# CCIG-Champalimaud/adell-mri

Hardware: AMD Instinct MI355X
Metric: volumes/sec 3D U-Net 128^3 2-ch seg (train step: fwd+loss+bwd+SGD) (higher is better)
Workload: dtype f32 (f16x3 split MFMA, fp32 accumulate); 1 GPU; BASELINE configs[1]: u-net-3d-resnet.yaml UNetPL, 2x128^3, batch 2/GPU, dice+focal, SGD-Nesterov; per_gpu_batch=2, parallelism=dp1, yaml=configs/u-net-3d-resnet.yaml, built_by=parse_config_unet -> get_segmentation_network('unet'), gradient_exchange=none (1 rank)

## Files before the change

### adell_mri_amd/_lib.py

```python
import ctypes
import os

_HERE = os.path.dirname(os.path.abspath(__file__))
LIB_PATH = os.environ.get("ADELL_HIP_LIBRARY") or os.path.join(_HERE, "libadellhip.so")

_lib = None

OK = 0
E_BADARG, E_UNSUPPORTED, E_HIP, E_NOMEM = -1, -2, -3, -4

ACT_IDS = {
    "identity": 0, "swish": 1, "silu": 1, "relu": 2, "leaky_relu": 3, "prelu": 4,
    "gelu": 5, "sigmoid": 6, "tanh": 7, "elu": 8,
}


class AdellHipError(RuntimeError):
    pass


class ConvDesc(ctypes.Structure):
    _fields_ = [(n, ctypes.c_int32) for n in (
        "N", "D", "H", "W", "C0", "C1", "Cout", "KD", "KH", "KW", "SD", "SH", "SW",
        "PD", "PH", "PW", "Do", "Ho", "Wo")]


class NormActDesc(ctypes.Structure):
    _fields_ = [
        ("N", ctypes.c_int64), ("V", ctypes.c_int64), ("C", ctypes.c_int32),
        ("stats_per_item", ctypes.c_int32), ("act", ctypes.c_int32),
        ("act_w_n", ctypes.c_int32), ("act_p", ctypes.c_float),
        ("drop_p", ctypes.c_float), ("seed", ctypes.c_uint64),
        ("rng_offset", ctypes.c_uint32),
    ]


class AdnSite(ctypes.Structure):
    _fields_ = [("y", ctypes.c_void_p), ("mean", ctypes.c_void_p), ("rstd", ctypes.c_void_p),
                ("keep_mask", ctypes.c_void_p), ("drop_p", ctypes.c_float),
                ("act_p", ctypes.c_float), ("act", ctypes.c_int32)]


_vp, _i, _l, _f = ctypes.c_void_p, ctypes.c_int, ctypes.c_long, ctypes.c_float
_d = ctypes.c_double

DECONF_MAX_HEADS = 8


class DeconfHeads(ctypes.Structure):
    _fields_ = [("n_heads", ctypes.c_int32), ("n_cont", ctypes.c_int32),
                ("K", ctypes.c_int32 * DECONF_MAX_HEADS), ("W", _vp * DECONF_MAX_HEADS),
                ("b", _vp * DECONF_MAX_HEADS), ("Wc", _vp), ("bc", _vp)]


class DeconfHeadGrads(ctypes.Structure):
    _fields_ = [("dW", _vp * DECONF_MAX_HEADS), ("db", _vp * DECONF_MAX_HEADS), ("dWc", _vp),
                ("dbc", _vp)]


class AttentionDesc(ctypes.Structure):
    _fields_ = [("BH", ctypes.c_int32), ("H", ctypes.c_int32), ("T", ctypes.c_int32),
                ("A", ctypes.c_int32), ("Dv", ctypes.c_int32), ("scale", _f), ("drop_p", _f),
                ("rng_offset", ctypes.c_uint32), ("seed", ctypes.c_uint64), ("bias", _vp),
                ("labels", _vp), ("nbias", ctypes.c_int32), ("nlab", ctypes.c_int32),
                ("strided", ctypes.c_int32), ("stride", ctypes.c_int64 * 3 * 8)]


SIGNATURES = {
    "adell_abi_version": (_i, []),
    "adell_last_error": (ctypes.c_char_p, []),
    "adell_pack_weight": (_i, [_vp, _vp, _i, _i, _i, _i, _i, _i, _vp]),
    "adell_conv3d_fwd_ntiles": (_i, [ctypes.POINTER(ConvDesc)]),
    "adell_plan_epoch": (_l, []),
    "adell_conv3d_fwd": (_i, [ctypes.POINTER(ConvDesc), _vp, _vp, _vp, _vp, _vp, _vp, _vp, _i, _vp]),
    "adell_conv3d_bwd_data": (_i, [ctypes.POINTER(ConvDesc), _vp, _vp, _vp, _vp, _vp]),
    "adell_pack_weight_f16x3_bytes": (_l, [_i, _i, _i, _i]),
    "adell_pack_weight_f16x3": (_i, [_vp, _vp, _vp, _i, _i, _i, _i, _i, _i, _vp]),
    "adell_conv3d_fwd_ntiles_f16x3": (_i, [ctypes.POINTER(ConvDesc)]),
    "adell_conv3d_fwd_ntiles_f16x3_ws": (_i, [ctypes.POINTER(ConvDesc)]),
    "adell_conv3d_fwd_f16x3": (_i, [ctypes.POINTER(ConvDesc)] + [_vp] * 8 + [_i, _vp, _vp]),
    "adell_conv3d_bwd_data_f16x3": (_i, [ctypes.POINTER(ConvDesc)] + [_vp] * 7),
    "adell_pack_weight_f16x3_multi": (_i, [_vp, _i, _l, _vp]),
    "adell_conv3d_bwd_data_s2_f16x3": (_i, [ctypes.POINTER(ConvDesc)] + [_vp] * 6),
    "adell_conv3d_bwd_data_s2_f16x3_add": (_i, [ctypes.POINTER(ConvDesc)] + [_vp] * 7),
    "adell_conv3d_fwd_s2_fused_applicable": (_i, [ctypes.POINTER(ConvDesc)]),
    "adell_conv3d_fwd_s2_fused_ntiles": (_i, [ctypes.POINTER(ConvDesc)]),
    "adell_conv3d_fwd_s2_fused": (_i, [ctypes.POINTER(ConvDesc)] + [_vp] * 6 + [_i, _vp, _vp]),
    "adell_conv3d_bwd_data_s2_fused_applicable": (_i, [ctypes.POINTER(ConvDesc)]),
    "adell_conv3d_bwd_data_s2_fused": (_i, [ctypes.POINTER(ConvDesc)] + [_vp] * 7),
    "adell_conv3d_splitk_workspace": (_l, [ctypes.POINTER(ConvDesc), _i]),
    "adell_conv3d_f16x3_plan": (_i, [ctypes.POINTER(ConvDesc), _i, _vp]),
    "adell_conv3d_fwd_f16x3_ws": (_i, [ctypes.POINTER(ConvDesc)] + [_vp] * 8 + [_i, _vp, _vp,
                                                                         ctypes.c_size_t, _vp]),
    "adell_conv3d_bwd_data_f16x3_ws": (_i, [ctypes.POINTER(ConvDesc)] + [_vp] * 7 + [ctypes.c_size_t, _vp]),
    "adell_conv3d_bwd_data_f16x3_add": (_i, [ctypes.POINTER(ConvDesc)] + [_vp] * 7
                                        + [ctypes.c_size_t, _vp]),
    "adell_conv3d_bwd_weight_workspace": (_l, [ctypes.POINTER(ConvDesc)]),
    "adell_conv3d_bwd_weight": (_i, [ctypes.POINTER(ConvDesc), _vp, _vp, _vp, _vp, _vp, _vp, ctypes.c_size_t, _vp]),
    "adell_conv3d_bwd_weight_f16x3_workspace": (_l, [ctypes.POINTER(ConvDesc)]),
    "adell_conv3d_bwd_weight_f16x3": (_i, [ctypes.POINTER(ConvDesc), _vp, _vp, _vp, _vp, _vp, _vp, _vp, _vp, ctypes.c_size_t, _vp]),
    "adell_bias_grad_workspace": (_l, [_l, _i]),
    "adell_bias_grad": (_i, [_vp, _l, _i, _vp, _vp, ctypes.c_size_t, _vp]),
    "adell_convtranspose3d_k2s2_bwd_weight_workspace": (_l, [_i, _i, _i, _i, _i, _i]),
    "adell_convtranspose3d_k2s2_bwd_weight": (_i, [_i, _i, _i, _i, _i, _i, _vp, _vp, _vp, _vp, ctypes.c_size_t, _vp]),
    "adell_convtranspose3d_fwd": (_i, [_i] * 9 + [_vp] * 5),
    "adell_convtranspose3d_bwd_data": (_i, [_i] * 9 + [_vp] * 4),
    "adell_convtranspose3d_bwd_weight_workspace": (_l, [_i] * 9),
    "adell_convtranspose3d_bwd_weight": (_i, [_i] * 9 + [_vp] * 4 + [ctypes.c_size_t, _vp]),
    "adell_convtranspose3d_k2s2_fwd": (_i, [_i, _i, _i, _i, _i, _i, _vp, _vp, _vp, _vp, _vp]),
    "adell_convtranspose3d_k2s2_bwd_data": (_i, [_i, _i, _i, _i, _i, _i, _vp, _vp, _vp, _vp]),
    "adell_stats_finalize_workspace": (_l, [_i, _i, _i]),
    "adell_stats_finalize": (_i, [_vp, _i, _i, _i, _l, _f, _i, _vp, _vp, _vp, ctypes.c_size_t, _vp]),
    "adell_bn_running_update": (_i, [_vp] * 5 + [_i, _l, _f, _f, _vp]),
    "adell_bn_stats_sums": (_i, [_vp, _i, _i, _i, _l, _vp, _vp, ctypes.c_size_t, _vp]),
    "adell_bn_stats_from_sums": (_i, [_vp, _i, _f, _vp, _vp, _vp, _vp, _vp, _f, _vp]),
    "adell_channel_partials_ntiles": (_i, [_l]),
    "adell_channel_partials": (_i, [_vp, _i, _l, _i, _vp, _vp]),
    "adell_norm_act_fwd": (_i, [ctypes.POINTER(NormActDesc), _vp, _vp, _vp, _vp, _vp, _vp, _vp, _vp]),
    "adell_norm_act_mask_bytes": (_l, [ctypes.POINTER(NormActDesc)]),
    "adell_norm_act_fwd_split": (_i, [ctypes.POINTER(NormActDesc)] + [_vp] * 7 + [_i, _vp, _vp]),
    "adell_split_rows_from_f32": (_i, [_vp, _i, _l, _i, _vp, _vp, _vp]),
    "adell_split_rows_to_f32": (_i, [_vp, _i, _l, _i, _vp, _vp, _vp]),
    "adell_conv3d_f16x3_rows_ok": (_i, [ctypes.POINTER(ConvDesc)]),
    "adell_conv3d_bwd_weight_f16x3_rows_ok": (_i, [ctypes.POINTER(ConvDesc)]),
    "adell_conv3d_bwd_weight_f16x3_plan": (_i, [ctypes.POINTER(ConvDesc), _vp]),
    "adell_conv3d_bwd_weight_f16x3_rows": (_i, [ctypes.POINTER(ConvDesc)] + [_vp] * 10
                                           + [ctypes.c_size_t, _vp]),
    "adell_conv3d_bwd_weight_f16x3_share": (_i, [ctypes.POINTER(ConvDesc)] + [_vp] * 8
                                            + [ctypes.c_size_t, _vp, _i]),
    "adell_conv3d_bwd_weight_f16x3_rows_share": (_i, [ctypes.POINTER(ConvDesc)] + [_vp] * 10
                                                 + [ctypes.c_size_t, _vp, _i]),
    "adell_conv3d_fwd_f16x3_rows": (_i, [ctypes.POINTER(ConvDesc)] + [_vp] * 10 + [_i, _vp, _vp]),
    "adell_norm_act_fwd_mask": (_i, [ctypes.POINTER(NormActDesc)] + [_vp] * 9),
    "adell_norm_act_bwd_from_dt": (_i, [ctypes.POINTER(NormActDesc)] + [_vp] * 5 + [_i, _i, _i, _vp, _vp,
                                                                              ctypes.c_size_t, _vp]),
    "adell_conv3d_bwd_data_f16x3_adn_ntiles": (_i, [ctypes.POINTER(ConvDesc)]),
    "adell_conv3d_bwd_data_f16x3_adn": (_i, [ctypes.POINTER(ConvDesc)] + [_vp] * 7
                                        + [ctypes.POINTER(AdnSite), ctypes.POINTER(AdnSite), _vp, _i, _vp]),
    "adell_norm_act_bwd_workspace": (_l, [ctypes.POINTER(NormActDesc)]),
    "adell_norm_act_bwd": (_i, [ctypes.POINTER(NormActDesc)] + [_vp] * 11 + [ctypes.c_size_t, _vp]),
    "adell_norm_act_plan": (_i, [ctypes.POINTER(NormActDesc)] + [_i] * 6 + [_vp]),
    "adell_norm_act_stats_plan": (_i, [_i, _i, _i, _vp]),
    "adell_norm_act_bwd_sums": (_i, [ctypes.POINTER(NormActDesc)] + [_vp] * 11 + [ctypes.c_size_t, _vp]),
    "adell_norm_act_bwd_apply_sums": (_i, [ctypes.POINTER(NormActDesc)] + [_vp] * 10
                                      + [ctypes.c_size_t, _vp]),
    "adell_norm_act_bwd_lowrank": (_i, [ctypes.POINTER(NormActDesc), _vp, _vp, _vp, _i, _vp, _vp, _vp,
                                        _vp, ctypes.c_size_t, _vp]),
    "adell_dice_focal_workspace": (_l, [_i, _l]),
    "adell_dice_focal_fwd": (_i, [_vp, _vp, _i, _l, _f, _f, _f, _f, _f, _vp, _vp, _vp, _vp, ctypes.c_size_t, _vp]),
    "adell_dice_focal_bwd": (_i, [_vp, _vp, _i, _l, _f, _f, _f, _f, _f, _vp, _f, _f, _vp, _vp]),
    "adell_dice_focal_bwd_dev": (_i, [_vp, _vp, _i, _l, _f, _f, _f, _f, _f, _vp, _vp, _vp, _vp, _vp]),
    "adell_class_sums_workspace": (_l, [_i, _l, _i]),
    "adell_class_sums_fwd": (_i, [_vp, _vp, _i, _l, _i, _vp, _vp, ctypes.c_size_t, _vp]),
    "adell_class_sums_bwd": (_i, [_vp, _vp, _i, _l, _i, _vp, _vp]),
    "adell_sgd_step": (_i, [_vp, _vp, _vp, _l, _f, _f, _f, _i, _i, _f, _vp]),
    "adell_adamw_step": (_i, [_vp, _vp, _vp, _vp, _l, _f, _d, _d, _f, _f, _l, _f, _vp]),
    "adell_adam_step": (_i, [_vp, _vp, _vp, _vp, _l, _f, _d, _d, _f, _f, _l, _f, _vp]),
    "adell_ema_update": (_i, [_vp, _vp, _l, _f, _vp]),
    "adell_layernorm_fwd": (_i, [_vp, _vp, _vp, _vp, _vp, _vp, _l, _i, _f, _vp]),
    "adell_layernorm_bwd_workspace": (_l, [_l, _i]),
    "adell_layernorm_bwd": (_i, [_vp] * 8 + [_l, _i, _vp, ctypes.c_size_t, _vp]),
    "adell_add_bcast": (_i, [_vp, _vp, _vp, _l, _l, _vp]),
    "adell_sum_bcast": (_i, [_vp, _vp, _l, _l, _vp]),
    "adell_attention_fwd": (_i, [ctypes.POINTER(AttentionDesc)] + [_vp] * 6),
    "adell_attention_bwd": (_i, [ctypes.POINTER(AttentionDesc)] + [_vp] * 10),
    "adell_attention_plan": (_i, [_i] * 5 + [_vp]),
    "adell_attention_bias_grad_workspace_floats": (_l, [_i, _i]),
    "adell_attention_bias_grad": (_i, [ctypes.POINTER(AttentionDesc)] + [_vp] * 8 + [_l, _vp]),
    "adell_copy_channels": (_i, [_vp, _vp, _l, _i, _i, _i, _i, _vp]),
    "adell_interp_nearest_fwd": (_i, [_vp, _vp] + [_i] * 8 + [_vp]),
    "adell_interp_nearest_bwd": (_i, [_vp, _vp] + [_i] * 8 + [_vp]),
    "adell_interp_linear_fwd": (_i, [_vp, _vp] + [_i] * 8 + [_f] * 3 + [_i, _vp]),
    "adell_interp_linear_bwd": (_i, [_vp, _vp] + [_i] * 8 + [_f] * 3 + [_i, _vp]),
    "adell_fold_x_taps": (_i, [_vp, _vp] + [_i] * 8 + [_vp]),
    "adell_scale_bc": (_i, [_vp, _vp, _vp, _i, _l, _i, _vp]),
    "adell_scale_bc_dscale_workspace_floats": (_l, [_i, _l, _i]),
    "adell_scale_bc_dscale": (_i, [_vp, _vp, _vp, _i, _l, _i, _vp, _vp]),
    "adell_cse_apply": (_i, [_vp, _vp, _vp, _vp, _vp, _vp, _i, _l, _i, _vp]),
    "adell_cse_apply_bwd_workspace_floats": (_l, [_i, _l, _i]),
    "adell_cse_apply_bwd": (_i, [_vp, _vp, _vp, _vp, _vp, _vp, _vp, _vp, _i, _l, _i, _vp, _vp]),
    "adell_bcast_nc": (_i, [_vp, _vp, _i, _l, _i, _f, _vp]),
    "adell_maxpool3d_fwd": (_i, [ctypes.POINTER(ConvDesc), _vp, _vp, _vp, _vp]),
    "adell_maxpool3d_bwd": (_i, [ctypes.POINTER(ConvDesc), _vp, _vp, _vp, _vp]),
    "adell_dwconv3d_fwd": (_i, [_i] * 8 + [_vp] * 5),
    "adell_dwconv3d_bwd_data": (_i, [_i] * 8 + [_vp] * 4),
    "adell_dwconv3d_bwd_weight_workspace_floats": (_l, [_i] * 8),
    "adell_dwconv3d_bwd_weight": (_i, [_i] * 8 + [_vp] * 6),
    "adell_vicreg_scratch_floats": (_l, [_i, _i]),
    "adell_vicreg_fwd": (_i, [_vp, _vp, _i, _i, _f, _f, _vp, _vp, _vp]),
    "adell_vicreg_bwd": (_i, [_vp, _vp, _i, _i, _f, _f, _vp, _vp, _vp, _vp, _vp]),
    "adell_top_pairs_workspace_words": (_l, [_i, _i, _i]),
    "adell_top_pairs": (_i, [_vp, _vp, _i, _i, _i, _i, _vp, _l, _vp, _vp, _vp]),
    "adell_top_pairs_boxes": (_i, [_vp, _vp, _i, _i, ctypes.POINTER(ctypes.c_int), _i, _vp, _l, _vp,
                                   _vp, _vp]),
    "adell_gather_rows_fwd": (_i, [_vp, _vp, _i, _i, _i, _i, _i, _vp, _vp]),
    "adell_gather_rows_bwd": (_i, [_vp, _vp, _i, _i, _i, _i, _i, _vp, _vp]),
    "adell_dino_loss_plan": (_i, [_i, _i, _vp]),
    "adell_dino_loss_workspace_floats": (_l, [_i, _i]),
    "adell_dino_loss_fwd": (_i, [_vp, _vp, _vp, _i, _i, _f, _f, _i, _vp, _l, _vp, _vp, _vp, _vp]),
    "adell_dino_loss_bwd": (_i, [_vp, _vp, _vp, _vp, _vp, _vp, _f, _i, _i, _f, _f, _i, _vp, _vp,
                                 _vp]),
    "adell_dino_scores": (_i, [_vp, _vp, _vp, _i, _i, _i, _i, _f, _vp, _vp]),
    "adell_dino_center_sum": (_i, [_vp, _i, _i, _vp, _vp]),
    "adell_dino_center_apply": (_i, [_vp, _vp, _i, _f, _f, _f, _vp]),
    "adell_dino_sk_proto_sums": (_i, [_vp, _vp, _i, _i, _f, _vp, _vp]),
    "adell_dino_sk_sample_weights": (_i, [_vp, _vp, _i, _i, _f, _f, _vp, _vp]),
    "adell_dino_sk_final": (_i, [_vp, _vp, _vp, _i, _i, _f, _f, _vp, _vp]),
    "adell_l2_normalize_rows_fwd": (_i, [_vp, _i, _i, _f, _vp, _vp, _vp]),
    "adell_l2_normalize_rows_bwd": (_i, [_vp, _vp, _vp, _i, _i, _f, _vp, _vp]),
    "adell_row_inv_norm_fwd": (_i, [_vp, _vp, _i, _i, _vp, _vp]),
    "adell_row_inv_norm_bwd": (_i, [_vp, _vp, _vp, _i, _i, _vp, _vp]),
    "adell_row_mean_fwd": (_i, [_vp, _i, _i, _vp, _vp]),
    "adell_row_mean_bwd": (_i, [_vp, _i, _i, _vp, _vp]),
    "adell_col_scale": (_i, [_vp, _vp, _i, _i, _vp, _vp]),
    "adell_col_scale_dscale": (_i, [_vp, _vp, _i, _i, _vp, _vp]),
    "adell_ibot_mask_tokens_fwd": (_i, [_vp, _vp, _vp, _i, _i, _i, _i, _vp, _vp]),
    "adell_ibot_mask_tokens_bwd": (_i, [_vp, _vp, _i, _i, _i, _i, _vp, _vp, _vp]),
    "adell_ibot_token_sums_plan": (_i, [_i, _i, _i, _vp]),
    "adell_ibot_token_sums_workspace_doubles": (_l, [_i, _i, _i]),
    "adell_ibot_center_sum": (_i, [_vp, _i, _i, _vp, _vp]),
    "adell_ibot_token_sums": (_i, [_vp, _i, _i, _i, _i, _f, _vp, _l, _vp, _vp, _vp]),
    "adell_ibot_loss_fwd": (_i, [_vp, _vp, _vp, _vp, _i, _i, _i, _i, _f, _f, _i, _vp, _l, _vp, _vp,
                                 _vp, _vp]),
    "adell_ibot_bwd": (_i, [_vp, _vp, _vp, _vp, _vp, _vp, _vp, _i, _i, _i, _i, _i, _i, _f, _f, _i,
                            _vp, _vp]),
    "adell_ijepa_gather_fwd": (_i, [_vp, _vp, _i, _i, _i, _i, _vp, _vp]),
    "adell_ijepa_gather_bwd": (_i, [_vp, _vp, _i, _i, _i, _i, _vp, _vp]),
    "adell_ijepa_predictor_fwd": (_i, [_vp, _vp, _vp, _vp, _vp, _i, _i, _i, _i, _i, _vp, _vp]),
    "adell_ijepa_predictor_bwd": (_i, [_vp, _vp, _vp, _vp, _i, _i, _i, _i, _i, _vp, _vp, _vp, _vp]),
    "adell_ijepa_loss_fwd": (_i, [_vp, _vp, _vp, _i, _i, _i, _i, _vp, _vp, _vp, _vp]),
    "adell_ijepa_loss_bwd": (_i, [_vp, _vp, _vp, _vp, _vp, _i, _i, _i, _i, _vp, _vp]),
    "adell_mae_gather_rows": (_i, [_vp, _vp, _i, _i, _i, _i, _vp, _vp]),
    "adell_mae_restore_fwd": (_i, [_vp, _vp, _vp, _vp, _vp, _i, _i, _i, _i, _vp, _vp]),
    "adell_mae_restore_bwd_chunks": (_i, [_i, _i]),
    "adell_mae_restore_bwd": (_i, [_vp, _vp, _vp, _vp, _vp, _i, _i, _i, _i, _vp, _vp, _vp, _vp, _vp,
                                   _i, _vp]),
    "adell_mae_loss_fwd": (_i, [_vp, _vp, _i, _i, _i, _i, _vp, _vp, _vp]),
    "adell_mae_loss_bwd": (_i, [_vp, _vp, _vp, _i, _i, _i, _i, _vp, _vp]),
    "adell_mae_to_image": (_i, [_vp, _i, _i, _i, _i, _vp, _vp]),
    "adell_mae_from_image": (_i, [_vp, _i, _i, _i, _i, _vp, _vp]),
    "adell_cls_loss_fwd": (_i, [_i, _vp, _vp, _vp, _vp, _i, _i, _i, _vp, _vp, _vp, _vp]),
    "adell_cls_loss_bwd": (_i, [_i, _vp, _vp, _vp, _vp, _i, _vp, _i, _vp, _i, _i, _vp, _vp]),
    "adell_cls_roc_fwd": (_i, [_vp, _vp, _i, _vp, _vp, _vp, _vp]),
    "adell_cls_roc_bwd": (_i, [_vp, _vp, _vp, _vp, _i, _vp, _vp]),
    "adell_cls_mixup": (_i, [_vp, _vp, _vp, _i, _l, _vp, _vp]),
    "adell_cls_confusion_update": (_i, [_i, _vp, _vp, _vp, _l, _i, _vp, _vp]),
    "adell_cls_auroc_pairs": (_i, [_vp, _vp, _i, _vp, _vp]),
    "adell_mil_volume_to_slices": (_i, [_vp, _i, _i, _i, _i, _vp, _vp]),
    "adell_mil_slices_to_volume": (_i, [_vp, _i, _i, _i, _i, _vp, _vp]),
    "adell_mil_pool_fwd": (_i, [_i] + [_vp] * 5 + [_i] * 4 + [_vp] * 5),
    "adell_mil_pool_bwd": (_i, [_i] + [_vp] * 9 + [_i] * 4 + [_vp] * 7),
    "adell_mil_slice_tokens_fwd": (_i, [_vp, _vp, _vp, _i, _i, _i, _vp, _vp]),
    "adell_mil_slice_tokens_bwd": (_i, [_vp, _i, _i, _i, _i, _vp, _vp, _vp, _vp]),
    "adell_det_table_blocks": (_l, [_l]),
    "adell_det_positive_table": (_i, [_vp] + [_i] * 9 + [_f] + [_vp] * 4),
    "adell_det_loss_partials": (_l, [_l]),
    "adell_det_loss_fwd": (_i, [_vp] * 7 + [_f] * 3 + [_i] * 9 + [_vp] * 4),
    "adell_det_loss_bwd": (_i, [_vp] * 7 + [_f] * 3 + [_i] * 9 + [_vp] * 5),
    "adell_det_nms_max": (_i, []),
    "adell_det_nms": (_i, [_vp, _i, _f, _vp, _vp, _vp]),
    "adell_det_decode": (_i, [_vp] * 4 + [_i] + [_vp] * 3 + [_f] * 3 + [_i] * 6 + [_vp] * 5),
    "adell_det_match": (_i, [_vp, _vp, _i, _vp, _vp, _vp, _vp, _vp]),
    "adell_det_encode": (_i, [_vp] * 4 + [ctypes.c_double] * 4 + [_i] * 6 + [_vp, _vp]),
    "adell_adamw_amsgrad_step": (_i, [_vp, _vp, _vp, _vp, _vp, _l, _f, _d, _d, _f, _f, _l, _f, _vp]),
    "adell_eca_gates_fwd": (_i, [_vp, _i, _vp, _i, _vp, _i, _i, _f, _vp, _vp]),
    "adell_eca_gates_bwd": (_i, [_vp, _i, _vp, _vp, _i, _i, _vp]),
    "adell_eca_apply_fwd": (_i, [_vp, _vp, _i, _vp, _i, _l, _i, _vp]),
    "adell_eca_apply_bwd_workspace_doubles": (_l, [_i, _l, _i]),
    "adell_eca_apply_bwd": (_i, [_vp, _vp, _vp, _i, _vp, _vp, _vp, _i, _l, _i, _vp]),
    "adell_diffusion_noise": (_i, [_vp, _vp, _vp, _i, _vp, _vp, _i, _l, _vp]),
    "adell_diffusion_reverse_step": (_i, [_vp] * 5 + [_l] + [_f] * 7 + [_i, _vp]),
    "adell_mse_workspace_bytes": (_l, []),
    "adell_mse_fwd": (_i, [_vp, _vp, _l, _vp, _vp, _vp]),
    "adell_mse_bwd": (_i, [_vp, _vp, _vp, _l, _vp, _vp]),
    "adell_gp_route": (_i, [_i, _i, _i]),
    "adell_gp_phi_fwd": (_i, [_vp] * 6 + [_i] * 4 + [_f, _f] + [_vp] * 5),
    "adell_gp_phi_bwd": (_i, [_vp] * 11 + [_i] * 4 + [_f, _f] + [_vp] * 6),
    "adell_gp_cos": (_i, [_vp, _vp, _vp, _l, _i, _f, _vp, _vp]),
    "adell_gp_precision_update": (_i, [_vp, _vp, _i, _i, _i, _i, _f, _vp, _vp]),
    "adell_gp_variance": (_i, [_vp, _vp, _i, _i, _vp, _vp]),
    "adell_gp_sample": (_i, [_vp, _vp, _vp, _i, _i, _i, _vp, _vp, _vp, _vp]),
    "adell_ensemble_pool_fwd": (_i, [_vp, _vp, _vp, _i, _i, _vp, _vp, _vp]),
    "adell_ensemble_pool_bwd": (_i, [_vp, _vp, _vp, _vp, _i, _i, _vp, _vp]),
    "adell_ensemble_average_fwd": (_i, [_vp, _i, _i, _i, _vp, _vp]),
    "adell_ensemble_average_bwd": (_i, [_vp, _vp, _i, _i, _i, _vp, _vp]),
    "adell_be_expand": (_i, [_vp, _vp, _vp, _i, _i, _i, _f, _vp, _i, _l, _i, _vp]),
    "adell_be_members_sum": (_i, [_vp, _vp, _vp, _i, _i, _i, _f, _i, _vp, _i, _l, _i, _vp]),
    "adell_be_tgrad_workspace_doubles": (_l, [_i, _l, _i, _i]),
    "adell_be_tgrad": (_i, [_vp, _vp, _vp, _vp, _i, _i, _i, _f, _vp, _vp, _vp, _i, _l, _i, _vp]),
    "adell_deconf_split_fwd": (_i, [_vp, _vp, _vp, _i, _i, _i, _vp]),
    "adell_deconf_split_bwd": (_i, [_vp, _vp, _vp, _i, _i, _i, _vp]),
    "adell_deconf_corr_workspace_doubles": (_l, [_i, _i, _i]),
    "adell_deconf_corr_saved_doubles": (_l, [_i, _i, _i]),
    "adell_deconf_corr_fwd": (_i, [_vp, _i, _i, _i, _vp, _vp, _vp, _vp]),
    "adell_deconf_corr_bwd": (_i, [_vp, _vp, _vp, _i, _i, _i, _vp, _vp]),
# ... 193 lines not shown
```

### adell_mri_amd/csrc/norm_act.hip

```cpp
#include "common.h"

ADELL_RNG_STEP_DEFINE(norm_act)

#define ADELL_NA_GENERIC_MAXBLOCKS (256 * 16)
#define ADELL_NA_FAST_MAXROWS 1024
#define ADELL_NA_FAST_MAXC 1024
#define ADELL_STATS_FOLD_ABOVE 512
#define ADELL_STATS_FOLD_ROWS 256
#define ADELL_FIN8_SPAN 56
#define ADELL_FIN2_SPAN 32

__global__ __launch_bounds__(256) void adell_stats_finalize_kernel(
    const float* __restrict__ part, int N, int ntiles, int C, double count, float eps,
    int per_item, float* __restrict__ mean, float* __restrict__ rstd) {
  __shared__ double sh[8][32][2];
  const int cl = threadIdx.x & 31, sl = threadIdx.x >> 5;
  const int c = blockIdx.x * 32 + cl;
  const int nbeg = per_item ? blockIdx.y : 0, nend = per_item ? blockIdx.y + 1 : N;
  double s1 = 0.0, s2 = 0.0;
  if (c < C) {
    for (int n = nbeg; n < nend; ++n) {
      const float* p = part + ((size_t)n * ntiles * C + c) * 2;
      int t = sl;
      for (; t + ADELL_FIN8_SPAN < ntiles; t += 64) {
        float2 v[8];
#pragma unroll
        for (int u = 0; u < 8; ++u)
          v[u] = *reinterpret_cast<const float2*>(p + (size_t)(t + 8 * u) * C * 2);
#pragma unroll
        for (int u = 0; u < 8; ++u) {
          s1 += (double)v[u].x;
          s2 += (double)v[u].y;
        }
      }
      for (; t < ntiles; t += 8) {
        const float2 v = *reinterpret_cast<const float2*>(p + (size_t)t * C * 2);
        s1 += (double)v.x;
        s2 += (double)v.y;
      }
    }
  }
  sh[sl][cl][0] = s1;
  sh[sl][cl][1] = s2;
  __syncthreads();
  if (sl == 0 && c < C) {
    double a = 0.0, b = 0.0;
#pragma unroll
    for (int k = 0; k < 8; ++k) {
      a += sh[k][cl][0];
      b += sh[k][cl][1];
    }
    const double cnt = per_item ? count : count * N;
    const double m = a / cnt;
    double var = b / cnt - m * m;
    if (var < 0.0) var = 0.0;
    const size_t o = per_item ? (size_t)blockIdx.y * C + c : (size_t)c;
    mean[o] = (float)m;
    rstd[o] = (float)(1.0 / sqrt(var + (double)eps));
  }
}

__global__ __launch_bounds__(256) void adell_stats_fold_kernel(const float* __restrict__ part,
                                                               int ntiles, int C, int Z,
                                                               float* __restrict__ out,
                                                               int pstride, int poff) {
  __shared__ double sh[8][32][2];
  const int cl = threadIdx.x & 31, sl = threadIdx.x >> 5;
  const int c = blockIdx.x * 32 + cl, n = blockIdx.y, z = blockIdx.z;
  const int t0 = z * ADELL_STATS_FOLD_ROWS;
  const int t1 = t0 + ADELL_STATS_FOLD_ROWS < ntiles ? t0 + ADELL_STATS_FOLD_ROWS : ntiles;
  double s1 = 0.0, s2 = 0.0;
  if (c < C) {
    const float* p = part + ((size_t)n * ntiles * pstride + poff + c) * 2;
    int t = t0 + sl;
    for (; t + ADELL_FIN8_SPAN < t1; t += 64) {
      float2 v[8];
#pragma unroll
      for (int u = 0; u < 8; ++u)
        v[u] = *reinterpret_cast<const float2*>(p + (size_t)(t + 8 * u) * pstride * 2);
#pragma unroll
      for (int u = 0; u < 8; ++u) {
        s1 += (double)v[u].x;
        s2 += (double)v[u].y;
      }
    }
    for (; t < t1; t += 8) {
      const float2 v = *reinterpret_cast<const float2*>(p + (size_t)t * pstride * 2);
      s1 += (double)v.x;
      s2 += (double)v.y;
    }
  }
  sh[sl][cl][0] = s1;
  sh[sl][cl][1] = s2;
  __syncthreads();
  if (sl == 0 && c < C) {
    double a = 0.0, b = 0.0;
#pragma unroll
    for (int k = 0; k < 8; ++k) {
      a += sh[k][cl][0];
      b += sh[k][cl][1];
    }
    float* o = out + (((size_t)n * Z + z) * C + c) * 2;
    o[0] = (float)a;
    o[1] = (float)b;
  }
}

struct AdellNaStatsPlan {
  int levels;
  int Z;
  long ws_bytes;
};

static AdellNaStatsPlan adell_na_stats_plan(long N, long ntiles, long C) {
  AdellNaStatsPlan p = {1, 0, 0};
  if (ntiles <= ADELL_STATS_FOLD_ABOVE) return p;
  p.levels = 2;
  p.Z = (int)((ntiles + ADELL_STATS_FOLD_ROWS - 1) / ADELL_STATS_FOLD_ROWS);
  p.ws_bytes = (long)sizeof(float) * N * p.Z * C * 2;
  return p;
}

extern "C" long adell_stats_finalize_workspace(int N, int ntiles, int C) {
  return adell_na_stats_plan(N, ntiles, C).ws_bytes;
}

extern "C" int adell_norm_act_stats_plan(int N, int ntiles, int C, long* out) {
  ADELL_REQUIRE(out && N > 0 && ntiles > 0 && C > 0, "norm_act_stats_plan: bad arguments");
  const AdellNaStatsPlan p = adell_na_stats_plan(N, ntiles, C);
  out[0] = p.levels;
  out[1] = p.Z;
  out[2] = p.ws_bytes;
  out[3] = ADELL_FIN8_SPAN + 1;
  out[4] = ADELL_FIN2_SPAN + 1;
  return ADELL_OK;
}

extern "C" int adell_stats_finalize(const float* partials, int N, int ntiles, int C,
                                    long count, float eps, int per_item, float* mean,
                                    float* rstd, void* workspace, size_t workspace_bytes,
                                    void* stream) {
  ADELL_REQUIRE(N > 0 && ntiles > 0 && C > 0 && count > 0, "stats_finalize: bad dims");
  const AdellNaStatsPlan sp = adell_na_stats_plan(N, ntiles, C);
  ADELL_REQUIRE(sp.levels == 1 || (workspace && (long)workspace_bytes >= sp.ws_bytes),
                "stats_finalize: workspace too small");
  ADELL_REQUIRE(partials && mean && rstd, "stats_finalize: null pointer");
  hipStream_t st = (hipStream_t)stream;
  if (sp.levels == 2) {
    const int Z = sp.Z;
    hipLaunchKernelGGL(adell_stats_fold_kernel, dim3(adell_cdiv(C, 32), N, Z), dim3(256), 0, st,
                       partials, ntiles, C, Z, (float*)workspace, C, 0);
    partials = (const float*)workspace;
    ntiles = Z;
  }
  hipLaunchKernelGGL(adell_stats_finalize_kernel, dim3(adell_cdiv(C, 32), per_item ? N : 1),
                     dim3(256), 0, st, partials, N, ntiles, C, (double)count, eps, per_item, mean,
                     rstd);
  ADELL_CHECK_HIP(hipGetLastError());
  return ADELL_OK;
}

__global__ __launch_bounds__(256) void adell_bn_running_update_kernel(
    const float* __restrict__ mean, const float* __restrict__ rstd, float* __restrict__ rmean,
    float* __restrict__ rvar, long long* __restrict__ nbt, int C, float unbias, float eps,
    float momentum) {
  long long t = nbt != nullptr ? nbt[0] + 1 : 0;
  const float mom = momentum >= 0.f ? momentum : 1.f / (float)t;
  __syncthreads();
  for (int c = threadIdx.x; c < C; c += 256) {
    const float r = rstd[c];
    const float var = (1.f / (r * r) - eps) * unbias;
    rmean[c] = rmean[c] * (1.f - mom) + mom * mean[c];
    rvar[c] = rvar[c] * (1.f - mom) + mom * var;
  }
  if (threadIdx.x == 0 && nbt != nullptr) nbt[0] = t;
}

extern "C" int adell_bn_running_update(const float* mean, const float* rstd, float* running_mean,
                                       float* running_var, long long* num_batches_tracked, int C,
                                       long count, float eps, float momentum, void* stream) {
  ADELL_REQUIRE(mean && rstd && running_mean && running_var && C > 0 && count > 0,
                "bn_running_update: bad arguments");
  ADELL_REQUIRE(momentum >= 0.f || num_batches_tracked != nullptr,
                "bn_running_update: the cumulative average needs num_batches_tracked");
  const float unbias = (float)((double)count / (double)(count > 1 ? count - 1 : 1));
  hipLaunchKernelGGL(adell_bn_running_update_kernel, dim3(1), dim3(256), 0, (hipStream_t)stream, mean,
                     rstd, running_mean, running_var, num_batches_tracked, C, unbias, eps, momentum);
  ADELL_CHECK_HIP(hipGetLastError());
  return ADELL_OK;
}

#define ADELL_STATS_SLAB 1024
__global__ __launch_bounds__(256) void adell_channel_partials_kernel(
    const float* __restrict__ x, long V, int C, float* __restrict__ part,
    int ntiles) {
  __shared__ float sh[256][2];
  const int n = blockIdx.y, tile = blockIdx.x;
  const long v0 = (long)tile * ADELL_STATS_SLAB;
  long v1 = v0 + ADELL_STATS_SLAB;
  if (v1 > V) v1 = V;
  const int CG = C < 256 ? C : 256;
  const int VL = 256 / CG;
  const int cl = threadIdx.x % CG, vl = threadIdx.x / CG;
  for (int cb = 0; cb < C; cb += CG) {
    const int c = cb + cl;
    float s1 = 0.f, s2 = 0.f;
    if (vl < VL && c < C) {
      const float* p = x + ((size_t)n * V) * C + c;
      for (long v = v0 + vl; v < v1; v += VL) {
        const float t = p[v * C];
        s1 += t;
        s2 += t * t;
      }
    }
    sh[threadIdx.x][0] = s1;
    sh[threadIdx.x][1] = s2;
    __syncthreads();
    if (vl == 0 && c < C) {
      float a = 0.f, b = 0.f;
      for (int k = 0; k < VL; ++k) {
        a += sh[k * CG + cl][0];
        b += sh[k * CG + cl][1];
      }
      float* o = part + (((size_t)n * ntiles + tile) * C + c) * 2;
      o[0] = a;
      o[1] = b;
    }
    __syncthreads();
  }
}

__global__ __launch_bounds__(256) void adell_channel_partials_vec_kernel(
    const float* __restrict__ x, long V, int C, float* __restrict__ part, int ntiles) {
  __shared__ f32x4 sh[256][2];
  const int n = blockIdx.y, tile = blockIdx.x;
  const long v0 = (long)tile * ADELL_STATS_SLAB;
  long v1 = v0 + ADELL_STATS_SLAB;
  if (v1 > V) v1 = V;
  const int CQ = C >> 2;
  const int QG = CQ < 256 ? CQ : 256;
  const int VL = 256 / QG;
  const int ql = threadIdx.x % QG, vl = threadIdx.x / QG;
  for (int qb = 0; qb < CQ; qb += QG) {
    const int q = qb + ql;
    f32x4 s1 = {0.f, 0.f, 0.f, 0.f}, s2 = {0.f, 0.f, 0.f, 0.f};
    if (vl < VL && q < CQ) {
      const f32x4* p = reinterpret_cast<const f32x4*>(x + ((size_t)n * V) * C) + q;
      long v = v0 + vl;
      for (; v + 3L * VL < v1; v += 4L * VL) {
        const f32x4 a = p[v * CQ], b = p[(v + VL) * CQ], c = p[(v + 2L * VL) * CQ],
                    d = p[(v + 3L * VL) * CQ];
        s1 += (a + b) + (c + d);
        s2 += (a * a + b * b) + (c * c + d * d);
      }
      for (; v < v1; v += VL) {
        const f32x4 a = p[v * CQ];
        s1 += a;
        s2 += a * a;
      }
    }
    sh[threadIdx.x][0] = s1;
    sh[threadIdx.x][1] = s2;
    __syncthreads();
    if (vl == 0 && q < CQ) {
      f32x4 a = {0.f, 0.f, 0.f, 0.f}, b = {0.f, 0.f, 0.f, 0.f};
      for (int k = 0; k < VL; ++k) {
        a += sh[k * QG + ql][0];
        b += sh[k * QG + ql][1];
      }
      float* o = part + (((size_t)n * ntiles + tile) * C + 4 * q) * 2;
      o[0] = a.x; o[1] = b.x; o[2] = a.y; o[3] = b.y; o[4] = a.z; o[5] = b.z; o[6] = a.w; o[7] = b.w;
    }
    __syncthreads();
  }
}

extern "C" int adell_channel_partials_ntiles(long V) {
  return (int)((V + ADELL_STATS_SLAB - 1) / ADELL_STATS_SLAB);
}

extern "C" int adell_channel_partials(const float* x, int N, long V, int C,
                                      float* partials, void* stream) {
  ADELL_REQUIRE(x && partials, "channel_partials: null pointer");
  ADELL_REQUIRE(N > 0 && V > 0 && C > 0, "channel_partials: bad dims");
  const int nt = adell_channel_partials_ntiles(V);
  if ((C & 3) == 0 && (((uintptr_t)x) & 15) == 0)
    hipLaunchKernelGGL(adell_channel_partials_vec_kernel, dim3(nt, N), dim3(256), 0,
                       (hipStream_t)stream, x, V, C, partials, nt);
  else
    hipLaunchKernelGGL(adell_channel_partials_kernel, dim3(nt, N), dim3(256), 0,
                       (hipStream_t)stream, x, V, C, partials, nt);
  ADELL_CHECK_HIP(hipGetLastError());
  return ADELL_OK;
}


struct NormActArgs {
  const float* x;
  const float* mean;
  const float* rstd;
  const float* gamma;
  const float* beta;
  const float* act_w;
  float* out;
  long VC;
  long total;
  int C;
  int stat_stride_n;
  int act;
  int act_w_n;
  float act_p;
  float drop_p;
  uint32_t seed_lo, seed_hi;
  uint32_t rng_offset;
  int vec;
  unsigned long long* mask;
  long groups;
  int rev;
  int split;
  float split_scale;
};

__global__ __launch_bounds__(256) void adell_norm_act_fwd_kernel(NormActArgs a) {
  const long n4 = a.vec ? (a.total >> 2) : 0;
  const float keep_scale = a.drop_p > 0.f ? 1.0f / (1.0f - a.drop_p) : 1.0f;
  for (long i = blockIdx.x * (long)blockDim.x + threadIdx.x; i < n4;
       i += (long)gridDim.x * blockDim.x) {
    const long e = i << 2;
    const int c = (int)(e % a.C);
    const long nidx = e / a.VC;
    float4 v = reinterpret_cast<const float4*>(a.x)[i];
    float h[4] = {v.x, v.y, v.z, v.w};
    uint4 r = make_uint4(0, 0, 0, 0);
    if (a.drop_p > 0.f)
      r = adell_philox4((uint32_t)i, (uint32_t)(i >> 32), a.rng_offset + g_adell_rng_step, 0u, a.seed_lo,
                        a.seed_hi);
    const uint32_t rr[4] = {r.x, r.y, r.z, r.w};
#pragma unroll
    for (int j = 0; j < 4; ++j) {
      const int cj = c + j;
      float t = h[j];
      if (a.mean) {
        const long si = nidx * a.stat_stride_n + cj;
        t = (t - a.mean[si]) * a.rstd[si];
      }
      if (a.gamma) t = t * a.gamma[cj];
      if (a.beta) t = t + a.beta[cj];
      if (a.drop_p > 0.f) {
        const float u = (float)(rr[j] >> 8) * (1.0f / 16777216.0f);
        t = (u >= a.drop_p) ? t * keep_scale : 0.f;
      }
      float p = a.act_p;
      if (a.act_w) p = a.act_w[a.act_w_n > 1 ? cj : 0];
      h[j] = adell_act_fwd(a.act, t, p);
    }
    reinterpret_cast<float4*>(a.out)[i] = make_float4(h[0], h[1], h[2], h[3]);
  }
  const long tail0 = n4 << 2;
  for (long e = tail0 + blockIdx.x * (long)blockDim.x + threadIdx.x; e < a.total;
       e += (long)gridDim.x * blockDim.x) {
    const int cj = (int)(e % a.C);
    const long nidx = e / a.VC;
    float t = a.x[e];
    if (a.mean) {
      const long si = nidx * a.stat_stride_n + cj;
      t = (t - a.mean[si]) * a.rstd[si];
    }
    if (a.gamma) t = t * a.gamma[cj];
    if (a.beta) t = t + a.beta[cj];
    if (a.drop_p > 0.f) {
      const uint4 r = adell_philox4((uint32_t)(e >> 2), (uint32_t)(e >> 34),
                                    a.rng_offset + g_adell_rng_step, 0u, a.seed_lo, a.seed_hi);
      const uint32_t rr[4] = {r.x, r.y, r.z, r.w};
      const float u = (float)(rr[e & 3] >> 8) * (1.0f / 16777216.0f);
      t = (u >= a.drop_p) ? t * keep_scale : 0.f;
    }
    float p = a.act_p;
    if (a.act_w) p = a.act_w[a.act_w_n > 1 ? cj : 0];
    a.out[e] = adell_act_fwd(a.act, t, p);
  }
}

#ifndef ADELL_EW_UNROLL
#define ADELL_EW_UNROLL 4
#endif
#define ADELL_ACT_DISPATCH(KERN, act, grid, st, args)                                         \
  switch (act) {                                                                              \
    case 0: hipLaunchKernelGGL(KERN<0>, grid, dim3(256), 0, st, args); break;                 \
    case 1: hipLaunchKernelGGL(KERN<1>, grid, dim3(256), 0, st, args); break;                 \
    case 2: hipLaunchKernelGGL(KERN<2>, grid, dim3(256), 0, st, args); break;                 \
    case 3: hipLaunchKernelGGL(KERN<3>, grid, dim3(256), 0, st, args); break;                 \
    case 4: hipLaunchKernelGGL(KERN<4>, grid, dim3(256), 0, st, args); break;                 \
    case 5: hipLaunchKernelGGL(KERN<5>, grid, dim3(256), 0, st, args); break;                 \
    case 6: hipLaunchKernelGGL(KERN<6>, grid, dim3(256), 0, st, args); break;                 \
    case 7: hipLaunchKernelGGL(KERN<7>, grid, dim3(256), 0, st, args); break;                 \
    default: hipLaunchKernelGGL(KERN<8>, grid, dim3(256), 0, st, args); break;                \
  }
#define ADELL_ACT_DISPATCH_LR(KERN, act, grid, st, args)                                      \
  switch (act) {                                                                              \
    case 0: hipLaunchKernelGGL((KERN<0, true>), grid, dim3(256), 0, st, args); break;         \
    case 1: hipLaunchKernelGGL((KERN<1, true>), grid, dim3(256), 0, st, args); break;         \
    case 2: hipLaunchKernelGGL((KERN<2, true>), grid, dim3(256), 0, st, args); break;         \
    case 3: hipLaunchKernelGGL((KERN<3, true>), grid, dim3(256), 0, st, args); break;         \
    case 4: hipLaunchKernelGGL((KERN<4, true>), grid, dim3(256), 0, st, args); break;         \
    case 5: hipLaunchKernelGGL((KERN<5, true>), grid, dim3(256), 0, st, args); break;         \
    case 6: hipLaunchKernelGGL((KERN<6, true>), grid, dim3(256), 0, st, args); break;         \
    case 7: hipLaunchKernelGGL((KERN<7, true>), grid, dim3(256), 0, st, args); break;         \
    default: hipLaunchKernelGGL((KERN<8, true>), grid, dim3(256), 0, st, args); break;        \
  }
#ifndef ADELL_EW_MAXBLOCKS
#define ADELL_EW_MAXBLOCKS 65535
#endif
#ifndef ADELL_EW_CONTIG
#define ADELL_EW_CONTIG 1
#endif
__device__ __forceinline__ unsigned adell_ew_block(int rev) {
  if (!rev) return blockIdx.x;
  const unsigned nb = gridDim.x, per = nb >> 3;
  if (per == 0 || (nb & 7)) return nb - 1 - blockIdx.x;
  return (blockIdx.x & 7) * per + (per - 1 - (blockIdx.x >> 3));
}
#if ADELL_EW_CONTIG
#define ADELL_EW_RANGE(n4)                                                                   \
  const long chunk_ = (((n4) + gridDim.x - 1) / gridDim.x + 1023) / 1024 * 1024;            \
  const long jbeg = (long)adell_ew_block(a.rev) * chunk_;                         \
  const long jend = jbeg + chunk_ < (n4) ? jbeg + chunk_ : (n4);                             \
  const long j0 = jbeg + threadIdx.x;                                                        \
  const long stride = 256
#else
#define ADELL_EW_RANGE(n4)                                                                   \
  const long jbeg = (long)blockIdx.x * 256;                                                  \
  const long jend = (n4);                                                                    \
  const long j0 = jbeg + threadIdx.x;                                                        \
  const long stride = (long)gridDim.x * 256
#endif
template <int ACT> __global__ void adell_norm_act_fwd_fast_kernel(NormActArgs a);

static int adell_na_fill(NormActArgs* a, const adell_norm_act_desc* d) {
  ADELL_REQUIRE(d != nullptr, "norm_act: null descriptor");
  ADELL_REQUIRE(d->N > 0 && d->V > 0 && d->C > 0, "norm_act: bad dims");
  ADELL_REQUIRE(d->act >= 0 && d->act <= ADELL_ACT_ELU, "norm_act: unknown activation");
  ADELL_REQUIRE(d->drop_p >= 0.f && d->drop_p < 1.f, "norm_act: dropout p must be in [0,1)");
  ADELL_REQUIRE(d->stats_per_item == 0 || d->stats_per_item == 1,
                "norm_act: stats_per_item must be 0/1");
  a->VC = d->V * d->C;
  a->total = d->N * a->VC;
  a->C = d->C;
  a->stat_stride_n = d->stats_per_item ? d->C : 0;
  a->act = d->act;
  a->act_w_n = d->act_w_n;
  a->act_p = d->act_p;
  a->drop_p = d->drop_p;
  a->seed_lo = (uint32_t)(d->seed & 0xffffffffu);
  a->seed_hi = (uint32_t)(d->seed >> 32);
  a->rng_offset = d->rng_offset;
  a->rev = 0;
  return ADELL_OK;
}

struct AdellNaPlan {
  int fwd;
  long fwd_gx, fwd_gy;
  int bwd;
  long rows;
  long apply_gx, apply_gy;
  int finalize;
  long ws_bytes;
  long mask_bytes;
};

static long adell_ew_blocks(long units) {
  long b = (units + 255) / 256;
  if (b > ADELL_NA_GENERIC_MAXBLOCKS) b = ADELL_NA_GENERIC_MAXBLOCKS;
  if (b < 1) b = 1;
  return b;
}
static long adell_na_fast_grid(long VC) {
  long bx = ((VC >> 2) + 256 * ADELL_EW_UNROLL - 1) / (256 * ADELL_EW_UNROLL);
  if (bx > ADELL_EW_MAXBLOCKS) bx = ADELL_EW_MAXBLOCKS;
  if (bx < 1) bx = 1;
  return bx;
}
static long adell_na_fast_blocks(long V, int C) {
  long bx = ((V * C >> 2) + 256 * 4 - 1) / (256 * 4);
  if (bx > ADELL_NA_FAST_MAXROWS) bx = ADELL_NA_FAST_MAXROWS;
  if (bx < 1) bx = 1;
  return bx;
}

static long adell_na_mask_bytes(const adell_norm_act_desc* d) {
  return d->N * ((d->V * d->C + 255) / 256) * 32;
}
static long adell_na_bwd_ws_bytes(const adell_norm_act_desc* d) {
  long nt = adell_channel_partials_ntiles(d->V);
  const long ntf = adell_na_fast_blocks(d->V, d->C);
  if (ntf > nt) nt = ntf;
  return (long)sizeof(float) * (d->N * nt * d->C * 2 + 2 * d->N * d->C);
}

static AdellNaPlan adell_na_plan(const adell_norm_act_desc* d, bool al_x, bool al_out, bool al_dout,
                                 bool al_dx, bool want_mask, bool split, int lr_co, bool norm,
                                 bool affine_grads) {
  AdellNaPlan p = {};
  const long VC = d->V * d->C, total = d->N * VC;
  const bool mask = want_mask && d->drop_p > 0.f;
  const bool fast_c = adell_is_pow2(d->C) && d->C <= ADELL_NA_FAST_MAXC;
  {
    const bool aligned = al_x && al_out;
    const bool vec = d->C % 4 == 0 && aligned;
    const bool narrow = d->C < 4 && VC % 4 == 0 && !mask && aligned;
    if ((vec || narrow) && fast_c && (VC >> 2) < (1L << 40)) {
      p.fwd = vec ? ADELL_NA_FAST : ADELL_NA_NARROW;
      p.fwd_gx = adell_na_fast_grid(VC);
      p.fwd_gy = d->N;
    } else if (mask || split) {
      p.fwd = ADELL_NA_REFUSED;
    } else {
      p.fwd = vec ? ADELL_NA_FLOAT4 : ADELL_NA_SCALAR;
      p.fwd_gx = adell_ew_blocks(vec ? total >> 2 : total);
      p.fwd_gy = 1;
    }
    if (split && d->C < 16) p.fwd = ADELL_NA_REFUSED, p.fwd_gx = p.fwd_gy = 0;
    p.mask_bytes = mask && p.fwd == ADELL_NA_FAST ? adell_na_mask_bytes(d) : 0;
  }
  {
    const bool aligned = al_x && al_dout && al_dx;
    const bool vec = d->C % 4 == 0 && aligned;
    const bool narrow = d->C < 4 && VC % 4 == 0 && lr_co == 0 && aligned;
    const bool fast = (vec || narrow) && fast_c;
    const bool reduce = norm || affine_grads;
    if (fast) {
      p.bwd = vec ? ADELL_NA_FAST : ADELL_NA_NARROW;
      p.rows = reduce ? adell_na_fast_blocks(d->V, d->C) : 0;
      p.apply_gx = adell_na_fast_grid(VC);
      p.apply_gy = d->N;
    } else if (lr_co != 0) {
      p.bwd = ADELL_NA_REFUSED;
    } else {
      p.bwd = vec ? ADELL_NA_FLOAT4 : ADELL_NA_SCALAR;
      p.rows = reduce ? adell_channel_partials_ntiles(d->V) : 0;
      p.apply_gx = adell_ew_blocks(vec ? total / 4 : total);
      p.apply_gy = 1;
    }
    if (p.bwd != ADELL_NA_REFUSED && reduce) {
      p.finalize = d->stats_per_item && !affine_grads && d->N <= 65535 ? ADELL_NA_FIN_PER_ITEM
                                                                       : ADELL_NA_FIN_ALL_ITEMS;
      p.ws_bytes = adell_na_bwd_ws_bytes(d);
    }
  }
  return p;
}

static bool adell_na_al16(const void* p) { return ((uintptr_t)p & 15) == 0; }

extern "C" int adell_norm_act_plan(const adell_norm_act_desc* d, int aligned, int want_mask,
                                   int split, int lowrank, int norm, int affine_grads, long* out) {
  ADELL_REQUIRE(d && out && d->N > 0 && d->V > 0 && d->C > 0, "norm_act_plan: bad arguments");
  ADELL_REQUIRE(lowrank >= 0 && lowrank <= 4, "norm_act_plan: 0..4 low-rank factors");
  const AdellNaPlan p =
      adell_na_plan(d, (aligned & ADELL_NA_ALIGNED_X) != 0, (aligned & ADELL_NA_ALIGNED_OUT) != 0,
                    (aligned & ADELL_NA_ALIGNED_DOUT) != 0, (aligned & ADELL_NA_ALIGNED_DX) != 0,
                    want_mask != 0, split != 0, lowrank, norm != 0, affine_grads != 0);
  out[0] = p.fwd; out[1] = p.fwd_gx; out[2] = p.fwd_gy;
  out[3] = p.bwd; out[4] = p.rows; out[5] = p.apply_gx; out[6] = p.apply_gy;
  out[7] = p.finalize; out[8] = p.ws_bytes; out[9] = p.mask_bytes;
  return ADELL_OK;
}

extern "C" long adell_norm_act_mask_bytes(const adell_norm_act_desc* d) {
  if (!d || d->N <= 0 || d->V <= 0 || d->C <= 0) return ADELL_E_BADARG;
  return adell_na_mask_bytes(d);
}

static int adell_norm_act_fwd_impl(const adell_norm_act_desc* d, const float* x,
                                   const float* mean, const float* rstd,
                                   const float* gamma, const float* beta,
                                   const float* act_w, float* out, void* keep_mask,
                                   void* stream, int split = 0, int split_exp = 0) {
  NormActArgs a = {};
  int rc = adell_na_fill(&a, d);
  if (rc != ADELL_OK) return rc;
  a.split = split;
  a.split_scale = __builtin_ldexpf(1.0f, split_exp);
  a.mask = (unsigned long long*)keep_mask;
  a.groups = (a.VC + 255) / 256;
  ADELL_REQUIRE(x && out, "norm_act_fwd: null pointer");
  ADELL_REQUIRE((mean == nullptr) == (rstd == nullptr), "norm_act_fwd: mean/rstd mismatch");
  ADELL_REQUIRE(d->C % 4 == 0 || a.total < (1L << 31),
                "norm_act_fwd: C %% 4 != 0 needs < 2^31 elements");
  a.x = x; a.mean = mean; a.rstd = rstd; a.gamma = gamma; a.beta = beta;
  a.act_w = act_w; a.out = out;
  const AdellNaPlan p = adell_na_plan(d, adell_na_al16(x), adell_na_al16(out), true, true,
                                      keep_mask != nullptr, split != 0, 0, false, false);
  if (p.fwd == ADELL_NA_REFUSED) {
    adell_set_error("norm_act_fwd_mask / _split: needs a power-of-two C <= 1024 and 16-byte aligned tensors");
    return ADELL_E_UNSUPPORTED;
  }
  a.vec = p.fwd == ADELL_NA_FLOAT4;
  const dim3 grid((unsigned)p.fwd_gx, (unsigned)p.fwd_gy);
  if (p.fwd == ADELL_NA_FAST || p.fwd == ADELL_NA_NARROW) {
    ADELL_ACT_DISPATCH(adell_norm_act_fwd_fast_kernel, d->act, grid, (hipStream_t)stream, a);
  } else {
    hipLaunchKernelGGL(adell_norm_act_fwd_kernel, grid, dim3(256), 0, (hipStream_t)stream, a);
  }
  ADELL_CHECK_HIP(hipGetLastError());
  return ADELL_OK;
}

extern "C" int adell_norm_act_fwd(const adell_norm_act_desc* d, const float* x,
                                  const float* mean, const float* rstd,
                                  const float* gamma, const float* beta,
                                  const float* act_w, float* out, void* stream) {
  return adell_norm_act_fwd_impl(d, x, mean, rstd, gamma, beta, act_w, out, nullptr, stream);
}

extern "C" int adell_norm_act_fwd_mask(const adell_norm_act_desc* d, const float* x,
                                       const float* mean, const float* rstd,
                                       const float* gamma, const float* beta,
                                       const float* act_w, float* out, void* keep_mask,
                                       void* stream) {
  ADELL_REQUIRE(d && (d->drop_p == 0.f || keep_mask), "norm_act_fwd_mask: null mask");
  return adell_norm_act_fwd_impl(d, x, mean, rstd, gamma, beta, act_w, out,
                                 d->drop_p > 0.f ? keep_mask : nullptr, stream);
}

extern "C" int adell_norm_act_fwd_split(const adell_norm_act_desc* d, const float* x,
                                        const float* mean, const float* rstd,
                                        const float* gamma, const float* beta,
                                        const float* act_w, void* out_rows, int split_exp,
                                        void* keep_mask, void* stream) {
  ADELL_REQUIRE(d && d->N > 0 && d->V > 0 && d->C > 0, "norm_act_fwd_split: bad dims");
  ADELL_REQUIRE(split_exp >= -100 && split_exp <= 100, "norm_act_fwd_split: bad exponent");
  ADELL_REQUIRE(adell_na_plan(d, adell_na_al16(x), adell_na_al16(out_rows), true, true,
                              keep_mask != nullptr, true, 0, false, false).fwd == ADELL_NA_FAST,
                "norm_act_fwd_split: C must be a power of two in 16..1024, the tensors 16-byte aligned");
  return adell_norm_act_fwd_impl(d, x, mean, rstd, gamma, beta, act_w, (float*)out_rows,
                                 d->drop_p > 0.f ? keep_mask : nullptr, stream, 1, split_exp);
}

typedef _Float16 na_half8 __attribute__((ext_vector_type(8)));
typedef _Float16 na_half4 __attribute__((ext_vector_type(4)));
__global__ __launch_bounds__(256) void adell_rows_from_f32_kernel(const float* __restrict__ x,
                                                                  const int* __restrict__ xk,
                                                                  char* __restrict__ rows, long V,
                                                                  int C, long total) {
  const int nch = C >> 4;
  for (long i = blockIdx.x * 256L + threadIdx.x; i < total; i += (long)gridDim.x * 256L) {
    const int ch = (int)(i % nch);
    const long v = i / nch;
    const int n = (int)(v / V);
    const float scale = __int_as_float((xk[n * nch + ch] + 127) << 23);
    const float4* p = reinterpret_cast<const float4*>(x + v * C + ch * 16);
    na_half8 o[4];
#pragma unroll
    for (int q = 0; q < 4; ++q) {
      const float4 t4 = p[q];
      const float t[4] = {t4.x * scale, t4.y * scale, t4.z * scale, t4.w * scale};
#pragma unroll
      for (int j = 0; j < 4; ++j) {
        const _Float16 h = (_Float16)t[j];
        o[q >> 1][(q & 1) * 4 + j] = h;
        o[2 + (q >> 1)][(q & 1) * 4 + j] = (_Float16)(t[j] - (float)h);
      }
    }
    na_half8* dst = reinterpret_cast<na_half8*>(rows + i * 64);
    dst[0] = o[0]; dst[1] = o[1]; dst[2] = o[2]; dst[3] = o[3];
  }
}
__global__ __launch_bounds__(256) void adell_rows_to_f32_kernel(const char* __restrict__ rows,
                                                                const int* __restrict__ xk,
                                                                float* __restrict__ x, long V, int C,
                                                                long total) {
  const int nch = C >> 4;
  for (long i = blockIdx.x * 256L + threadIdx.x; i < total; i += (long)gridDim.x * 256L) {
    const int ch = (int)(i % nch);
    const long v = i / nch;
    const int n = (int)(v / V);
    const float inv = __int_as_float((127 - xk[n * nch + ch]) << 23);
    const na_half8* src = reinterpret_cast<const na_half8*>(rows + i * 64);
    const na_half8 h0 = src[0], h1 = src[1], l0 = src[2], l1 = src[3];
    float4* p = reinterpret_cast<float4*>(x + v * C + ch * 16);
    p[0] = make_float4(((float)h0[0] + (float)l0[0]) * inv, ((float)h0[1] + (float)l0[1]) * inv,
                       ((float)h0[2] + (float)l0[2]) * inv, ((float)h0[3] + (float)l0[3]) * inv);
    p[1] = make_float4(((float)h0[4] + (float)l0[4]) * inv, ((float)h0[5] + (float)l0[5]) * inv,
                       ((float)h0[6] + (float)l0[6]) * inv, ((float)h0[7] + (float)l0[7]) * inv);
    p[2] = make_float4(((float)h1[0] + (float)l1[0]) * inv, ((float)h1[1] + (float)l1[1]) * inv,
                       ((float)h1[2] + (float)l1[2]) * inv, ((float)h1[3] + (float)l1[3]) * inv);
    p[3] = make_float4(((float)h1[4] + (float)l1[4]) * inv, ((float)h1[5] + (float)l1[5]) * inv,
                       ((float)h1[6] + (float)l1[6]) * inv, ((float)h1[7] + (float)l1[7]) * inv);
  }
}
static int adell_rows_convert(const void* src, void* dst, int N, long V, int C, const int* xk,
                              int to_rows, void* stream) {
  ADELL_REQUIRE(src && dst && xk && N > 0 && V > 0 && C >= 16 && C % 16 == 0,
                "split rows: bad arguments (C must be a multiple of 16)");
  ADELL_REQUIRE((((uintptr_t)src | (uintptr_t)dst) & 15) == 0, "split rows: 16-byte aligned tensors");
  const long total = (long)N * V * (C >> 4);
  long blocks = (total + 255) / 256;
  if (blocks > 65536) blocks = 65536;
  if (to_rows)
    hipLaunchKernelGGL(adell_rows_from_f32_kernel, dim3((unsigned)blocks), dim3(256), 0,
                       (hipStream_t)stream, (const float*)src, xk, (char*)dst, V, C, total);
  else
    hipLaunchKernelGGL(adell_rows_to_f32_kernel, dim3((unsigned)blocks), dim3(256), 0,
                       (hipStream_t)stream, (const char*)src, xk, (float*)dst, V, C, total);
  ADELL_CHECK_HIP(hipGetLastError());
  return ADELL_OK;
}
extern "C" int adell_split_rows_from_f32(const float* x, int N, long V, int C, const int* xk,
                                         void* rows, void* stream) {
  return adell_rows_convert(x, rows, N, V, C, xk, 1, stream);
}
extern "C" int adell_split_rows_to_f32(const void* rows, int N, long V, int C, const int* xk,
                                       float* x, void* stream) {
  return adell_rows_convert(rows, x, N, V, C, xk, 0, stream);
}

struct NormActBwdArgs {
  const float* x;
  const float* dout;
  const float* mean;
  const float* rstd;
  const float* gamma;
  const float* beta;
  const float* act_w;
  const float* c1;
  const float* c2;
  float* dx;
  float* part;
  long V;
  long VC, total;
  int C, stat_stride_n, act, act_w_n, ntiles;
  float act_p, drop_p;
  uint32_t seed_lo, seed_hi, rng_offset;
  int rev;
  const float* lr_g;
  const float* lr_w;
  int lr_co, lr_shift;
};

__device__ __forceinline__ void adell_na_bwd_elem(const NormActBwdArgs& a, float x, float dout,
                                                  long nidx, int c, bool keep,
                                                  float keep_scale, float* dt, float* hn) {
  float h = x;
  if (a.mean) {
    const long si = nidx * a.stat_stride_n + c;
    h = (x - a.mean[si]) * a.rstd[si];
  }
  float t = h;
  if (a.gamma) t *= a.gamma[c];
  if (a.beta) t += a.beta[c];
  const float u = keep ? t * keep_scale : 0.f;
  float p = a.act_p;
  if (a.act_w) p = a.act_w[a.act_w_n > 1 ? c : 0];
  const float du = dout * adell_act_grad(a.act, u, p);
  *dt = keep ? du * keep_scale : 0.f;
  *hn = h;
}

__device__ __forceinline__ void adell_na_keep4(const NormActBwdArgs& a, long e4, bool keep[4]) {
  keep[0] = keep[1] = keep[2] = keep[3] = true;
  if (a.drop_p > 0.f) {
    const uint4 r = adell_philox4((uint32_t)e4, (uint32_t)(e4 >> 32), a.rng_offset + g_adell_rng_step, 0u,
                                  a.seed_lo, a.seed_hi);
    const uint32_t rr[4] = {r.x, r.y, r.z, r.w};
#pragma unroll
    for (int j = 0; j < 4; ++j)
      keep[j] = (float)(rr[j] >> 8) * (1.0f / 16777216.0f) >= a.drop_p;
  }
}

template <bool VEC>
__global__ __launch_bounds__(256) void adell_na_bwd_partials_kernel(NormActBwdArgs a) {
  __shared__ float sh[256][2][VEC ? 4 : 1];
  constexpr int W = VEC ? 4 : 1;
  const int n = blockIdx.y, tile = blockIdx.x;
  const long v0 = (long)tile * ADELL_STATS_SLAB;
  long v1 = v0 + ADELL_STATS_SLAB;
  if (v1 > a.V) v1 = a.V;
  const int CW = a.C / W;
  const int CG = CW < 256 ? CW : 256;
  const int VL = 256 / CG;
  const int cl = threadIdx.x % CG, vl = threadIdx.x / CG;
  const float keep_scale = a.drop_p > 0.f ? 1.0f / (1.0f - a.drop_p) : 1.0f;
  for (int cb = 0; cb < CW; cb += CG) {
    const int cw = cb + cl;
    float A[W], B[W];
#pragma unroll
    for (int j = 0; j < W; ++j) A[j] = B[j] = 0.f;
    if (vl < VL && cw < CW) {
      for (long v = v0 + vl; v < v1; v += VL) {
        const long e = ((long)n * a.V + v) * a.C + (long)cw * W;
        if constexpr (VEC) {
          const float4 xv = *reinterpret_cast<const float4*>(a.x + e);
          const float4 gv = *reinterpret_cast<const float4*>(a.dout + e);
          const float xs[4] = {xv.x, xv.y, xv.z, xv.w}, gs[4] = {gv.x, gv.y, gv.z, gv.w};
          bool keep[4];
          adell_na_keep4(a, e >> 2, keep);
#pragma unroll
          for (int j = 0; j < 4; ++j) {
            float dt, hn;
            adell_na_bwd_elem(a, xs[j], gs[j], n, cw * 4 + j, keep[j], keep_scale, &dt, &hn);
            A[j] += dt;
            B[j] += dt * hn;
          }
        } else {
          bool keep[4];
          adell_na_keep4(a, e >> 2, keep);
          float dt, hn;
          adell_na_bwd_elem(a, a.x[e], a.dout[e], n, cw, keep[e & 3], keep_scale, &dt, &hn);
          A[0] += dt;
          B[0] += dt * hn;
        }
      }
    }
#pragma unroll
    for (int j = 0; j < W; ++j) {
      sh[threadIdx.x][0][j] = A[j];
      sh[threadIdx.x][1][j] = B[j];
    }
    __syncthreads();
    if (vl == 0 && cw < CW) {
#pragma unroll
      for (int j = 0; j < W; ++j) {
        float s1 = 0.f, s2 = 0.f;
        for (int k = 0; k < VL; ++k) {
          s1 += sh[k * CG + cl][0][j];
          s2 += sh[k * CG + cl][1][j];
        }
        float* o = a.part + (((size_t)n * a.ntiles + tile) * a.C + cw * W + j) * 2;
        o[0] = s1;
        o[1] = s2;
      }
    }
    __syncthreads();
  }
}

__global__ __launch_bounds__(1024) void adell_na_bwd_finalize_kernel(
    const float* __restrict__ part, int N, int ntiles, int C, double count, int per_item,
    const float* __restrict__ gamma, float* __restrict__ c1, float* __restrict__ c2,
    float* __restrict__ dgamma, float* __restrict__ dbeta) {
  __shared__ double sh[32][32][2];
  const int cl = threadIdx.x & 31, sl = threadIdx.x >> 5;
  const int c = blockIdx.x * 32 + cl;
  double accA = 0.0, accB = 0.0;
  for (int n = 0; n < N; ++n) {
    double s1 = 0.0, s2 = 0.0;
    if (c < C)
      for (int t = sl; t < ntiles; t += 32) {
        const float2 v =
            *reinterpret_cast<const float2*>(part + (((size_t)n * ntiles + t) * C + c) * 2);
        s1 += (double)v.x;
        s2 += (double)v.y;
      }
    sh[sl][cl][0] = s1;
    sh[sl][cl][1] = s2;
    __syncthreads();
    if (sl == 0 && c < C) {
      double A = 0.0, B = 0.0;
#pragma unroll
      for (int k = 0; k < 32; ++k) {
        A += sh[k][cl][0];
        B += sh[k][cl][1];
      }
      accA += A;
      accB += B;
      if (per_item) {
        const double g = gamma ? (double)gamma[c] : 1.0;
        c1[(size_t)n * C + c] = (float)(g * A / count);
        c2[(size_t)n * C + c] = (float)(g * B / count);
      }
    }
    __syncthreads();
  }
  if (sl == 0 && c < C) {
    if (!per_item) {
      const double g = gamma ? (double)gamma[c] : 1.0;
      c1[c] = (float)(g * accA / (count * N));
      c2[c] = (float)(g * accB / (count * N));
    }
    if (dgamma) dgamma[c] = (float)accB;
    if (dbeta) dbeta[c] = (float)accA;
  }
}

__global__ __launch_bounds__(256) void adell_na_bwd_finalize_item_kernel(
    const float* __restrict__ part, int ntiles, int C, double count,
    const float* __restrict__ gamma, float* __restrict__ c1, float* __restrict__ c2,
    int pstride, int poff) {
  __shared__ double sh[32][8][2];
  const int cl = threadIdx.x & 7, sl = threadIdx.x >> 3;
  const int c = blockIdx.x * 8 + cl, n = blockIdx.y;
  double a0 = 0.0, a1 = 0.0, b0 = 0.0, b1 = 0.0;
  if (c < C) {
    int t = sl;
    for (; t + ADELL_FIN2_SPAN < ntiles; t += 64) {
      const float2 u =
          *reinterpret_cast<const float2*>(part + (((size_t)n * ntiles + t) * pstride + poff + c) * 2);
      const float2 v = *reinterpret_cast<const float2*>(
          part + (((size_t)n * ntiles + t + 32) * pstride + poff + c) * 2);
      a0 += (double)u.x; b0 += (double)u.y;
      a1 += (double)v.x; b1 += (double)v.y;
    }
    for (; t < ntiles; t += 32) {
      const float2 u =
          *reinterpret_cast<const float2*>(part + (((size_t)n * ntiles + t) * pstride + poff + c) * 2);
      a0 += (double)u.x; b0 += (double)u.y;
    }
  }
  sh[sl][cl][0] = a0 + a1;
  sh[sl][cl][1] = b0 + b1;
  __syncthreads();
  if (sl == 0 && c < C) {
    double A = 0.0, B = 0.0;
#pragma unroll
    for (int k = 0; k < 32; ++k) {
      A += sh[k][cl][0];
      B += sh[k][cl][1];
    }
    const double g = gamma ? (double)gamma[c] : 1.0;
    c1[(size_t)n * C + c] = (float)(g * A / count);
    c2[(size_t)n * C + c] = (float)(g * B / count);
  }
}

template <bool VEC>
__global__ __launch_bounds__(256) void adell_na_bwd_apply_kernel(NormActBwdArgs a) {
  constexpr int W = VEC ? 4 : 1;
  const long nw = a.total / W;
  const float keep_scale = a.drop_p > 0.f ? 1.0f / (1.0f - a.drop_p) : 1.0f;
  for (long i = blockIdx.x * (long)blockDim.x + threadIdx.x; i < nw;
       i += (long)gridDim.x * blockDim.x) {
    const long e = i * W;
    const int c = (int)(e % a.C);
    const long nidx = e / a.VC;
    bool keep[4];
    adell_na_keep4(a, e >> 2, keep);
    float xs[W], gs[W], out[W];
    if constexpr (VEC) {
      const float4 xv = *reinterpret_cast<const float4*>(a.x + e);
      const float4 gv = *reinterpret_cast<const float4*>(a.dout + e);
      xs[0] = xv.x; xs[1] = xv.y; xs[2] = xv.z; xs[3] = xv.w;
      gs[0] = gv.x; gs[1] = gv.y; gs[2] = gv.z; gs[3] = gv.w;
    } else {
      xs[0] = a.x[e];
      gs[0] = a.dout[e];
    }
#pragma unroll
    for (int j = 0; j < W; ++j) {
      const int cj = c + j;
      float dt, hn;
      adell_na_bwd_elem(a, xs[j], gs[j], nidx, cj, VEC ? keep[j] : keep[e & 3], keep_scale,
                        &dt, &hn);
      float r = dt;
      if (a.gamma) r *= a.gamma[cj];
      if (a.mean) {
        const long si = nidx * a.stat_stride_n + cj;
        r = a.rstd[si] * (r - a.c1[si] - hn * a.c2[si]);
      }
      out[j] = r;
    }
    if constexpr (VEC)
      *reinterpret_cast<float4*>(a.dx + e) = make_float4(out[0], out[1], out[2], out[3]);
    else
      a.dx[e] = out[0];
  }
}

template <int ACT, bool LR = false> __global__ void adell_na_bwd_apply_fast_kernel(NormActBwdArgs a);
template <int ACT, bool LR = false> __global__ void adell_na_bwd_partials_fast_kernel(NormActBwdArgs a);

static int adell_nab_fill(NormActBwdArgs* a, const adell_norm_act_desc* d) {
  ADELL_REQUIRE(d != nullptr, "norm_act_bwd: null descriptor");
  ADELL_REQUIRE(d->N > 0 && d->V > 0 && d->C > 0, "norm_act_bwd: bad dims");
  ADELL_REQUIRE(d->act >= 0 && d->act <= ADELL_ACT_ELU, "norm_act_bwd: unknown activation");
  ADELL_REQUIRE(d->drop_p >= 0.f && d->drop_p < 1.f, "norm_act_bwd: dropout p must be in [0,1)");
  a->V = d->V;
  a->VC = d->V * d->C;
  a->total = d->N * a->VC;
  a->C = d->C;
  a->stat_stride_n = d->stats_per_item ? d->C : 0;
  a->act = d->act;
  a->act_w_n = d->act_w_n;
  a->act_p = d->act_p;
  a->drop_p = d->drop_p;
  a->seed_lo = (uint32_t)(d->seed & 0xffffffffu);
  a->seed_hi = (uint32_t)(d->seed >> 32);
  a->rng_offset = d->rng_offset;
  a->ntiles = adell_channel_partials_ntiles(d->V);
  return ADELL_OK;
}

extern "C" long adell_norm_act_bwd_workspace(const adell_norm_act_desc* d) {
  if (!d || d->N <= 0 || d->V <= 0 || d->C <= 0) return ADELL_E_BADARG;
  return adell_na_bwd_ws_bytes(d);
}

static int adell_norm_act_bwd_impl(const adell_norm_act_desc* d, const float* x,
                                   const float* dout, const float* mean, const float* rstd,
                                   const float* gamma, const float* beta, const float* act_w,
                                   float* dx, float* dgamma, float* dbeta, void* workspace,
                                   size_t workspace_bytes, void* stream, const float* lr_g,
                                   const float* lr_w, int lr_co);

extern "C" int adell_norm_act_bwd(const adell_norm_act_desc* d, const float* x,
                                  const float* dout, const float* mean, const float* rstd,
                                  const float* gamma, const float* beta, const float* act_w,
                                  float* dx, float* dgamma, float* dbeta, void* workspace,
                                  size_t workspace_bytes, void* stream) {
  ADELL_REQUIRE(dout, "norm_act_bwd: null pointer");
  return adell_norm_act_bwd_impl(d, x, dout, mean, rstd, gamma, beta, act_w, dx, dgamma, dbeta,
                                 workspace, workspace_bytes, stream, nullptr, nullptr, 0);
}

extern "C" int adell_norm_act_bwd_lowrank(const adell_norm_act_desc* d, const float* x,
                                          const float* g, const float* w, int co,
                                          const float* mean, const float* rstd, float* dx,
                                          void* workspace, size_t workspace_bytes, void* stream) {
  ADELL_REQUIRE(d && g && w && co >= 1 && co <= 4, "norm_act_bwd_lowrank: 1..4 factors expected");
  return adell_norm_act_bwd_impl(d, x, x, mean, rstd, nullptr, nullptr, nullptr, dx, nullptr,
                                 nullptr, workspace, workspace_bytes, stream, g, w, co);
}

static AdellNaPlan adell_na_bwd_plan(const NormActBwdArgs& a, const adell_norm_act_desc* d, bool norm,
                                     bool affine_grads) {
  return adell_na_plan(d, adell_na_al16(a.x), true, adell_na_al16(a.dout), adell_na_al16(a.dx), false,
                       false, a.lr_g ? a.lr_co : 0, norm, affine_grads);
}

static void adell_na_bwd_partials_launch(NormActBwdArgs& a, const adell_norm_act_desc* d,
                                         const AdellNaPlan& p, hipStream_t st) {
  a.ntiles = (int)p.rows;
  const dim3 grid(a.ntiles, (unsigned)d->N);
  if (p.bwd == ADELL_NA_FAST || p.bwd == ADELL_NA_NARROW) {
    if (a.lr_g) {
      ADELL_ACT_DISPATCH_LR(adell_na_bwd_partials_fast_kernel, d->act, grid, st, a);
    } else {
      ADELL_ACT_DISPATCH(adell_na_bwd_partials_fast_kernel, d->act, grid, st, a);
    }
  } else if (p.bwd == ADELL_NA_FLOAT4)
    hipLaunchKernelGGL(adell_na_bwd_partials_kernel<true>, grid, dim3(256), 0, st, a);
  else
    hipLaunchKernelGGL(adell_na_bwd_partials_kernel<false>, grid, dim3(256), 0, st, a);
}

static void adell_na_bwd_apply_launch(const NormActBwdArgs& a, const adell_norm_act_desc* d,
                                      const AdellNaPlan& p, hipStream_t st) {
  const dim3 grid((unsigned)p.apply_gx, (unsigned)p.apply_gy);
  if (p.bwd == ADELL_NA_FAST || p.bwd == ADELL_NA_NARROW) {
    if (a.lr_g) {
      ADELL_ACT_DISPATCH_LR(adell_na_bwd_apply_fast_kernel, d->act, grid, st, a);
    } else {
      ADELL_ACT_DISPATCH(adell_na_bwd_apply_fast_kernel, d->act, grid, st, a);
    }
  } else if (p.bwd == ADELL_NA_FLOAT4)
    hipLaunchKernelGGL(adell_na_bwd_apply_kernel<true>, grid, dim3(256), 0, st, a);
  else
    hipLaunchKernelGGL(adell_na_bwd_apply_kernel<false>, grid, dim3(256), 0, st, a);
}

static int adell_norm_act_bwd_impl(const adell_norm_act_desc* d, const float* x,
                                   const float* dout, const float* mean, const float* rstd,
                                   const float* gamma, const float* beta, const float* act_w,
                                   float* dx, float* dgamma, float* dbeta, void* workspace,
                                   size_t workspace_bytes, void* stream, const float* lr_g,
                                   const float* lr_w, int lr_co) {
  NormActBwdArgs a = {};
  int rc = adell_nab_fill(&a, d);
  if (rc != ADELL_OK) return rc;
  a.lr_g = lr_g; a.lr_w = lr_w; a.lr_co = lr_co;
  a.lr_shift = adell_ilog2(d->C) - 2;
  hipStream_t st = (hipStream_t)stream;
  a.x = x; a.dout = dout; a.mean = mean; a.rstd = rstd; a.gamma = gamma; a.beta = beta;
  a.act_w = act_w; a.dx = dx;
  const AdellNaPlan p = adell_na_bwd_plan(a, d, mean != nullptr, dgamma || dbeta);
  ADELL_REQUIRE(p.bwd != ADELL_NA_REFUSED,
                "norm_act_bwd_lowrank: needs a power-of-two C in 4..1024 and aligned tensors");
  ADELL_REQUIRE(p.finalize == ADELL_NA_FIN_NONE || (workspace && (long)workspace_bytes >= p.ws_bytes),
                "norm_act_bwd: workspace too small");
  ADELL_REQUIRE(x && dout && dx, "norm_act_bwd: null pointer");
  ADELL_REQUIRE((mean == nullptr) == (rstd == nullptr), "norm_act_bwd: mean/rstd mismatch");
  if (p.finalize != ADELL_NA_FIN_NONE) {
    float* part = (float*)workspace;
    float* c1 = part + (size_t)p.ws_bytes / sizeof(float) - 2 * (size_t)d->N * d->C;
    float* c2 = c1 + (size_t)d->N * d->C;
    a.part = part; a.c1 = c1; a.c2 = c2;
    adell_na_bwd_partials_launch(a, d, p, st);
    if (p.finalize == ADELL_NA_FIN_PER_ITEM)
      hipLaunchKernelGGL(adell_na_bwd_finalize_item_kernel,
                         dim3(adell_cdiv(d->C, 8), (unsigned)d->N), dim3(256), 0, st,
                         (const float*)part, a.ntiles, d->C, (double)d->V, gamma, c1, c2, d->C, 0);
    else
      hipLaunchKernelGGL(adell_na_bwd_finalize_kernel, dim3(adell_cdiv(d->C, 32)), dim3(1024), 0,
                         st, (const float*)part, (int)d->N, a.ntiles, d->C, (double)d->V,
                         d->stats_per_item, gamma, c1, c2, dgamma, dbeta);
  }
  adell_na_bwd_apply_launch(a, d, p, st);
  ADELL_CHECK_HIP(hipGetLastError());
  return ADELL_OK;
}

struct NaConst {
  float m[4], r[4], g[4], b[4], p[4], c1[4], c2[4];
};

__device__ __forceinline__ void adell_na_consts(NaConst& k, const float* mean, const float* rstd,
                                                const float* gamma, const float* beta,
                                                const float* act_w, int act_w_n, float act_p,
                                                const float* c1, const float* c2, long sbase,
                                                int c, int cmask) {
#pragma unroll
  for (int j = 0; j < 4; ++j) {
    const int cj = (c + j) & cmask;
    k.m[j] = mean ? mean[sbase + cj] : 0.f;
    k.r[j] = rstd ? rstd[sbase + cj] : 1.f;
    k.g[j] = gamma ? gamma[cj] : 1.f;
    k.b[j] = beta ? beta[cj] : 0.f;
    k.p[j] = act_w ? act_w[act_w_n > 1 ? cj : 0] : act_p;
    k.c1[j] = c1 ? c1[sbase + cj] : 0.f;
    k.c2[j] = c2 ? c2[sbase + cj] : 0.f;
  }
}

struct NaLowRank {
  float w[4][4];
};
__device__ __forceinline__ void adell_na_lr_load(NaLowRank& l, const NormActBwdArgs& a, int c) {
#pragma unroll
  for (int o = 0; o < 4; ++o)
#pragma unroll
    for (int q = 0; q < 4; ++q)
      l.w[o][q] = o < a.lr_co ? a.lr_w[o * a.C + c + q] : 0.f;
}
__device__ __forceinline__ float4 adell_na_lr_dout(const NaLowRank& l, const NormActBwdArgs& a,
                                                   int n, long jj) {
  const float* g = a.lr_g + ((long)n * a.V + (jj >> a.lr_shift)) * a.lr_co;
  float4 r = make_float4(0.f, 0.f, 0.f, 0.f);
#pragma unroll
  for (int o = 0; o < 4; ++o)
    if (o < a.lr_co) {
      const float gv = g[o];
      r.x = fmaf(gv, l.w[o][0], r.x); r.y = fmaf(gv, l.w[o][1], r.y);
      r.z = fmaf(gv, l.w[o][2], r.z); r.w = fmaf(gv, l.w[o][3], r.w);
    }
  return r;
}

template <int ACT>
__global__ __launch_bounds__(256) void adell_norm_act_fwd_fast_kernel(NormActArgs a) {
  const int n = a.rev ? (int)(gridDim.y - 1 - blockIdx.y) : (int)blockIdx.y;
  const long n4 = a.VC >> 2;
  ADELL_EW_RANGE(n4);
  const int c = (int)((j0 << 2) & (a.C - 1));
  NaConst k;
  adell_na_consts(k, a.mean, a.rstd, a.gamma, a.beta, a.act_w, a.act_w_n, a.act_p, nullptr,
                  nullptr, (long)n * a.stat_stride_n, c, a.C - 1);
  const float keep_scale = a.drop_p > 0.f ? 1.0f / (1.0f - a.drop_p) : 1.0f;
  const float4* xin = reinterpret_cast<const float4*>(a.x) + (long)n * n4;
  float4* yout = reinterpret_cast<float4*>(a.out) + (long)n * n4;
  for (long j = j0; j < jend; j += stride * ADELL_EW_UNROLL) {
    float4 v[ADELL_EW_UNROLL];
#pragma unroll
    for (int u = 0; u < ADELL_EW_UNROLL; ++u)
      if (j + u * stride < jend) v[u] = xin[j + u * stride];
#pragma unroll
    for (int u = 0; u < ADELL_EW_UNROLL; ++u) {
      const long jj = j + u * stride;
      if (jj >= jend) break;
      float h[4] = {v[u].x, v[u].y, v[u].z, v[u].w};
      uint32_t rr[4] = {0, 0, 0, 0};
      if (a.drop_p > 0.f) {
        const long gi = (long)n * n4 + jj;
        const uint4 r = adell_philox4((uint32_t)gi, (uint32_t)(gi >> 32), a.rng_offset + g_adell_rng_step, 0u,
                                      a.seed_lo, a.seed_hi);
        rr[0] = r.x; rr[1] = r.y; rr[2] = r.z; rr[3] = r.w;
      }
      bool kept[4] = {true, true, true, true};
#pragma unroll
      for (int q = 0; q < 4; ++q) {
        float t = ((h[q] - k.m[q]) * k.r[q]) * k.g[q] + k.b[q];
        if (a.drop_p > 0.f) {
          const float uu = (float)(rr[q] >> 8) * (1.0f / 16777216.0f);
          kept[q] = uu >= a.drop_p;
          t = kept[q] ? t * keep_scale : 0.f;
        }
        h[q] = adell_act_fwd(ACT, t, k.p[q]);
      }
      if (a.split) {
        na_half4 hi, lo;
#pragma unroll
        for (int q = 0; q < 4; ++q) {
          const float t = __builtin_amdgcn_fmed3f(h[q] * a.split_scale, -65504.f, 65504.f);
          const _Float16 hh = (_Float16)t;
          hi[q] = hh;
          lo[q] = (_Float16)(t - (float)hh);
        }
        const int within = (int)((jj << 2) & 15);
        char* row = reinterpret_cast<char*>(a.out) + 4 * ((long)n * a.VC + (jj << 2) - within);
        *reinterpret_cast<na_half4*>(row + within * 2) = hi;
        *reinterpret_cast<na_half4*>(row + 32 + within * 2) = lo;
      } else {
        yout[jj] = make_float4(h[0], h[1], h[2], h[3]);
      }
      if (a.mask != nullptr) {
        unsigned long long b[4];
#pragma unroll
        for (int q = 0; q < 4; ++q) b[q] = __ballot(kept[q]);
        const int ln = threadIdx.x & 63;
        unsigned long long* w = a.mask + ((long)n * a.groups + (jj >> 6)) * 4;
        if (ln < 4) w[ln] = ln == 0 ? b[0] : (ln == 1 ? b[1] : (ln == 2 ? b[2] : b[3]));
        const unsigned long long live = __ballot(true);
        if (live < 15 && ln == 0) {
          if (!(live & 2)) w[1] = b[1];
          if (!(live & 4)) w[2] = b[2];
          w[3] = b[3];
        }
      }
    }
  }
}

template <int ACT, bool LR>
__global__ __launch_bounds__(256) void adell_na_bwd_apply_fast_kernel(NormActBwdArgs a) {
  const int n = blockIdx.y;
  const long n4 = a.VC >> 2;
  ADELL_EW_RANGE(n4);
  const int c = (int)((j0 << 2) & (a.C - 1));
  NaConst k;
  adell_na_consts(k, a.mean, a.rstd, a.gamma, a.beta, a.act_w, a.act_w_n, a.act_p, a.c1, a.c2,
                  (long)n * a.stat_stride_n, c, a.C - 1);
  const float keep_scale = a.drop_p > 0.f ? 1.0f / (1.0f - a.drop_p) : 1.0f;
  const float4* xin = reinterpret_cast<const float4*>(a.x) + (long)n * n4;
  const float4* gin = reinterpret_cast<const float4*>(a.dout) + (long)n * n4;
  float4* dxo = reinterpret_cast<float4*>(a.dx) + (long)n * n4;
  const bool norm = a.mean != nullptr;
  NaLowRank lr;
  if (LR) adell_na_lr_load(lr, a, c);
  for (long j = j0; j < jend; j += stride * ADELL_EW_UNROLL) {
    float4 xv[ADELL_EW_UNROLL], gv[ADELL_EW_UNROLL];
#pragma unroll
    for (int u = 0; u < ADELL_EW_UNROLL; ++u)
      if (j + u * stride < jend) {
        xv[u] = xin[j + u * stride];
        gv[u] = LR ? adell_na_lr_dout(lr, a, n, j + u * stride) : gin[j + u * stride];
      }
#pragma unroll
    for (int u = 0; u < ADELL_EW_UNROLL; ++u) {
      const long jj = j + u * stride;
      if (jj >= jend) break;
      const float xs[4] = {xv[u].x, xv[u].y, xv[u].z, xv[u].w};
      const float gs[4] = {gv[u].x, gv[u].y, gv[u].z, gv[u].w};
      bool keep[4];
      adell_na_keep4(a, (long)n * n4 + jj, keep);
      float o[4];
#pragma unroll
      for (int q = 0; q < 4; ++q) {
        const float hn = (xs[q] - k.m[q]) * k.r[q];
        const float t = hn * k.g[q] + k.b[q];
        const float uu = keep[q] ? t * keep_scale : 0.f;
        const float du = gs[q] * adell_act_grad(ACT, uu, k.p[q]);
        const float dt = keep[q] ? du * keep_scale : 0.f;
        float r = dt * k.g[q];
        if (norm) r = k.r[q] * (r - k.c1[q] - hn * k.c2[q]);
        o[q] = r;
      }
      dxo[jj] = make_float4(o[0], o[1], o[2], o[3]);
    }
  }
}

template <int ACT, bool LR>
__global__ __launch_bounds__(256) void adell_na_bwd_partials_fast_kernel(NormActBwdArgs a) {
  __shared__ float sh[8][256];
  const int n = blockIdx.y;
  const long n4 = a.VC >> 2;
  ADELL_EW_RANGE(n4);
  const int c = (int)((j0 << 2) & (a.C - 1));
  NaConst k;
  adell_na_consts(k, a.mean, a.rstd, a.gamma, a.beta, a.act_w, a.act_w_n, a.act_p, nullptr,
                  nullptr, (long)n * a.stat_stride_n, c, a.C - 1);
  const float keep_scale = a.drop_p > 0.f ? 1.0f / (1.0f - a.drop_p) : 1.0f;
  const float4* xin = reinterpret_cast<const float4*>(a.x) + (long)n * n4;
  const float4* gin = reinterpret_cast<const float4*>(a.dout) + (long)n * n4;
  float A[4] = {0.f, 0.f, 0.f, 0.f}, B[4] = {0.f, 0.f, 0.f, 0.f};
  NaLowRank lr;
  if (LR) adell_na_lr_load(lr, a, c);
  for (long j = j0; j < jend; j += stride * ADELL_EW_UNROLL) {
    float4 xv[ADELL_EW_UNROLL], gv[ADELL_EW_UNROLL];
#pragma unroll
    for (int u = 0; u < ADELL_EW_UNROLL; ++u)
      if (j + u * stride < jend) {
        xv[u] = xin[j + u * stride];
        gv[u] = LR ? adell_na_lr_dout(lr, a, n, j + u * stride) : gin[j + u * stride];
      }
#pragma unroll
    for (int u = 0; u < ADELL_EW_UNROLL; ++u) {
      const long jj = j + u * stride;
      if (jj >= jend) break;
      const float xs[4] = {xv[u].x, xv[u].y, xv[u].z, xv[u].w};
      const float gs[4] = {gv[u].x, gv[u].y, gv[u].z, gv[u].w};
      bool keep[4];
      adell_na_keep4(a, (long)n * n4 + jj, keep);
#pragma unroll
      for (int q = 0; q < 4; ++q) {
        const float hn = (xs[q] - k.m[q]) * k.r[q];
        const float t = hn * k.g[q] + k.b[q];
        const float uu = keep[q] ? t * keep_scale : 0.f;
        const float du = gs[q] * adell_act_grad(ACT, uu, k.p[q]);
        const float dt = keep[q] ? du * keep_scale : 0.f;
        A[q] += dt;
        B[q] += dt * hn;
      }
    }
  }
#pragma unroll
  for (int q = 0; q < 4; ++q) {
    sh[q][threadIdx.x] = A[q];
    sh[4 + q][threadIdx.x] = B[q];
  }
  __syncthreads();
  if (a.C < 4) {
    if (threadIdx.x < 2 * a.C) {
      const int ch = threadIdx.x % a.C, which = threadIdx.x / a.C;
      float s1 = 0.f;
      for (int kk = 0; kk < 256; ++kk)
        for (int q = ch; q < 4; q += a.C) s1 += sh[which * 4 + q][kk];
      a.part[(((size_t)n * a.ntiles + blockIdx.x) * a.C + ch) * 2 + which] = s1;
    }
    return;
  }
  const int CG = a.C >> 2;
  const int VL = CG >= 256 ? 1 : 256 / CG;
  const int nout = (CG < 256 ? CG : 256) * 8;
  for (int o = threadIdx.x; o < nout; o += 256) {
    const int cl = o % (nout / 8), q8 = o / (nout / 8);
    float s1 = 0.f;
    for (int kk = 0; kk < VL; ++kk) s1 += sh[q8][kk * CG + cl];
    const int quad = (int)(((jbeg + cl) << 2) & (a.C - 1));
    const int ch = quad + (q8 & 3);
    a.part[(((size_t)n * a.ntiles + blockIdx.x) * a.C + ch) * 2 + (q8 >> 2)] = s1;
  }
}


__global__ __launch_bounds__(256) void adell_na_bwd_apply_dt_kernel(NormActBwdArgs a) {
  const int n = blockIdx.y;
  const long n4 = a.VC >> 2;
  ADELL_EW_RANGE(n4);
  const int c = (int)((j0 << 2) & (a.C - 1));
  NaConst k;
  adell_na_consts(k, a.mean, a.rstd, nullptr, nullptr, nullptr, 0, 0.f, a.c1, a.c2,
                  (long)n * a.stat_stride_n, c, a.C - 1);
  const float4* xin = reinterpret_cast<const float4*>(a.x) + (long)n * n4;
  const float4* gin = reinterpret_cast<const float4*>(a.dout) + (long)n * n4;
  float4* dxo = reinterpret_cast<float4*>(a.dx) + (long)n * n4;
  for (long j = j0; j < jend; j += stride * ADELL_EW_UNROLL) {
    float4 xv[ADELL_EW_UNROLL], gv[ADELL_EW_UNROLL];
#pragma unroll
    for (int u = 0; u < ADELL_EW_UNROLL; ++u)
      if (j + u * stride < jend) {
        xv[u] = xin[j + u * stride];
        gv[u] = gin[j + u * stride];
      }
#pragma unroll
    for (int u = 0; u < ADELL_EW_UNROLL; ++u) {
      const long jj = j + u * stride;
      if (jj >= jend) break;
      const float xs[4] = {xv[u].x, xv[u].y, xv[u].z, xv[u].w};
      const float gs[4] = {gv[u].x, gv[u].y, gv[u].z, gv[u].w};
      float o[4];
#pragma unroll
      for (int q = 0; q < 4; ++q) {
        const float hn = (xs[q] - k.m[q]) * k.r[q];
        o[q] = k.r[q] * (gs[q] - k.c1[q] - hn * k.c2[q]);
      }
      dxo[jj] = make_float4(o[0], o[1], o[2], o[3]);
    }
  }
}

extern "C" int adell_norm_act_bwd_from_dt(const adell_norm_act_desc* d, const float* x,
                                          const float* dt, const float* mean, const float* rstd,
                                          const float* partials, int ntiles, int pstride, int poff,
                                          float* dx, void* workspace, size_t workspace_bytes,
                                          void* stream) {
  NormActBwdArgs a = {};
  int rc = adell_nab_fill(&a, d);
  if (rc != ADELL_OK) return rc;
  ADELL_REQUIRE(d->stats_per_item == 1 && d->N <= 65535,
                "norm_act_bwd_from_dt: instance statistics only");
  ADELL_REQUIRE(ntiles > 0 && pstride >= d->C && poff >= 0 && poff + d->C <= pstride,
                "norm_act_bwd_from_dt: bad partials layout");
  a.x = x; a.dout = dt; a.dx = dx;
  const AdellNaPlan p = adell_na_bwd_plan(a, d, true, false);
  ADELL_REQUIRE(p.bwd == ADELL_NA_FAST,
                "norm_act_bwd_from_dt: needs a power-of-two C in 4..1024 and aligned tensors");
  const AdellNaStatsPlan sp = adell_na_stats_plan(d->N, ntiles, d->C);
  const int Z = sp.Z;
  ADELL_REQUIRE(workspace && workspace_bytes >= sizeof(float) * 2 * (size_t)d->N * d->C + (size_t)sp.ws_bytes,
                "norm_act_bwd_from_dt: workspace too small");
  ADELL_REQUIRE(x && dt && dx && mean && rstd && partials, "norm_act_bwd_from_dt: null pointer");
  hipStream_t st = (hipStream_t)stream;
  float* c1 = (float*)workspace;
  float* c2 = c1 + (size_t)d->N * d->C;
  if (Z > 0) {
    float* folded = c2 + (size_t)d->N * d->C;
    hipLaunchKernelGGL(adell_stats_fold_kernel, dim3(adell_cdiv(d->C, 32), (unsigned)d->N, Z),
                       dim3(256), 0, st, partials, ntiles, d->C, Z, folded, pstride, poff);
    partials = folded;
    ntiles = Z;
    pstride = d->C;
    poff = 0;
  }
  hipLaunchKernelGGL(adell_na_bwd_finalize_item_kernel, dim3(adell_cdiv(d->C, 8), (unsigned)d->N),
                     dim3(256), 0, st, partials, ntiles, d->C, (double)d->V, (const float*)nullptr,
                     c1, c2, pstride, poff);
  a.x = x; a.dout = dt; a.mean = mean; a.rstd = rstd; a.c1 = c1; a.c2 = c2; a.dx = dx;
  hipLaunchKernelGGL(adell_na_bwd_apply_dt_kernel, dim3((unsigned)p.apply_gx, (unsigned)p.apply_gy),
                     dim3(256), 0, st, a);
  ADELL_CHECK_HIP(hipGetLastError());
  return ADELL_OK;
}

__global__ __launch_bounds__(256) void adell_prelu_wgrad_partial_kernel(NormActBwdArgs a, int chunk) {
  __shared__ float sh[4][64];
  const long rows = a.total / a.C;
  const long r0 = (long)blockIdx.x * chunk;
  long r1 = r0 + chunk;
  if (r1 > rows) r1 = rows;
  const int cl = threadIdx.x & 63, vl = threadIdx.x >> 6;
  const int c = blockIdx.y * 64 + cl;
  const float keep_scale = a.drop_p > 0.f ? 1.0f / (1.0f - a.drop_p) : 1.0f;
  float s = 0.f;
  if (c < a.C) {
    for (long r = r0 + vl; r < r1; r += 4) {
      const long n = r / a.V;
      const long e = r * a.C + c;
      float h = a.x[e];
      if (a.mean) {
        const long si = n * a.stat_stride_n + c;
        h = (h - a.mean[si]) * a.rstd[si];
      }
      float t = h;
      if (a.gamma) t *= a.gamma[c];
      if (a.beta) t += a.beta[c];
      bool keep[4];
      adell_na_keep4(a, e >> 2, keep);
      const float u = keep[e & 3] ? t * keep_scale : 0.f;
      if (u < 0.f) s += a.dout[e] * u;
    }
  }
  sh[vl][cl] = s;
  __syncthreads();
  if (vl == 0 && c < a.C)
    a.part[(size_t)blockIdx.x * a.C + c] = (sh[0][cl] + sh[1][cl]) + (sh[2][cl] + sh[3][cl]);
}

__global__ __launch_bounds__(1024) void adell_prelu_wgrad_final_kernel(
    const float* __restrict__ part, int nb, int C, int single, float* __restrict__ out) {
  __shared__ double sh[16][64];
  __shared__ double tot[64];
  const int cl = threadIdx.x & 63, vl = threadIdx.x >> 6;
  double grand = 0.0;
  for (int cb = 0; cb < C; cb += 64) {
    const int c = cb + cl;
    double s = 0.0;
    if (c < C)
      for (int b = vl; b < nb; b += 16) s += (double)part[(size_t)b * C + c];
    sh[vl][cl] = s;
    __syncthreads();
    if (vl == 0) {
      s = 0.0;
#pragma unroll
      for (int k = 0; k < 16; ++k) s += sh[k][cl];
      if (c < C && !single) out[c] = (float)s;
      tot[cl] = c < C ? s : 0.0;
    }
    __syncthreads();
    if (threadIdx.x == 0)
      for (int k = 0; k < 64; ++k) grand += tot[k];
    __syncthreads();
  }
  if (single && threadIdx.x == 0) out[0] = (float)grand;
}

static int adell_prelu_chunk(long rows) {
  long chunk = (rows + 1023) / 1024;
  if (chunk < 16) chunk = 16;
  return (int)((chunk + 3) / 4 * 4);
}

extern "C" long adell_prelu_wgrad_workspace(const adell_norm_act_desc* d) {
  if (!d || d->N <= 0 || d->V <= 0 || d->C <= 0) return ADELL_E_BADARG;
  const long rows = d->N * d->V;
  const int chunk = adell_prelu_chunk(rows);
  return (long)sizeof(float) * ((rows + chunk - 1) / chunk) * d->C;
}

extern "C" int adell_prelu_wgrad(const adell_norm_act_desc* d, const float* x, const float* dout,
                                 const float* mean, const float* rstd, const float* gamma,
                                 const float* beta, float* dact_w, void* workspace,
                                 size_t workspace_bytes, void* stream) {
  NormActBwdArgs a = {};
  int rc = adell_nab_fill(&a, d);
  if (rc != ADELL_OK) return rc;
  ADELL_REQUIRE(x && dout && dact_w && workspace, "prelu_wgrad: null pointer");
  ADELL_REQUIRE(d->act == ADELL_ACT_PRELU && (d->act_w_n == 1 || d->act_w_n == d->C),
                "prelu_wgrad: needs a PReLU with 1 or C parameters");
  ADELL_REQUIRE((long)workspace_bytes >= adell_prelu_wgrad_workspace(d),
                "prelu_wgrad: workspace too small");
  a.x = x; a.dout = dout; a.mean = mean; a.rstd = rstd; a.gamma = gamma; a.beta = beta;
  a.part = (float*)workspace;
  const long rows = d->N * d->V;
  const int chunk = adell_prelu_chunk(rows);
  const int nb = (int)((rows + chunk - 1) / chunk);
  hipStream_t st = (hipStream_t)stream;
  hipLaunchKernelGGL(adell_prelu_wgrad_partial_kernel, dim3(nb, adell_cdiv(d->C, 64)), dim3(256), 0,
                     st, a, chunk);
  hipLaunchKernelGGL(adell_prelu_wgrad_final_kernel, dim3(1), dim3(1024), 0, st,
                     (const float*)workspace, nb, d->C, d->act_w_n == 1 ? 1 : 0, dact_w);
  ADELL_CHECK_HIP(hipGetLastError());
  return ADELL_OK;
}

__global__ __launch_bounds__(256) void adell_bn_sums_kernel(const float* __restrict__ part, int N,
                                                            int ntiles, int C, double count,
                                                            double* __restrict__ rec) {
  __shared__ double sh[8][32][2];
  const int cl = threadIdx.x & 31, sl = threadIdx.x >> 5;
  const int c = blockIdx.x * 32 + cl;
  double s1 = 0.0, s2 = 0.0;
  if (c < C) {
    for (int n = 0; n < N; ++n) {
      const float* p = part + ((size_t)n * ntiles * C + c) * 2;
      int t = sl;
      for (; t + ADELL_FIN8_SPAN < ntiles; t += 64) {
        float2 v[8];
#pragma unroll
        for (int u = 0; u < 8; ++u)
          v[u] = *reinterpret_cast<const float2*>(p + (size_t)(t + 8 * u) * C * 2);
#pragma unroll
        for (int u = 0; u < 8; ++u) {
          s1 += (double)v[u].x;
          s2 += (double)v[u].y;
        }
      }
      for (; t < ntiles; t += 8) {
        const float2 v = *reinterpret_cast<const float2*>(p + (size_t)t * C * 2);
        s1 += (double)v.x;
        s2 += (double)v.y;
      }
    }
  }
  sh[sl][cl][0] = s1;
  sh[sl][cl][1] = s2;
  __syncthreads();
  if (sl == 0 && c < C) {
    double a = 0.0, b = 0.0;
#pragma unroll
    for (int k = 0; k < 8; ++k) {
      a += sh[k][cl][0];
      b += sh[k][cl][1];
    }
    rec[c] = a;
    rec[C + c] = b;
  }
  if (blockIdx.x == 0 && threadIdx.x == 0) rec[2 * C] = count * N;
}

extern "C" int adell_bn_stats_sums(const float* partials, int N, int ntiles, int C, long count,
// ... 173 lines not shown
```

### adell_mri_amd/functional.py

```python
import collections
import ctypes
import itertools
import math
import os
import weakref

import numpy as np
import torch
import torch.distributed as dist

from . import _lib, ops

_dropout_counter = itertools.count(1)

CONV_PRECISION = os.environ.get("ADELL_CONV_PRECISION", "f16x3")
FLAGS = {"s2class_always": bool(os.environ.get("ADELL_S2CLASS_ALWAYS")),
         "no_s2class": bool(os.environ.get("ADELL_NO_S2CLASS")),
         "no_fold": bool(os.environ.get("ADELL_NO_FOLD")),
         "no_adn_fuse": bool(os.environ.get("ADELL_NO_ADN_FUSE")),
         "no_lowrank": bool(os.environ.get("ADELL_NO_LOWRANK")),
         "wgrad_stream": os.environ.get("ADELL_WGRAD_STREAM", "1") != "0",
         "no_wgrad_share": bool(os.environ.get("ADELL_NO_WGRAD_SHARE")),
         "no_rows": bool(os.environ.get("ADELL_NO_ROWS")),
         "no_pointwise_gemm": bool(os.environ.get("ADELL_NO_POINTWISE_GEMM")),
         "no_seq_attention": bool(os.environ.get("ADELL_NO_SEQ_ATTENTION")),
         "no_mlp_fuse": not bool(os.environ.get("ADELL_MLP_FUSE")),
         "mlp_min_elems": int(os.environ.get("ADELL_MLP_MIN_ELEMS", str(1 << 20))),
         "no_cinfold_wgrad_f16": bool(os.environ.get("ADELL_NO_CINFOLD_WGRAD_F16"))}


def set_conv_precision(mode):
    global CONV_PRECISION
    if mode not in ("f16x3", "fp32"):
        raise ValueError("conv precision must be 'f16x3' or 'fp32'")
    CONV_PRECISION = mode
    _sync_dw_precision()


def _sync_dw_precision():
    if os.path.exists(_lib.LIB_PATH) and not os.environ.get("ADELL_DW_NOMFMA"):
        _lib.lib().adell_set_tuning(b"dw_nomfma", 1 if CONV_PRECISION == "fp32" else 0)


if CONV_PRECISION == "fp32":
    _sync_dw_precision()


class _Ref:

    __slots__ = ("obj",)

    def __init__(self, obj):
        self.obj = obj


_PACK_REG = {}
_PACK_BATCH = {"epoch": -1, "sig": None, "table": None, "blocks": 0}


class _PackFence:

    __slots__ = ("stream", "event")

    def __init__(self):
        self.stream = ops._stream().value
        self.event = torch.cuda.Event()
        self.event.record()

    def order(self):
        if ops._stream().value != self.stream:
            torch.cuda.current_stream().wait_event(self.event)


def _pack_tag(w):
    return (w._version, w.data_ptr(), ops.WEIGHT_EPOCH)


def _repack_registered():
    live = []
    for key, ent in list(_PACK_REG.items()):
        w = ent[0]()
        if w is None or not w.is_contiguous() or not w.is_cuda:
            del _PACK_REG[key]
            continue
        live.append((w, ent))
    if not live:
        return False
    rows, first = [], 0
    for w, ent in live:
        d0, d1 = w.shape[0], w.shape[1]
        taps = w.shape[2] * w.shape[3] * w.shape[4]
        rows.append((w.data_ptr(), ent[2].halfs.data_ptr(), ent[2].scale.data_ptr(), ent[1], d0,
                     d1, taps, first))
        first += d0 if ent[1] == 0 else d1
    sig = tuple(rows)
    if _PACK_BATCH["sig"] != sig and torch.cuda.is_current_stream_capturing():
        return False
    if _PACK_BATCH["sig"] != sig:
        _PACK_BATCH["table"] = torch.tensor(rows, dtype=torch.int64, device=live[0][0].device)
        _PACK_BATCH["sig"] = sig
        _PACK_BATCH["blocks"] = first
    ops.pack_weight_f16x3_multi(_PACK_BATCH["table"], len(rows), _PACK_BATCH["blocks"])
    fence = _PackFence()
    for w, ent in live:
        ent[3] = _pack_tag(w)
        ent[4] = fence
    _PACK_BATCH["epoch"] = ops.WEIGHT_EPOCH
    return True


def _tensor_pack_cache(w, key, build):
    cache = getattr(w, "_adell_packs", None)
    if cache is None:
        cache = w._adell_packs = {}
    tag = _pack_tag(w)
    hit = cache.get(key)
    if hit is not None and hit[0] == tag:
        if w.is_cuda:
            hit[2].order()
        return hit[1]
    p = build()
    cache[key] = (tag, p, _PackFence() if w.is_cuda else None)
    return p


def _packed(w, mode):
    split = CONV_PRECISION == "f16x3" and mode in (0, 1, 2, 3)
    transient = w.grad_fn is not None or getattr(w, "_adell_transient", False) \
        or (w._base is not None and getattr(w._base, "_adell_transient", False))
    if split and mode in (0, 1) and w.dim() == 5 and w.is_contiguous() and not transient:
        key = (id(w), mode)
        ent = _PACK_REG.get(key)
        if ent is not None and ent[0]() is not w:
            ent = None
        if ent is not None:
            if ent[3] == _pack_tag(w):
                ent[4].order()
                return ent[2]
            if _PACK_BATCH["epoch"] != ops.WEIGHT_EPOCH and _repack_registered() \
                    and ent[3] == _pack_tag(w):
                ent[4].order()
                return ent[2]
        p = ops.pack_weight_f16x3(w.detach(), mode)
        _PACK_REG[key] = [weakref.ref(w), mode, p, _pack_tag(w), _PackFence()]
        return p

    def build():
        wd = w.detach()
        if wd.dim() == 2:
            wd = wd.view(wd.shape[0], wd.shape[1], 1, 1, 1)
        if split and mode == 2:
            v = wd.permute(2, 3, 4, 1, 0).reshape(-1, wd.shape[0], 1, 1, 1)
            return ops.pack_weight_f16x3(v, 0)
        if split and mode == 3:
            return ops.pack_weight_f16x3(wd, 0)
        return ops.pack_weight_f16x3(wd, mode) if split else ops.pack_weight(wd, mode)
    return _tensor_pack_cache(w, (mode, split), build)


def _packed_s2_classes(w, padding):
    def build():
        wd = w.detach()
        packs = []
        for c in range(8):
            par = (c >> 2, (c >> 1) & 1, c & 1)
            t0 = [(par[a] + padding[a]) & 1 for a in range(3)]
            sub = wd[:, :, t0[0]::2, t0[1]::2, t0[2]::2].contiguous()
            packs.append(ops.pack_weight_f16x3(sub, 1))
        return packs
    return _tensor_pack_cache(w, ("s2", tuple(padding)), build)


def _packed_folded(w):
    def build():
        wd = w.detach()
        co, ci, kd, kh, kw = wd.shape
        wf = wd.permute(0, 4, 1, 2, 3).reshape(co, kw * ci, kd, kh, 1)
        if kw * ci < 16:
            wf = torch.cat([wf, wf.new_zeros(co, 16 - kw * ci, kd, kh, 1)], 1)
        return ops.pack_weight_f16x3(wf.contiguous(), 0)
    return _tensor_pack_cache(w, "fold", build)
# ... 504 lines not shown
def conv3d(x0, weight, bias=None, stride=1, padding=0, x1=None, residual=None, want_stats=True,
           carry_in=None, carry_out=None, carry_x0=None, carry_cat=None):
    stride, padding = ops._triple(stride), ops._triple(padding)
    rows0 = getattr(x0, "_adell_rows", None)
    rows1 = getattr(x1, "_adell_rows", None) if x1 is not None else None
    route = conv3d_route(x0, weight, stride, padding,
                         None if x1 is None else x1.shape[1], residual is not None,
                         not (carry_in is None and carry_out is None and carry_x0 is None
                              and carry_cat is None), rows0 is not None)
    if route == "pointwise_gemm":
        xr = ops.ndhwc(x0)
        N, C, D, H, W = xr.shape
        y2 = linear(xr.permute(0, 2, 3, 4, 1).reshape(-1, C), weight.view(weight.shape[0], C), bias)
        return y2.view(N, D, H, W, -1).permute(0, 4, 1, 2, 3)
    _note_use(weight)
    adn = _adn_sites_of(x0, x1, weight, stride, padding)
    site = getattr(x0, "_adell_site", None) if getattr(x0, "_adell_single", False) else None
    lowrank_site = site if (route == "conv1_small" and site is not None and x1 is None
                            and carry_in is None and carry_x0 is None and not grad_observed(x0)
                            and not FLAGS["no_adn_fuse"] and not FLAGS["no_lowrank"]
                            and torch.is_grad_enabled()
                            and ops.norm_act_lowrank_ok(x0, weight.shape[0])) else None
    wp = (_packed_folded(weight) if route == "fold" else
          _packed(weight, 0) if route == "igemm" else None)
    call = _ConvCall(route, stride, padding, want_stats, _Ref(weight), carry_in, carry_out,
                     carry_x0, carry_cat, adn, lowrank_site, rows0, rows1)
    y, part = _Conv3dFn.apply(x0, x1, weight, bias, residual, wp, call)
    if want_stats and part.numel() > 0:
        y._adell_partials = part
    return y


def conv_transpose3d_route(x_shape, weight_shape):
    return "k2" if len(x_shape) == 5 and ops.convt_k2_ok(x_shape, _Shape(weight_shape)) else "igemm"


class _ConvT3dFn(torch.autograd.Function):
    @staticmethod
    def forward(ctx, x, weight, bias, wp, wref, route):
        factors = tuple(weight.shape[2:])
        y = (ops.convt_k2_fwd(x, weight, bias) if route == "k2" else
             ops.convtranspose3d_fwd(x, wp, bias, weight.shape[1], factors))
        ctx.save_for_backward(x, weight)
        ctx.route, ctx.wref, ctx.factors = route, wref, factors
        ctx.has_bias, ctx.bias_ref = bias is not None, _Ref(bias)
        return y

    @staticmethod
    def backward(ctx, dy):
        x, weight = ctx.saved_tensors
        need = ctx.needs_input_grad
        k2 = ctx.route == "k2"
        dy = ops.ndhwc(dy)
        dx = dw = db = None
        if need[0]:
            dx = (ops.convt_k2_bwd_data(dy, weight) if k2 else
                  ops.convtranspose3d_bwd_data(dy, _packed(ctx.wref.obj, 3), weight.shape[0],
                                               ctx.factors))
        want_db = ctx.has_bias and need[2]

        def weight_grads():
            dw = db = None
            if need[1] and k2 and want_db:
                dw, db = ops.convt_k2_bwd_weight(x, dy, want_db=True, factors=ctx.factors)
            elif need[1]:
                dw = (ops.convt_k2_bwd_weight(x, dy, factors=ctx.factors) if k2 else
                      ops.convtranspose3d_bwd_weight(x, dy, ctx.factors))
            if want_db and db is None:
                db = ops.bias_grad(dy)
            return dw, db

        if (need[1] or want_db) and _side_ok(ctx.wref.obj, ctx.bias_ref.obj):
            dw, db = side_run(weight_grads, (x, dy))
        else:
            dw, db = weight_grads()
        return dx, dw, db, None, None, None


def conv_transpose3d(x, weight, bias=None):
    route = conv_transpose3d_route(x.shape, weight.shape)
    wp = _packed(weight, 2) if route == "igemm" else None
    _note_use(weight)
    return _ConvT3dFn.apply(x, weight, bias, wp, _Ref(weight), route)


conv_transpose3d_k2s2 = conv_transpose3d


class _NormDropActFn(torch.autograd.Function):
    @staticmethod
    def forward(ctx, x, mean, rstd, gamma, beta, act_w, conf):
        act, act_p, per_item, drop_p, seed, offset, site, split_exp, _group = conf
        if site is not None:
            out, mask = ops.norm_act_fwd(x, mean, rstd, act, gamma=gamma, beta=beta, act_w=act_w,
                                         act_p=act_p, stats_per_item=per_item, drop_p=drop_p,
                                         seed=seed, rng_offset=offset, want_mask=True,
                                         split_exp=split_exp)
            site.x, site.mean, site.rstd, site.mask = x, mean, rstd, mask
        else:
            out = ops.norm_act_fwd(x, mean, rstd, act, gamma=gamma, beta=beta, act_w=act_w,
                                   act_p=act_p, stats_per_item=per_item, drop_p=drop_p, seed=seed,
                                   rng_offset=offset, split_exp=split_exp)
        ctx.save_for_backward(x, mean, rstd, gamma, beta, act_w)
        ctx.conf = conf
        return out

    @staticmethod
    def backward(ctx, dout):
        x, mean, rstd, gamma, beta, act_w = ctx.saved_tensors
        act, act_p, per_item, drop_p, seed, offset, site, _split_exp, group = ctx.conf
        if site is not None:
            fused, part, poff = site.fused, site.part, site.poff
            site.fused, site.part = False, None
            lowrank, site.lowrank = site.lowrank, None
            site.x = site.mean = site.rstd = site.mask = None
            if lowrank is not None:
                dx = ops.norm_act_bwd_lowrank(x, lowrank[0], lowrank[1], mean, rstd, act,
                                              act_p=act_p, drop_p=drop_p, seed=seed,
                                              rng_offset=offset)
                return dx, None, None, None, None, None, None
            if fused:
                dx = ops.norm_act_bwd_from_dt(x, ops.ndhwc(dout), mean, rstd, part, poff)
                return dx, None, None, None, None, None, None
        dact_w = None
        if act_w is not None and ctx.needs_input_grad[5]:
            dact_w = ops.prelu_wgrad(x, dout, mean, rstd, act_w, gamma=gamma, beta=beta,
                                     stats_per_item=per_item, drop_p=drop_p, seed=seed,
                                     rng_offset=offset)
        want_affine = gamma is not None and (ctx.needs_input_grad[3] or ctx.needs_input_grad[4])
        if group is not None:
            rec, dgamma, dbeta = ops.norm_act_bwd_sums(
                x, dout, mean, rstd, act, gamma=gamma, beta=beta, act_w=act_w, act_p=act_p,
                drop_p=drop_p, seed=seed, rng_offset=offset, want_affine_grads=want_affine)
            dist.all_reduce(rec, op=dist.ReduceOp.SUM, group=group)
            dx = ops.norm_act_bwd_apply_sums(x, dout, mean, rstd, rec, act, gamma=gamma, beta=beta,
                                             act_w=act_w, act_p=act_p, drop_p=drop_p, seed=seed,
                                             rng_offset=offset)
            if beta is None:
                dbeta = None
            return dx, None, None, dgamma, dbeta, dact_w, None
        dx, dgamma, dbeta = ops.norm_act_bwd(
            x, dout, mean, rstd, act, gamma=gamma, beta=beta, act_w=act_w, act_p=act_p,
            stats_per_item=per_item, drop_p=drop_p, seed=seed, rng_offset=offset,
            want_affine_grads=want_affine)
        if beta is None:
            dbeta = None
        return dx, None, None, dgamma, dbeta, dact_w, None


def norm_drop_act(x, *, norm="none", eps=1e-5, gamma=None, beta=None, running=None,
                  momentum=0.1, act="identity", act_p=0.0, act_w=None, drop_p=0.0,
                  training=False, rows_reader=None, sync_group=None):
    part = getattr(x, "_adell_partials", None)
    x = ops.ndhwc(x)
    N, C = x.shape[:2]
    V = x.shape[2] * x.shape[3] * x.shape[4]
    mean = rstd = group = None
    per_item = 1
    if norm == "instance":
        if part is None:
            part = ops.channel_partials(x.detach())
        mean, rstd = ops.stats_finalize(part, V, eps, per_item=True)
    elif norm == "batch":
        per_item = 0
        if (training and sync_group is not None
                and dist.get_world_size(group=sync_group) > 1):
            if part is None:
                part = ops.channel_partials(x.detach())
            rec = ops.bn_stats_sums(part, V)
            dist.all_reduce(rec, op=dist.ReduceOp.SUM, group=sync_group)
            mean, rstd = ops.bn_stats_from_sums(rec, eps, running, momentum)
            group = sync_group
        elif training or running is None or running[0] is None:
            if part is None:
                part = ops.channel_partials(x.detach())
            mean, rstd = ops.stats_finalize(part, V, eps, per_item=False)
            if training and running is not None and running[0] is not None:
                rm, rv, nbt = running
                if nbt is None and momentum is None:
                    raise ValueError("BatchNorm with momentum=None needs num_batches_tracked")
                ops.bn_running_update(mean, rstd, rm, rv, nbt, N * V, eps, momentum)
        else:
            rstd_c = torch.rsqrt(running[1] + eps)
            gamma = rstd_c if gamma is None else rstd_c * gamma
            shift = -running[0] * gamma
            beta = shift if beta is None else beta + shift
    elif norm != "none":
        raise NotImplementedError(f"norm {norm!r} has no HIP kernel yet")
    p = float(drop_p) if training else 0.0
    seed, offset = 0, 0
    if p > 0.0:
        seed = torch.initial_seed()
        offset = next(_dropout_counter)
    site = None
    if (norm == "instance" and gamma is None and beta is None and act_w is None
            and act in ("identity", "swish", "silu", "relu", "leaky_relu") and x.requires_grad
            and torch.is_grad_enabled() and not FLAGS["no_adn_fuse"] and CONV_PRECISION == "f16x3"
            and ops.norm_act_mask_ok(x)):
        site = AdnSite(None, None, None, None, p, act, float(act_p))
    split_exp = _rows_exponent(x, rows_reader, norm, gamma, beta, act, float(act_p), act_w, p)
    conf = (act, float(act_p), per_item, p, seed, offset, site, split_exp, group)
    out = _NormDropActFn.apply(x, mean, rstd, gamma, beta, act_w, conf)
    if site is not None:
        out._adell_site = site
    if split_exp is not None:
        out._adell_rows = ops.SplitRows(split_exp, ops.split_exponents(N, C, split_exp, x.device))
    return out


def _rows_as_volume(x):
    x = x.contiguous()
    C = x.shape[-1]
    return x.view(1, 1, 1, -1, C).permute(0, 4, 1, 2, 3)


def _volume_as_rows(y, lead_shape):
    C = y.shape[1]
    return y.permute(0, 2, 3, 4, 1).reshape(*lead_shape, C)


class _LinearFn(torch.autograd.Function):

    @staticmethod
    def forward(ctx, x, weight, bias, residual):
        N, K = weight.shape
        x2 = x.reshape(-1, K).contiguous()
        rows = x2.shape[0]
        w = weight.contiguous()
        res2 = None if residual is None else residual.reshape(rows, N).contiguous()
        split = CONV_PRECISION == "f16x3" and ops.gemm_f16x3_ok(rows, N, K, x2, K, True, w, K, True)
        if split:
            y = ops.gemm_f16x3(rows, N, K, x2, K, True, w, K, True, bias=bias, residual=res2)
        else:
            y = ops.gemm(rows, N, K, x2, K, True, w, K, True, bias=bias, residual=res2)
        ctx.save_for_backward(x2, w)
        ctx.split = split
        ctx.refs = (_Ref(weight), _Ref(bias))
        ctx.meta = (x.shape, bias is not None, residual is not None and residual.shape)
        return y.view(*x.shape[:-1], N)

    @staticmethod
    def backward(ctx, dy):
        x2, w = ctx.saved_tensors
        xshape, has_bias, res_shape = ctx.meta
        split = ctx.split
        N, K = w.shape
        rows = x2.shape[0]
        need = ctx.needs_input_grad
        dy2 = dy.reshape(rows, N).contiguous()
        dx = dw = db = dres = None
        if need[0]:
            if split and ops.gemm_f16x3_ok(rows, K, N, dy2, N, True, w, K, False):
                dx = ops.gemm_f16x3(rows, K, N, dy2, N, True, w, K, False)
            else:
                dx = ops.gemm(rows, K, N, dy2, N, True, w, K, False)
            dx = dx.view(xshape)
        def weight_grads():
            dw = db = None
            if need[1]:
                if split and ops.gemm_f16x3_ok(N, K, rows, dy2, N, False, x2, K, False):
                    dw = ops.gemm_f16x3(N, K, rows, dy2, N, False, x2, K, False)
                else:
                    dw = ops.gemm(N, K, rows, dy2, N, False, x2, K, False)
            if has_bias and need[2]:
                db = ops.bias_grad(_rows_as_volume(dy2))
            return dw, db

        if (need[1] or (has_bias and need[2])) and _side_ok(ctx.refs[0].obj, ctx.refs[1].obj):
            dw, db = side_run(weight_grads, (x2, dy2))
        else:
            dw, db = weight_grads()
        if res_shape and need[3]:
            dres = dy2.view(res_shape)
        return dx, dw, db, dres


class _MlpFn(torch.autograd.Function):

    @staticmethod
    def forward(ctx, x, w1, b1, w2, b2, residual, act, act_p):
        H, K = w1.shape
        N = w2.shape[0]
        x2 = x.reshape(-1, K).contiguous()
        rows = x2.shape[0]
        w1c, w2c = w1.contiguous(), w2.contiguous()
        res2 = None if residual is None else residual.reshape(rows, N).contiguous()
        h, g = ops.gemm_f16x3_act(rows, H, K, x2, K, True, w1c, K, True, act, act_p, bias=b1,
                                  want_act=True)
        y = ops.gemm_f16x3(rows, N, H, g, H, True, w2c, H, True, bias=b2, residual=res2)
        ctx.save_for_backward(x2, w1c, w2c, h, g)
        ctx.act = (act, act_p)
        ctx.refs = (_Ref(w1), _Ref(b1), _Ref(w2), _Ref(b2))
        ctx.meta = (x.shape, b1 is not None, b2 is not None,
                    residual is not None and residual.shape)
        return y.view(*x.shape[:-1], N)

    @staticmethod
    def backward(ctx, dy):
        x2, w1, w2, h, g = ctx.saved_tensors
        xshape, has_b1, has_b2, res_shape = ctx.meta
        H, K = w1.shape
        N = w2.shape[0]
        rows = x2.shape[0]
        need = ctx.needs_input_grad
        dy2 = dy.reshape(rows, N).contiguous()
        dh, _ = ops.gemm_f16x3_act(rows, H, N, dy2, N, True, w2, H, False, *ctx.act, dact_in=h)
# ... 2114 lines not shown
```

### adell_mri_amd/ops.py

```python
import collections
import ctypes
import functools
import math
import os

import numpy as np
import torch

from . import _lib
from ._lib import ACT_IDS, AdellHipError, ConvDesc, NormActDesc, check


class KernelTimer:

    def __init__(self, only=None):
        self.records = []
        self._agg = None
        self.only = None if only is None else set(only)
        self.active = True

    def start(self):
        e = torch.cuda.Event(enable_timing=True)
        e.record()
        return e
# ... 972 lines not shown
                            act_p=0.0, drop_p=0.0, seed=0, rng_offset=0):
    _require_cuda(x, dout, mean, rstd, gamma, beta, act_w)
    x, dout = ndhwc(x), ndhwc(dout)
    C = x.shape[1]
    _record_check(rec, C)
    d = make_na_desc(x, act, 0, act_p, 0 if act_w is None else act_w.numel(), drop_p, seed,
                     rng_offset)
    dx = new_act(*x.shape, x.device)
    ws = _workspace(8 * C, x.device)
    check(_timed(NORM_ACT_FAMILY, 0.0, lambda: _lib.lib().adell_norm_act_bwd_apply_sums(
        ctypes.byref(d), _ptr(x), _ptr(dout), _ptr(mean), _ptr(rstd), _ptr(gamma), _ptr(beta),
        _ptr(act_w), _ptr(rec), _ptr(dx), _ptr(ws), ws.numel() * 4, _stream()),
        "bwd_apply", 12.0 * x.numel()))
    return dx


def channel_partials(x):
    _require_cuda(x)
    x = ndhwc(x)
    N, C = x.shape[:2]
    V = x.shape[2] * x.shape[3] * x.shape[4]
    nt = _lib.lib().adell_channel_partials_ntiles(V)
    part = torch.empty((N, nt, C, 2), device=x.device, dtype=torch.float32)
    check(_lib.lib().adell_channel_partials(_ptr(x), N, V, C, _ptr(part), _stream()))
    return part


def instance_stats(x, eps=1e-5, partials=None):
    if partials is None:
        partials = channel_partials(x)
    V = x.shape[2] * x.shape[3] * x.shape[4]
    return stats_finalize(partials, V, eps)


def make_na_desc(x, act, stats_per_item=1, act_p=0.0, act_w_n=0, drop_p=0.0, seed=0,
                 rng_offset=0):
    N, C = x.shape[:2]
    V = x.shape[2] * x.shape[3] * x.shape[4]
    act_id = ACT_IDS[act] if isinstance(act, str) else int(act)
    return NormActDesc(N, V, C, stats_per_item, act_id, act_w_n, float(act_p), float(drop_p),
                       int(seed) & 0xFFFFFFFFFFFFFFFF, int(rng_offset) & 0xFFFFFFFF)


def norm_act_mask_ok(x):
    C = x.shape[1]
    return x.dim() == 5 and C % 4 == 0 and C <= 1024 and (C & (C - 1)) == 0


NormActPlan = collections.namedtuple(
    "NormActPlan", "fwd fwd_grid bwd rows apply_grid finalize workspace mask_bytes")
NA_ROUTES = ("scalar", "float4", "fast", "narrow", "refused")
NA_FINALIZE = ("none", "per_item", "all_items")
_NA_ALIGNED = {"x": 1, "out": 2, "dout": 4, "dx": 8}
NormActStatsPlan = collections.namedtuple("NormActStatsPlan",
                                          "levels Z workspace unroll8_from unroll2_from")


def norm_act_plan(N, V, C, stats_per_item=1, drop_p=0.0, unaligned=(), want_mask=False, split=False,
                  lowrank=0, norm=True, affine_grads=False):
    d = NormActDesc(int(N), int(V), int(C), int(stats_per_item), 0, 0, 0.0, float(drop_p), 0, 0)
    al = sum(bit for name, bit in _NA_ALIGNED.items() if name not in unaligned)
    assert set(unaligned) <= set(_NA_ALIGNED), unaligned
    out = (ctypes.c_long * 10)()
    check(_lib.lib().adell_norm_act_plan(ctypes.byref(d), al, int(bool(want_mask)), int(bool(split)),
                                         int(lowrank), int(bool(norm)), int(bool(affine_grads)), out))
    o = list(out)
    return NormActPlan(NA_ROUTES[o[0]], (o[1], o[2]), NA_ROUTES[o[3]], o[4], (o[5], o[6]),
                       NA_FINALIZE[o[7]], o[8], o[9])


def norm_act_stats_plan(N, ntiles, C):
    out = (ctypes.c_long * 5)()
    check(_lib.lib().adell_norm_act_stats_plan(int(N), int(ntiles), int(C), out))
    return NormActStatsPlan(*list(out))


class SplitRows:

    __slots__ = ("exp", "xk")

    def __init__(self, exp, xk):
        self.exp, self.xk = int(exp), xk


_XK_CACHE = {}


def split_exponents(N, C, exp, device):
    key = (device, int(N) * (int(C) // 16), int(exp))
    t = _XK_CACHE.get(key)
    if t is None:
        t = _XK_CACHE[key] = torch.full((key[1],), int(exp), device=device, dtype=torch.int32)
    return t


def rows_from_f32(x, exp):
    _require_cuda(x)
    x = ndhwc(x)
    N, C = x.shape[:2]
    V = x.numel() // (N * C)
    xk = split_exponents(N, C, exp, x.device)
    out = new_act(*x.shape, x.device)
    check(_lib.lib().adell_split_rows_from_f32(_ptr(x), N, V, C, _ptr(xk), _ptr(out), _stream()))
    return out, SplitRows(exp, xk)


def rows_to_f32(rows, sr):
    _require_cuda(rows)
    rows = ndhwc(rows)
    N, C = rows.shape[:2]
    V = rows.numel() // (N * C)
    out = new_act(*rows.shape, rows.device)
    check(_lib.lib().adell_split_rows_to_f32(_ptr(rows), N, V, C, _ptr(sr.xk), _ptr(out), _stream()))
    return out


def conv3d_rows_ok(N, in_size, C0, C1, Cout, kernel, stride, padding):
    k, st = _triple(kernel), _triple(stride)
    if k != (3, 3, 3) or st != (1, 1, 1) or C0 % 16 or C1 % 16:
        return False
    d = make_conv_desc(N, tuple(in_size), C0, C1, Cout, kernel, stride, padding)
    return bool(_lib.lib().adell_conv3d_f16x3_rows_ok(ctypes.byref(d)))


def norm_act_fwd(x, mean, rstd, act, gamma=None, beta=None, act_w=None, act_p=0.0,
                 stats_per_item=1, drop_p=0.0, seed=0, rng_offset=0, want_mask=False,
                 split_exp=None):
    _require_cuda(x, mean, rstd, gamma, beta, act_w)
    x = ndhwc(x)
    d = make_na_desc(x, act, stats_per_item, act_p, 0 if act_w is None else act_w.numel(),
                     drop_p, seed, rng_offset)
    out = new_act(*x.shape, x.device)
    mask = None
    if want_mask and drop_p > 0.0:
        nbytes = _lib.lib().adell_norm_act_mask_bytes(ctypes.byref(d))
        if nbytes < 0:
            check(int(nbytes))
        mask = torch.empty((nbytes // 8,), device=x.device, dtype=torch.int64)
    if split_exp is not None:
        check(_timed(NORM_ACT_FAMILY, 0.0, lambda: _lib.lib().adell_norm_act_fwd_split(
            ctypes.byref(d), _ptr(x), _ptr(mean), _ptr(rstd), _ptr(gamma), _ptr(beta), _ptr(act_w),
            _ptr(out), int(split_exp), _ptr(mask), _stream()), "fwd", 8.0 * x.numel()))
    elif mask is not None:
        check(_timed(NORM_ACT_FAMILY, 0.0, lambda: _lib.lib().adell_norm_act_fwd_mask(
            ctypes.byref(d), _ptr(x), _ptr(mean), _ptr(rstd), _ptr(gamma), _ptr(beta), _ptr(act_w),
            _ptr(out), _ptr(mask), _stream()), "fwd", 8.0 * x.numel()))
    else:
        check(_timed(NORM_ACT_FAMILY, 0.0, lambda: _lib.lib().adell_norm_act_fwd(
            ctypes.byref(d), _ptr(x), _ptr(mean), _ptr(rstd), _ptr(gamma), _ptr(beta), _ptr(act_w),
            _ptr(out), _stream()), "fwd", 8.0 * x.numel()))
    return (out, mask) if want_mask else out


def norm_act_bwd_from_dt(x, dt, mean, rstd, partials, poff=0):
    _require_cuda(x, dt, mean, rstd, partials)
    x, dt = ndhwc(x), ndhwc(dt)
    d = make_na_desc(x, "identity", 1)
    N, C = x.shape[:2]
    ws = _workspace(4 * (2 + 2 * ((int(partials.shape[1]) + 255) // 256)) * N * C, x.device)
    check(_timed(NORM_ACT_FAMILY, 0.0, lambda: _lib.lib().adell_norm_act_bwd_from_dt(
        ctypes.byref(d), _ptr(x), _ptr(dt), _ptr(mean), _ptr(rstd), _ptr(partials),
        int(partials.shape[1]), int(partials.shape[2]), int(poff), _ptr(dt), _ptr(ws),
        ws.numel() * 4, _stream()), "bwd", 12.0 * x.numel()))
    return dt


def prelu_wgrad(x, dout, mean, rstd, act_w, gamma=None, beta=None, stats_per_item=1, drop_p=0.0,
                seed=0, rng_offset=0):
    _require_cuda(x, dout, mean, rstd, gamma, beta, act_w)
    x, dout = ndhwc(x), ndhwc(dout)
    d = make_na_desc(x, "prelu", stats_per_item, 0.0, act_w.numel(), drop_p, seed, rng_offset)
    ws = _workspace(_lib.lib().adell_prelu_wgrad_workspace(ctypes.byref(d)), x.device)
    dw = torch.empty_like(act_w)
    check(_lib.lib().adell_prelu_wgrad(ctypes.byref(d), _ptr(x), _ptr(dout), _ptr(mean), _ptr(rstd),
                                       _ptr(gamma), _ptr(beta), _ptr(dw), _ptr(ws),
                                       ws.numel() * 4, _stream()))
    return dw


def norm_act_bwd(x, dout, mean, rstd, act, gamma=None, beta=None, act_w=None, act_p=0.0,
                 stats_per_item=1, drop_p=0.0, seed=0, rng_offset=0, want_affine_grads=False):
    _require_cuda(x, dout, mean, rstd, gamma, beta, act_w)
    x, dout = ndhwc(x), ndhwc(dout)
    d = make_na_desc(x, act, stats_per_item, act_p, 0 if act_w is None else act_w.numel(),
                     drop_p, seed, rng_offset)
    dx = new_act(*x.shape, x.device)
    dgamma = dbeta = None
    if want_affine_grads:
        dgamma = torch.empty((x.shape[1],), device=x.device, dtype=torch.float32)
        dbeta = torch.empty_like(dgamma)
    ws = None
    if mean is not None or want_affine_grads:
        ws = _workspace(_lib.lib().adell_norm_act_bwd_workspace(ctypes.byref(d)), x.device)
    check(_timed(NORM_ACT_FAMILY, 0.0, lambda: _lib.lib().adell_norm_act_bwd(
        ctypes.byref(d), _ptr(x), _ptr(dout), _ptr(mean), _ptr(rstd), _ptr(gamma), _ptr(beta),
        _ptr(act_w), _ptr(dx), _ptr(dgamma), _ptr(dbeta), _ptr(ws),
        0 if ws is None else ws.numel() * 4, _stream()), "bwd", 12.0 * x.numel()))
    return dx, dgamma, dbeta


def norm_act_lowrank_ok(x, co):
    C = x.shape[1]
    return 1 <= co <= 4 and 4 <= C <= 1024 and (C & (C - 1)) == 0


def norm_act_bwd_lowrank(x, g, w, mean, rstd, act, act_p=0.0, drop_p=0.0, seed=0, rng_offset=0):
    _require_cuda(x, g, w, mean, rstd)
    x, g = ndhwc(x), ndhwc(g)
    co = g.shape[1]
    w = w.reshape(co, x.shape[1]).contiguous()
    assert g.shape[0] == x.shape[0] and g.shape[2:] == x.shape[2:]
    d = make_na_desc(x, act, 1, act_p, 0, drop_p, seed, rng_offset)
    dx = new_act(*x.shape, x.device)
    ws = _workspace(_lib.lib().adell_norm_act_bwd_workspace(ctypes.byref(d)), x.device)
    nb = 8.0 * x.numel() + 4.0 * g.numel()
    check(_timed(NORM_ACT_FAMILY, 0.0, lambda: _lib.lib().adell_norm_act_bwd_lowrank(
        ctypes.byref(d), _ptr(x), _ptr(g), _ptr(w), co, _ptr(mean), _ptr(rstd), _ptr(dx), _ptr(ws),
        ws.numel() * 4, _stream()), "bwd", nb))
    return dx


def dice_focal_fwd(prob, target, smooth, dice_eps, gamma, focal_eps, focal_alpha=1.0):
    _require_cuda(prob, target)
    prob, target = prob.contiguous(), target.contiguous()
    B = prob.shape[0]
    S = prob.numel() // B
    assert target.numel() == prob.numel()
    ws = _workspace(_lib.lib().adell_dice_focal_workspace(B, S), prob.device)
    dice = torch.empty((B,), device=prob.device, dtype=torch.float32)
    focal = torch.empty_like(dice)
    sums = torch.empty((B, 3), device=prob.device, dtype=torch.float32)
    check(_lib.lib().adell_dice_focal_fwd(_ptr(prob), _ptr(target), B, S, smooth, dice_eps, gamma,
                                          float(focal_alpha), focal_eps, _ptr(dice), _ptr(focal),
                                          _ptr(sums),
                                          _ptr(ws), ws.numel() * 4, _stream()))
    return dice, focal, sums


def dice_focal_bwd(prob, target, sums, smooth, dice_eps, gamma, focal_eps, gdice, gfocal,
                   focal_alpha=1.0):
    prob, target = prob.contiguous(), target.contiguous()
    B = prob.shape[0]
    S = prob.numel() // B
    dprob = torch.empty_like(prob)
    check(_lib.lib().adell_dice_focal_bwd(_ptr(prob), _ptr(target), B, S, smooth, dice_eps, gamma,
                                          float(focal_alpha), focal_eps, _ptr(sums), float(gdice),
                                          float(gfocal),
                                          _ptr(dprob), _stream()))
    return dprob


def dice_focal_bwd_dev(prob, target, sums, smooth, dice_eps, gamma, focal_eps, gdice, gfocal,
                       focal_alpha=1.0):
    prob, target = prob.contiguous(), target.contiguous()
    B = prob.shape[0]
    S = prob.numel() // B
    dprob = torch.empty_like(prob)
    gd = None if gdice is None else gdice.contiguous().float()
    gf = None if gfocal is None else gfocal.contiguous().float()
    check(_lib.lib().adell_dice_focal_bwd_dev(_ptr(prob), _ptr(target), B, S, smooth, dice_eps,
                                              gamma, float(focal_alpha), focal_eps, _ptr(sums),
                                              _ptr(gd), _ptr(gf), _ptr(dprob), _stream()))
    return dprob


def class_sums_fwd(p, t):
    _require_cuda(p, t)
    B, V, C = p.shape
    nbytes = _lib.lib().adell_class_sums_workspace(B, V, C)
    ws = _workspace(nbytes, p.device)
    sums = torch.empty((B, C, 3), device=p.device, dtype=torch.float32)
    check(_lib.lib().adell_class_sums_fwd(_ptr(p), _ptr(t), B, V, C, _ptr(sums), _ptr(ws),
                                          ws.numel() * 4, _stream()))
    return sums


def class_sums_bwd(t, gsums):
    _require_cuda(t, gsums)
    B, V, C = t.shape
    dp = torch.empty_like(t)
    g = gsums.contiguous()
    check(_lib.lib().adell_class_sums_bwd(_ptr(t), _ptr(g), B, V, C, _ptr(dp), _stream()))
    return dp


WEIGHT_EPOCH = 0


def _weights_changed():
    global WEIGHT_EPOCH
    WEIGHT_EPOCH += 1


def sgd_step(param, grad, buf, lr, momentum, weight_decay, nesterov, first, grad_scale=1.0):
    _require_cuda(param, grad, buf)
    check(_lib.lib().adell_sgd_step(_ptr(param), _ptr(grad), _ptr(buf), param.numel(), lr,
                                    momentum, weight_decay, int(nesterov), int(first),
                                    grad_scale, _stream()))
    _weights_changed()


def adamw_step(param, grad, exp_avg, exp_avg_sq, lr, beta1, beta2, eps, weight_decay, step,
               grad_scale=1.0, decoupled=True):
    _require_cuda(param, grad, exp_avg, exp_avg_sq)
    fn = _lib.lib().adell_adamw_step if decoupled else _lib.lib().adell_adam_step
    check(fn(_ptr(param), _ptr(grad), _ptr(exp_avg), _ptr(exp_avg_sq), param.numel(), lr, beta1,
# ... 3436 lines not shown
```

### include/adell_hip.h

```cpp
#ifndef ADELL_HIP_H
#define ADELL_HIP_H

#include <stddef.h>
#include <stdint.h>

#ifdef __cplusplus
extern "C" {
#endif
#if defined(__GNUC__) || defined(__clang__)
#pragma GCC visibility push(default)
#endif

#define ADELL_OK 0
#define ADELL_E_BADARG (-1)
#define ADELL_E_UNSUPPORTED (-2)
#define ADELL_E_HIP (-3)
#define ADELL_E_NOMEM (-4)

#define ADELL_ABI_VERSION 2

enum {
  ADELL_ACT_IDENTITY = 0,
  ADELL_ACT_SILU = 1,
  ADELL_ACT_RELU = 2,
// ... 80 lines not shown
                              const void* w_split, const float* wscale, const float* bias,
                              const float* residual, float* y, float* stat_partials,
                              int partial_rows, uint32_t* in_absmax, void* workspace,
                              size_t workspace_bytes, void* stream);
int adell_conv3d_bwd_data_f16x3_ws(const adell_conv3d_desc* d, const float* dy,
                                   const void* w_split_bwd, const float* wscale, float* dx0,
                                   float* dx1, uint32_t* dy_absmax, void* workspace,
                                   size_t workspace_bytes, void* stream);
int adell_conv3d_bwd_data_f16x3_add(const adell_conv3d_desc* d, const float* dy,
                                    const void* w_split_bwd, const float* wscale,
                                    const float* add0, float* dx0, uint32_t* dy_absmax,
                                    void* workspace, size_t workspace_bytes, void* stream);

typedef struct adell_adn_site {
  const float* y;
  const float* mean;
  const float* rstd;
  const void* keep_mask;
  float drop_p;
  float act_p;
  int32_t act;
} adell_adn_site;
int adell_conv3d_bwd_data_f16x3_adn_ntiles(const adell_conv3d_desc* d);
int adell_conv3d_bwd_data_f16x3_adn(const adell_conv3d_desc* d, const float* dy,
                                    const void* w_split_bwd, const float* wscale,
                                    const float* add0, float* dx0, float* dx1,
                                    uint32_t* dy_absmax, const adell_adn_site* site0,
                                    const adell_adn_site* site1, float* partials,
                                    int partial_rows, void* stream);

long adell_conv3d_bwd_weight_workspace(const adell_conv3d_desc* d);
int adell_conv3d_bwd_weight(const adell_conv3d_desc* d, const float* x0,
                            const float* x1, const float* dy, float* dw, float* db,
                            void* workspace, size_t workspace_bytes, void* stream);

long adell_conv3d_bwd_weight_f16x3_workspace(const adell_conv3d_desc* d);
int adell_conv3d_bwd_weight_f16x3(const adell_conv3d_desc* d, const float* x0,
                                  const float* x1, const float* dy, float* dw, float* db,
                                  const uint32_t* x_absmax, const uint32_t* dy_absmax,
                                  void* workspace, size_t workspace_bytes, void* stream);
int adell_conv3d_bwd_weight_f16x3_rows_ok(const adell_conv3d_desc* d);
int adell_conv3d_bwd_weight_f16x3_rows(const adell_conv3d_desc* d, const void* x0, const int* xk0,
                                       const void* x1, const int* xk1, const float* dy, float* dw,
                                       float* db, const uint32_t* x_absmax,
                                       const uint32_t* dy_absmax, void* workspace,
                                       size_t workspace_bytes, void* stream);
#define ADELL_WGRAD_SHARE_NONE 0
#define ADELL_WGRAD_SHARE_AUTO 1
#define ADELL_WGRAD_SHARE_ALWAYS 2
int adell_conv3d_bwd_weight_f16x3_share(const adell_conv3d_desc* d, const float* x0,
                                        const float* x1, const float* dy, float* dw, float* db,
                                        const uint32_t* x_absmax, const uint32_t* dy_absmax,
                                        void* workspace, size_t workspace_bytes, void* stream,
                                        int share);
int adell_conv3d_bwd_weight_f16x3_rows_share(const adell_conv3d_desc* d, const void* x0,
                                             const int* xk0, const void* x1, const int* xk1,
                                             const float* dy, float* dw, float* db,
                                             const uint32_t* x_absmax, const uint32_t* dy_absmax,
                                             void* workspace, size_t workspace_bytes, void* stream,
                                             int share);
#define ADELL_WGRAD_SMALL 0
#define ADELL_WGRAD_ZRING32 1
#define ADELL_WGRAD_ZRING16 2
#define ADELL_WGRAD_S2 3
#define ADELL_WGRAD_PLANE 4
int adell_conv3d_bwd_weight_f16x3_plan(const adell_conv3d_desc* d, int* out);

long adell_bias_grad_workspace(long rows, int C);
int adell_bias_grad(const float* dy, long rows, int C, float* db, void* workspace,
                    size_t workspace_bytes, void* stream);

int adell_convtranspose3d_fwd(int N, int D, int H, int W, int Cin, int Cout, int FD, int FH,
                              int FW, const float* x, const float* w_packed, const float* bias,
                              float* y, void* stream);
int adell_convtranspose3d_bwd_data(int N, int D, int H, int W, int Cin, int Cout, int FD,
                                   int FH, int FW, const float* dy, const float* w_packed_bwd,
                                   float* dx, void* stream);
int adell_convtranspose3d_fwd_f16x3(int N, int D, int H, int W, int Cin, int Cout, int FD, int FH,
                                    int FW, const float* x, const void* w_split,
                                    const float* wscale, const float* bias, float* y,
                                    uint32_t* in_absmax, void* stream);
int adell_convtranspose3d_bwd_data_f16x3(int N, int D, int H, int W, int Cin, int Cout, int FD,
                                         int FH, int FW, const float* dy, const void* w_split_bwd,
                                         const float* wscale, float* dx, uint32_t* dy_absmax,
                                         void* stream);
int adell_convtranspose3d_f16x3_plan(int N, int D, int H, int W, int Cin, int Cout, int FD, int FH,
                                     int FW, int* out);
long adell_convtranspose3d_bwd_weight_workspace(int N, int D, int H, int W, int Cin, int Cout,
                                                int FD, int FH, int FW);
int adell_convtranspose3d_bwd_weight(int N, int D, int H, int W, int Cin, int Cout, int FD,
                                     int FH, int FW, const float* x, const float* dy, float* dw,
                                     void* workspace, size_t workspace_bytes, void* stream);
int adell_convtranspose3d_k2s2_fwd(int N, int D, int H, int W, int Cin, int Cout,
                                   const float* x, const float* w_packed,
                                   const float* bias, float* y, void* stream);
int adell_convtranspose3d_k2s2_bwd_data(int N, int D, int H, int W, int Cin,
                                        int Cout, const float* dy,
                                        const float* w_packed_bwd, float* dx,
                                        void* stream);
long adell_convtranspose3d_k2s2_bwd_weight_workspace(int N, int D, int H, int W,
                                                     int Cin, int Cout);
int adell_convtranspose3d_k2s2_bwd_weight(int N, int D, int H, int W, int Cin,
                                          int Cout, const float* x, const float* dy,
                                          float* dw, void* workspace,
                                          size_t workspace_bytes, void* stream);

long adell_stats_finalize_workspace(int N, int ntiles, int C);
int adell_stats_finalize(const float* partials, int N, int ntiles, int C,
                         long count, float eps, int per_item, float* mean,
                         float* rstd, void* workspace, size_t workspace_bytes,
                         void* stream);

int adell_bn_running_update(const float* mean, const float* rstd, float* running_mean,
                            float* running_var, long long* num_batches_tracked, int C, long count,
                            float eps, float momentum, void* stream);
int adell_bn_stats_sums(const float* partials, int N, int ntiles, int C, long count, double* sums,
                        void* workspace, size_t workspace_bytes, void* stream);
int adell_bn_stats_from_sums(const double* sums, int C, float eps, float* mean, float* rstd,
                             float* running_mean, float* running_var,
                             long long* num_batches_tracked, float momentum, void* stream);
int adell_channel_partials_ntiles(long V);
int adell_channel_partials(const float* x, int N, long V, int C, float* partials,
                           void* stream);

typedef struct adell_norm_act_desc {
  int64_t N, V;
  int32_t C;
  int32_t stats_per_item;
  int32_t act;
  int32_t act_w_n;
  float act_p;
  float drop_p;
  uint64_t seed;
  uint32_t rng_offset;
} adell_norm_act_desc;

int adell_norm_act_fwd(const adell_norm_act_desc* d, const float* x,
                       const float* mean, const float* rstd, const float* gamma,
                       const float* beta, const float* act_w, float* out,
                       void* stream);

long adell_norm_act_mask_bytes(const adell_norm_act_desc* d);
int adell_norm_act_fwd_mask(const adell_norm_act_desc* d, const float* x, const float* mean,
                            const float* rstd, const float* gamma, const float* beta,
                            const float* act_w, float* out, void* keep_mask, void* stream);
int adell_norm_act_fwd_split(const adell_norm_act_desc* d, const float* x, const float* mean,
                             const float* rstd, const float* gamma, const float* beta,
                             const float* act_w, void* out_rows, int split_exp, void* keep_mask,
                             void* stream);
int adell_split_rows_from_f32(const float* x, int N, long V, int C, const int* xk, void* rows,
                              void* stream);
int adell_split_rows_to_f32(const void* rows, int N, long V, int C, const int* xk, float* x,
                            void* stream);
int adell_norm_act_bwd_from_dt(const adell_norm_act_desc* d, const float* x, const float* dt,
                               const float* mean, const float* rstd, const float* partials,
                               int ntiles, int pstride, int poff, float* dx, void* workspace,
                               size_t workspace_bytes, void* stream);

long adell_norm_act_bwd_workspace(const adell_norm_act_desc* d);
int adell_norm_act_bwd(const adell_norm_act_desc* d, const float* x, const float* dout,
                       const float* mean, const float* rstd, const float* gamma,
                       const float* beta, const float* act_w, float* dx, float* dgamma,
                       float* dbeta, void* workspace, size_t workspace_bytes,
                       void* stream);
int adell_norm_act_bwd_sums(const adell_norm_act_desc* d, const float* x, const float* dout,
                            const float* mean, const float* rstd, const float* gamma,
                            const float* beta, const float* act_w, double* sums, float* dgamma,
                            float* dbeta, void* workspace, size_t workspace_bytes, void* stream);
int adell_norm_act_bwd_apply_sums(const adell_norm_act_desc* d, const float* x, const float* dout,
                                  const float* mean, const float* rstd, const float* gamma,
                                  const float* beta, const float* act_w, const double* sums,
                                  float* dx, void* workspace, size_t workspace_bytes, void* stream);
int adell_norm_act_bwd_lowrank(const adell_norm_act_desc* d, const float* x, const float* g,
                               const float* w, int co, const float* mean, const float* rstd,
                               float* dx, void* workspace, size_t workspace_bytes, void* stream);
#define ADELL_NA_SCALAR 0
#define ADELL_NA_FLOAT4 1
#define ADELL_NA_FAST 2
#define ADELL_NA_NARROW 3
#define ADELL_NA_REFUSED 4
#define ADELL_NA_FIN_NONE 0
#define ADELL_NA_FIN_PER_ITEM 1
#define ADELL_NA_FIN_ALL_ITEMS 2
#define ADELL_NA_ALIGNED_X 1
#define ADELL_NA_ALIGNED_OUT 2
#define ADELL_NA_ALIGNED_DOUT 4
#define ADELL_NA_ALIGNED_DX 8
int adell_norm_act_plan(const adell_norm_act_desc* d, int aligned, int want_mask, int split,
                        int lowrank, int norm, int affine_grads, long* out);
int adell_norm_act_stats_plan(int N, int ntiles, int C, long* out);
long adell_prelu_wgrad_workspace(const adell_norm_act_desc* d);
int adell_prelu_wgrad(const adell_norm_act_desc* d, const float* x, const float* dout,
                      const float* mean, const float* rstd, const float* gamma, const float* beta,
                      float* dact_w, void* workspace, size_t workspace_bytes, void* stream);

long adell_dice_focal_workspace(int B, long S);
int adell_dice_focal_fwd(const float* prob, const float* target, int B, long S,
                         float smooth, float dice_eps, float gamma, float focal_alpha, float focal_eps,
                         float* dice, float* focal, float* sums, void* workspace,
                         size_t workspace_bytes, void* stream);
int adell_dice_focal_bwd(const float* prob, const float* target, int B, long S,
                         float smooth, float dice_eps, float gamma, float focal_alpha, float focal_eps,
                         const float* sums, float gdice, float gfocal, float* dprob,
                         void* stream);
int adell_dice_focal_bwd_dev(const float* prob, const float* target, int B, long S, float smooth,
                             float dice_eps, float gamma, float focal_alpha, float focal_eps,
                             const float* sums, const float* gdice, const float* gfocal,
                             float* dprob, void* stream);
long adell_class_sums_workspace(int B, long V, int C);
int adell_class_sums_fwd(const float* p, const float* t, int B, long V, int C, float* sums,
                         void* workspace, size_t workspace_bytes, void* stream);
int adell_class_sums_bwd(const float* t, const float* gsums, int B, long V, int C, float* dp,
                         void* stream);

int adell_sgd_step(float* param, const float* grad, float* momentum_buf, long n, float lr,
                   float momentum, float weight_decay, int nesterov, int first_step,
                   float grad_scale, void* stream);
int adell_adamw_step(float* param, const float* grad, float* exp_avg, float* exp_avg_sq,
                     long n, float lr, double beta1, double beta2, float eps,
                     float weight_decay, long step, float grad_scale, void* stream);
int adell_adam_step(float* param, const float* grad, float* exp_avg, float* exp_avg_sq, long n,
                    float lr, double beta1, double beta2, float eps, float weight_decay, long step,
                    float grad_scale, void* stream);

int adell_optim_step(int kind, float* param, const float* grad, float* state1, float* state2,
                     long n, float weight_decay, float eps, float grad_scale, const double* c5,
                     void* stream);
int adell_ema_update(float* shadow, const float* param, long n, float decay, void* stream);

int adell_layernorm_fwd(const float* x, const float* gamma, const float* beta, float* y,
                        float* mean, float* rstd, long rows, int C, float eps, void* stream);
long adell_layernorm_bwd_workspace(long rows, int C);
int adell_layernorm_bwd(const float* x, const float* dy, const float* gamma,
                        const float* mean, const float* rstd, float* dx, float* dgamma,
                        float* dbeta, long rows, int C, void* workspace,
                        size_t workspace_bytes, void* stream);
int adell_add_bcast(const float* a, const float* b, float* out, long n, long period,
                    void* stream);
int adell_sum_bcast(const float* g, float* db, long n, long period, void* stream);
typedef struct adell_attention_desc {
  int32_t BH;
  int32_t H;
  int32_t T, A, Dv;
  float scale;
  float drop_p;
  uint32_t rng_offset;
  uint64_t seed;
  const float* bias;
  const int32_t* labels;
  int32_t nbias, nlab;
  int32_t strided;
  int64_t stride[8][3];
} adell_attention_desc;
int adell_attention_fwd(const adell_attention_desc* d, const float* q, const float* k,
                        const float* v, float* out, float* lse, void* stream);
int adell_attention_bwd(const adell_attention_desc* d, const float* q, const float* k,
                        const float* v, const float* out, const float* dout, const float* lse,
                        float* dq, float* dk, float* dv, void* stream);
#define ADELL_ATT_VALU 0
#define ADELL_ATT_MFMA_RESIDENT 1
#define ADELL_ATT_MFMA_STREAMED 2
#define ADELL_ATT_REFUSED 3
int adell_attention_plan(int pass, int T, int A, int Dv, int aligned, int* out);
long adell_attention_bias_grad_workspace_floats(int nbias, int T);
int adell_attention_bias_grad(const adell_attention_desc* d, const float* q, const float* k,
                              const float* v, const float* out, const float* dout,
                              const float* lse, float* dbias, float* workspace,
                              long workspace_floats, void* stream);

int adell_copy_channels(float* full, float* part, long V, int Cfull, int Cpart, int coff,
                        int direction, void* stream);
int adell_interp_nearest_fwd(const float* x, float* y, int N, int C, int Di, int Hi, int Wi,
                             int Do, int Ho, int Wo, void* stream);
int adell_interp_nearest_bwd(const float* dy, float* dx, int N, int C, int Di, int Hi, int Wi,
                             int Do, int Ho, int Wo, void* stream);
int adell_interp_linear_fwd(const float* x, float* y, int N, int C, int Di, int Hi, int Wi,
                            int Do, int Ho, int Wo, float scale_d, float scale_h, float scale_w,
                            int align_corners, void* stream);
int adell_interp_linear_bwd(const float* dy, float* dx, int N, int C, int Di, int Hi, int Wi,
                            int Do, int Ho, int Wo, float scale_d, float scale_h, float scale_w,
                            int align_corners, void* stream);

int adell_fold_x_taps(const float* x, float* out, int N, int D, int H, int W, int Cin, int K,
                      int P, int Cp, void* stream);
int adell_scale_bc(const float* x, const float* s, float* y, int N, long V, int C, void* stream);
long adell_scale_bc_dscale_workspace_floats(int N, long V, int C);
int adell_scale_bc_dscale(const float* x, const float* dy, float* ds, int N, long V, int C,
                          float* workspace, void* stream);

int adell_cse_apply(const float* x, const float* s, const float* c, const float* inv,
                    const float* acc, float* y, int N, long V, int C, void* stream);
long adell_cse_apply_bwd_workspace_floats(int N, long V, int C);
int adell_cse_apply_bwd(const float* x, const float* dy, const float* s, const float* c,
                        const float* inv, float* dx, float* ds, float* dc, int N, long V, int C,
                        float* workspace, void* stream);
int adell_bcast_nc(const float* g, float* out, int N, long V, int C, float scale, void* stream);

int adell_maxpool3d_fwd(const adell_conv3d_desc* d, const float* x, float* y,
                        int32_t* argmax, void* stream);
int adell_maxpool3d_bwd(const adell_conv3d_desc* d, const float* dy, const int32_t* argmax,
                        float* dx, void* stream);

int adell_dwconv3d_fwd(int N, int C, int D, int H, int W, int KD, int KH, int KW,
                       const float* x, const float* w, const float* bias, float* y,
                       void* stream);
int adell_dwconv3d_bwd_data(int N, int C, int D, int H, int W, int KD, int KH, int KW,
// ... 582 lines not shown
```

Measured before the change: 63.47 volumes/s.

## Fuse instance-norm statistics finalize into norm-act forward and backward kernels

Adds a fused path in which the norm+activation fast kernel folds the per-tile partial sums into mean/rstd (forward) or c1/c2 (backward) in shared memory, instead of launching a separate finalize kernel first. The goal is to cut a kernel launch and a round trip through global memory per norm layer. Each block recomputes the channel statistics redundantly, and the path is gated to small C and small partial buffers. Forward use needs callers to switch to the new fwd_stats entry point, which may not be wired in yet.

```diff
diff --git a/adell_mri_amd/_lib.py b/adell_mri_amd/_lib.py
--- a/adell_mri_amd/_lib.py
+++ b/adell_mri_amd/_lib.py
@@ -141,6 +141,16 @@
     "adell_norm_act_bwd": (_i, [ctypes.POINTER(NormActDesc)] + [_vp] * 11 + [ctypes.c_size_t, _vp]),
     "adell_norm_act_plan": (_i, [ctypes.POINTER(NormActDesc)] + [_i] * 6 + [_vp]),
     "adell_norm_act_stats_plan": (_i, [_i, _i, _i, _vp]),
+    "adell_norm_act_fwd_stats": (_i, [ctypes.POINTER(NormActDesc), _vp, _vp, _i, _l, _f] + [_vp] * 7
+                                 + [ctypes.c_size_t, _vp]),
+    "adell_norm_act_fwd_mask_stats": (_i, [ctypes.POINTER(NormActDesc), _vp, _vp, _i, _l, _f] + [_vp] * 8
+                                      + [ctypes.c_size_t, _vp]),
+    "adell_norm_act_fwd_split_stats": (_i, [ctypes.POINTER(NormActDesc), _vp, _vp, _i, _l, _f] + [_vp] * 6
+                                       + [_i, _vp, _vp, ctypes.c_size_t, _vp]),
+    "adell_norm_act_set_fused_finalize": (_i, [_i]),
+    "adell_norm_act_get_fused_finalize": (_i, []),
+    "adell_norm_act_finalize_counts": (_i, [_vp]),
+    "adell_norm_act_finalize_plan": (_i, [ctypes.POINTER(NormActDesc)] + [_i] * 5 + [_vp]),
     "adell_norm_act_bwd_sums": (_i, [ctypes.POINTER(NormActDesc)] + [_vp] * 11 + [ctypes.c_size_t, _vp]),
     "adell_norm_act_bwd_apply_sums": (_i, [ctypes.POINTER(NormActDesc)] + [_vp] * 10
                                       + [ctypes.c_size_t, _vp]),
diff --git a/adell_mri_amd/csrc/norm_act.hip b/adell_mri_amd/csrc/norm_act.hip
--- a/adell_mri_amd/csrc/norm_act.hip
+++ b/adell_mri_amd/csrc/norm_act.hip
@@ -10,53 +10,153 @@
 #define ADELL_FIN8_SPAN 56
 #define ADELL_FIN2_SPAN 32
 
+template <int STEP, int U = 8, typename IDX = size_t>
+__device__ __forceinline__ void adell_fold_rows(const float* __restrict__ p, IDX rs, int t0,
+                                                int rows, double& s1, double& s2) {
+  int t = t0;
+  for (; t + (U - 1) * STEP < rows; t += U * STEP) {
+    float2 v[U];
+#pragma unroll
+    for (int u = 0; u < U; ++u) v[u] = *reinterpret_cast<const float2*>(p + (IDX)(t + STEP * u) * rs);
+#pragma unroll
+    for (int u = 0; u < U; ++u) {
+      s1 += (double)v[u].x;
+      s2 += (double)v[u].y;
+    }
+  }
+  for (; t < rows; t += STEP) {
+    const float2 v = *reinterpret_cast<const float2*>(p + (IDX)t * rs);
+    s1 += (double)v.x;
+    s2 += (double)v.y;
+  }
+}
+__device__ __forceinline__ void adell_fold8_slot(const float* __restrict__ p, size_t rs, int rows,
+                                                 int sl, double& s1, double& s2) {
+  adell_fold_rows<8>(p, rs, sl, rows, s1, s2);
+}
+__device__ __forceinline__ void adell_fold32_slot(const float* __restrict__ p, size_t rs, int rows,
+                                                  int sl, double& A, double& B) {
+  double a0 = 0.0, a1 = 0.0, b0 = 0.0, b1 = 0.0;
+  adell_fold_rows<64>(p, rs, sl, rows, a0, b0);
+  adell_fold_rows<64>(p, rs, sl + 32, rows, a1, b1);
+  A = a0 + a1;
+  B = b0 + b1;
+}
+template <int SLOTS, int CH, int UNROLL = SLOTS>
+__device__ __forceinline__ void adell_fold_slots(const double* sh, int cl, double& A, double& B) {
+  A = 0.0;
+  B = 0.0;
+#pragma unroll UNROLL
+  for (int k = 0; k < SLOTS; ++k) {
+    A += sh[(k * CH + cl) * 2];
+    B += sh[(k * CH + cl) * 2 + 1];
+  }
+}
+__device__ __forceinline__ void adell_stats_from_sums(double a, double b, double cnt, float eps,
+                                                      float& mean, float& rstd) {
+  const double m = a / cnt;
+  double var = b / cnt - m * m;
+  if (var < 0.0) var = 0.0;
+  mean = (float)m;
+  rstd = (float)(1.0 / sqrt(var + (double)eps));
+}
+__device__ __forceinline__ void adell_c12_from_sums(double A, double B, double g, double count,
+                                                    float& c1, float& c2) {
+  c1 = (float)(g * A / count);
+  c2 = (float)(g * B / count);
+}
+
+#define ADELL_NA_FUSE_CAP_BYTES (64 * 1024)
+#define ADELL_NA_FUSE_MAXC 256
+struct NaFin {
+  const float* part;
+  float* mean;
+  float* rstd;
+  double count;
+  int rows, pstride, poff;
+  float eps;
+};
+
+template <int SLOTS, int G, typename Fin>
+__device__ __forceinline__ void adell_fin_block(const NaFin& f, int C, int n, double* sh, Fin fin) {
+  constexpr int CH = 256 / SLOTS;
+  constexpr int K = SLOTS == 8 ? 4 : 2;
+  const int cl = threadIdx.x % CH, sl = threadIdx.x / CH;
+  const unsigned rs = (unsigned)f.pstride * 2;
+  const float* base = f.part + ((size_t)n * f.rows * f.pstride + f.poff) * 2;
+  for (int c0 = 0; c0 < C; c0 += G * CH) {
+    float2 v[G][K];
+#pragma unroll
+    for (int g = 0; g < G; ++g) {
+      const unsigned c2 = (unsigned)min(c0 + g * CH + cl, C - 1) * 2;
+#pragma unroll
+      for (int k = 0; k < K; ++k)
+        v[g][k] = *reinterpret_cast<const float2*>(
+            base + ((unsigned)min(sl + (SLOTS == 8 ? 8 : 32) * k, f.rows - 1) * rs + c2));
+    }
+#pragma unroll
+    for (int g = 0; g < G; ++g) {
+      const float* p = base + (unsigned)min(c0 + g * CH + cl, C - 1) * 2;
+      double s1 = 0.0, s2 = 0.0;
+      if constexpr (SLOTS == 8) {
+#pragma unroll
+        for (int k = 0; k < K; ++k)
+          if (sl + 8 * k < f.rows) {
+            s1 += (double)v[g][k].x;
+            s2 += (double)v[g][k].y;
+          }
+        adell_fold_rows<8, 4, unsigned>(p, rs, sl + 8 * K, f.rows, s1, s2);
+      } else {
+        double a1 = 0.0, b1 = 0.0;
+        if (sl < f.rows) {
+          s1 += (double)v[g][0].x;
+          s2 += (double)v[g][0].y;
+        }
+        if (sl + 32 < f.rows) {
+          a1 += (double)v[g][1].x;
+          b1 += (double)v[g][1].y;
+        }
+        adell_fold_rows<64, 2, unsigned>(p, rs, sl + 64, f.rows, s1, s2);
+        adell_fold_rows<64, 2, unsigned>(p, rs, sl + 96, f.rows, a1, b1);
+        s1 = s1 + a1;
+        s2 = s2 + b1;
+      }
+      sh[((g * SLOTS + sl) * CH + cl) * 2] = s1;
+      sh[((g * SLOTS + sl) * CH + cl) * 2 + 1] = s2;
+    }
+    __syncthreads();
+    if (threadIdx.x < G * CH) {
+      const int g = threadIdx.x / CH, c = c0 + threadIdx.x;
+      if (c < C) {
+        double A, B;
+        adell_fold_slots<SLOTS, CH, 4>(sh + g * SLOTS * CH * 2, threadIdx.x % CH, A, B);
+        fin(c, A, B);
+      }
+    }
+    __syncthreads();
+  }
+}
+
 __global__ __launch_bounds__(256) void adell_stats_finalize_kernel(
     const float* __restrict__ part, int N, int ntiles, int C, double count, float eps,
     int per_item, float* __restrict__ mean, float* __restrict__ rstd) {
-  __shared__ double sh[8][32][2];
+  __shared__ double sh[8 * 32 * 2];
   const int cl = threadIdx.x & 31, sl = threadIdx.x >> 5;
   const int c = blockIdx.x * 32 + cl;
   const int nbeg = per_item ? blockIdx.y : 0, nend = per_item ? blockIdx.y + 1 : N;
   double s1 = 0.0, s2 = 0.0;
   if (c < C) {
-    for (int n = nbeg; n < nend; ++n) {
-      const float* p = part + ((size_t)n * ntiles * C + c) * 2;
-      int t = sl;
-      for (; t + ADELL_FIN8_SPAN < ntiles; t += 64) {
-        float2 v[8];
-#pragma unroll
-        for (int u = 0; u < 8; ++u)
-          v[u] = *reinterpret_cast<const float2*>(p + (size_t)(t + 8 * u) * C * 2);
-#pragma unroll
-        for (int u = 0; u < 8; ++u) {
-          s1 += (double)v[u].x;
-          s2 += (double)v[u].y;
-        }
-      }
-      for (; t < ntiles; t += 8) {
-        const float2 v = *reinterpret_cast<const float2*>(p + (size_t)t * C * 2);
-        s1 += (double)v.x;
-        s2 += (double)v.y;
-      }
-    }
-  }
-  sh[sl][cl][0] = s1;
-  sh[sl][cl][1] = s2;
+    for (int n = nbeg; n < nend; ++n)
+      adell_fold8_slot(part + ((size_t)n * ntiles * C + c) * 2, (size_t)C * 2, ntiles, sl, s1, s2);
+  }
+  sh[(sl * 32 + cl) * 2] = s1;
+  sh[(sl * 32 + cl) * 2 + 1] = s2;
   __syncthreads();
   if (sl == 0 && c < C) {
-    double a = 0.0, b = 0.0;
-#pragma unroll
-    for (int k = 0; k < 8; ++k) {
-      a += sh[k][cl][0];
-      b += sh[k][cl][1];
-    }
-    const double cnt = per_item ? count : count * N;
-    const double m = a / cnt;
-    double var = b / cnt - m * m;
-    if (var < 0.0) var = 0.0;
+    double a, b;
+    adell_fold_slots<8, 32>(sh, cl, a, b);
     const size_t o = per_item ? (size_t)blockIdx.y * C + c : (size_t)c;
-    mean[o] = (float)m;
-    rstd[o] = (float)(1.0 / sqrt(var + (double)eps));
+    adell_stats_from_sums(a, b, per_item ? count : count * N, eps, mean[o], rstd[o]);
   }
 }
 
@@ -319,6 +419,7 @@
   int rev;
   int split;
   float split_scale;
+  NaFin fin;
 };
 
 __global__ __launch_bounds__(256) void adell_norm_act_fwd_kernel(NormActArgs a) {
@@ -434,7 +535,7 @@
   const long j0 = jbeg + threadIdx.x;                                                        \
   const long stride = (long)gridDim.x * 256
 #endif
-template <int ACT> __global__ void adell_norm_act_fwd_fast_kernel(NormActArgs a);
+template <int ACT, bool FUSED = false> __global__ void adell_norm_act_fwd_fast_kernel(NormActArgs a);
 
 static int adell_na_fill(NormActArgs* a, const adell_norm_act_desc* d) {
   ADELL_REQUIRE(d != nullptr, "norm_act: null descriptor");
@@ -551,7 +652,62 @@
   return p;
 }
 
+static int g_adell_na_fused_finalize = 1;
+static long g_adell_na_fin_counts[4] = {0, 0, 0, 0};
+
+extern "C" int adell_norm_act_set_fused_finalize(int on) {
+  g_adell_na_fused_finalize = on != 0;
+  return ADELL_OK;
+}
+extern "C" int adell_norm_act_get_fused_finalize(void) { return g_adell_na_fused_finalize; }
+extern "C" int adell_norm_act_finalize_counts(long* out) {
+  ADELL_REQUIRE(out, "norm_act_finalize_counts: null pointer");
+  for (int i = 0; i < 4; ++i) out[i] = g_adell_na_fin_counts[i];
+  return ADELL_OK;
+}
+
+struct AdellNaFinPlan {
+  int fused;
+  long rows;
+  long bytes;
+};
+static AdellNaFinPlan adell_na_fin_plan(int route, int fin, long N, long ntiles, long C, bool two_level) {
+  AdellNaFinPlan f = {0, 0, 0};
+  if (ntiles <= 0) return f;
+  const AdellNaStatsPlan sp = adell_na_stats_plan(N, ntiles, C);
+  f.rows = two_level && sp.levels == 2 ? sp.Z : ntiles;
+  f.bytes = f.rows * C * 8;
+  f.fused = g_adell_na_fused_finalize && route == ADELL_NA_FAST && fin == ADELL_NA_FIN_PER_ITEM &&
+            C <= ADELL_NA_FUSE_MAXC && f.bytes <= ADELL_NA_FUSE_CAP_BYTES;
+  return f;
+}
+static int adell_na_fwd_fin(const adell_norm_act_desc* d) {
+  const bool keeps_waves = d->act == ADELL_ACT_LEAKY_RELU || d->act == ADELL_ACT_PRELU ||
+                           d->act == ADELL_ACT_GELU || d->act == ADELL_ACT_TANH || d->act == ADELL_ACT_ELU;
+  if (!keeps_waves) return ADELL_NA_FIN_NONE;
+  return d->stats_per_item && d->N <= 65535 ? ADELL_NA_FIN_PER_ITEM : ADELL_NA_FIN_ALL_ITEMS;
+}
+
 static bool adell_na_al16(const void* p) { return ((uintptr_t)p & 15) == 0; }
+
+extern "C" int adell_norm_act_finalize_plan(const adell_norm_act_desc* d, int aligned, int lowrank,
+                                            int affine_grads, int fwd_ntiles, int bwd_ntiles,
+                                            long* out) {
+  ADELL_REQUIRE(d && out && d->N > 0 && d->V > 0 && d->C > 0, "norm_act_finalize_plan: bad arguments");
+  ADELL_REQUIRE(lowrank >= 0 && lowrank <= 4 && fwd_ntiles >= 0 && bwd_ntiles >= 0,
+                "norm_act_finalize_plan: bad arguments");
+  const AdellNaPlan p =
+      adell_na_plan(d, (aligned & ADELL_NA_ALIGNED_X) != 0, (aligned & ADELL_NA_ALIGNED_OUT) != 0,
+                    (aligned & ADELL_NA_ALIGNED_DOUT) != 0, (aligned & ADELL_NA_ALIGNED_DX) != 0,
+                    false, false, lowrank, true, affine_grads != 0);
+  const AdellNaFinPlan f = adell_na_fin_plan(p.fwd, adell_na_fwd_fin(d), d->N, fwd_ntiles, d->C, true);
+  const AdellNaFinPlan b = bwd_ntiles > 0
+                               ? adell_na_fin_plan(p.bwd, p.finalize, d->N, bwd_ntiles, d->C, true)
+                               : adell_na_fin_plan(p.bwd, p.finalize, d->N, p.rows, d->C, false);
+  out[0] = f.fused; out[1] = f.rows; out[2] = f.bytes;
+  out[3] = b.fused; out[4] = b.rows; out[5] = b.bytes;
+  return ADELL_OK;
+}
 
 extern "C" int adell_norm_act_plan(const adell_norm_act_desc* d, int aligned, int want_mask,
                                    int split, int lowrank, int norm, int affine_grads, long* out) {
@@ -576,7 +732,8 @@
                                    const float* mean, const float* rstd,
                                    const float* gamma, const float* beta,
                                    const float* act_w, float* out, void* keep_mask,
-                                   void* stream, int split = 0, int split_exp = 0) {
+                                   void* stream, int split = 0, int split_exp = 0,
+                                   const NaFin* fin = nullptr) {
   NormActArgs a = {};
   int rc = adell_na_fill(&a, d);
   if (rc != ADELL_OK) return rc;
@@ -597,8 +754,14 @@
     return ADELL_E_UNSUPPORTED;
   }
   a.vec = p.fwd == ADELL_NA_FLOAT4;
+  if (fin) {
+    ADELL_REQUIRE(p.fwd == ADELL_NA_FAST && d->C <= ADELL_NA_FUSE_MAXC, "norm_act_fwd: fused finalize off its route");
+    a.fin = *fin;
+  }
   const dim3 grid((unsigned)p.fwd_gx, (unsigned)p.fwd_gy);
-  if (p.fwd == ADELL_NA_FAST || p.fwd == ADELL_NA_NARROW) {
+  if (fin) {
+    ADELL_ACT_DISPATCH_LR(adell_norm_act_fwd_fast_kernel, d->act, grid, (hipStream_t)stream, a);
+  } else if (p.fwd == ADELL_NA_FAST || p.fwd == ADELL_NA_NARROW) {
     ADELL_ACT_DISPATCH(adell_norm_act_fwd_fast_kernel, d->act, grid, (hipStream_t)stream, a);
   } else {
     hipLaunchKernelGGL(adell_norm_act_fwd_kernel, grid, dim3(256), 0, (hipStream_t)stream, a);
@@ -636,6 +799,82 @@
                 "norm_act_fwd_split: C must be a power of two in 16..1024, the tensors 16-byte aligned");
   return adell_norm_act_fwd_impl(d, x, mean, rstd, gamma, beta, act_w, (float*)out_rows,
                                  d->drop_p > 0.f ? keep_mask : nullptr, stream, 1, split_exp);
+}
+
+static int adell_norm_act_fwd_stats_impl(const adell_norm_act_desc* d, const float* x,
+                                         const float* partials, int ntiles, long count, float eps,
+                                         float* mean, float* rstd, const float* gamma,
+                                         const float* beta, const float* act_w, float* out,
+                                         void* keep_mask, void* workspace, size_t workspace_bytes,
+                                         void* stream, int split, int split_exp) {
+  ADELL_REQUIRE(d && d->N > 0 && d->V > 0 && d->C > 0 && ntiles > 0 && count > 0,
+                "norm_act_fwd_stats: bad dims");
+  ADELL_REQUIRE(d->stats_per_item == 1, "norm_act_fwd_stats: instance statistics only");
+  ADELL_REQUIRE(d->N <= 65535, "norm_act_fwd_stats: at most 65535 items (one grid row each)");
+  const int N = (int)d->N, C = d->C;
+  const AdellNaStatsPlan sp = adell_na_stats_plan(N, ntiles, C);
+  ADELL_REQUIRE(sp.levels == 1 || (workspace && (long)workspace_bytes >= sp.ws_bytes),
+                "norm_act_fwd_stats: workspace too small");
+  ADELL_REQUIRE(x && out && partials && mean && rstd, "norm_act_fwd_stats: null pointer");
+  const AdellNaPlan p = adell_na_plan(d, adell_na_al16(x), adell_na_al16(out), true, true,
+                                      keep_mask != nullptr, split != 0, 0, false, false);
+  const AdellNaFinPlan f = adell_na_fin_plan(p.fwd, adell_na_fwd_fin(d), N, ntiles, C, true);
+  if (!f.fused) {
+    const int rc = adell_stats_finalize(partials, N, ntiles, C, count, eps, 1, mean, rstd, workspace,
+                                        workspace_bytes, stream);
+    if (rc != ADELL_OK) return rc;
+    if (p.fwd == ADELL_NA_FAST) ++g_adell_na_fin_counts[1];
+    return adell_norm_act_fwd_impl(d, x, mean, rstd, gamma, beta, act_w, out, keep_mask, stream, split,
+                                   split_exp);
+  }
+  NaFin fin = {partials, mean, rstd, (double)count, ntiles, C, 0, eps};
+  if (sp.levels == 2) {
+    hipLaunchKernelGGL(adell_stats_fold_kernel, dim3(adell_cdiv(C, 32), N, sp.Z), dim3(256), 0,
+                       (hipStream_t)stream, partials, ntiles, C, sp.Z, (float*)workspace, C, 0);
+    fin.part = (const float*)workspace;
+    fin.rows = sp.Z;
+  }
+  ++g_adell_na_fin_counts[0];
+  return adell_norm_act_fwd_impl(d, x, nullptr, nullptr, gamma, beta, act_w, out, keep_mask, stream,
+                                 split, split_exp, &fin);
+}
+
+extern "C" int adell_norm_act_fwd_stats(const adell_norm_act_desc* d, const float* x,
+                                        const float* partials, int ntiles, long count, float eps,
+                                        float* mean, float* rstd, const float* gamma,
+                                        const float* beta, const float* act_w, float* out,
+                                        void* workspace, size_t workspace_bytes, void* stream) {
+  return adell_norm_act_fwd_stats_impl(d, x, partials, ntiles, count, eps, mean, rstd, gamma, beta,
+                                       act_w, out, nullptr, workspace, workspace_bytes, stream, 0, 0);
+}
+
+extern "C" int adell_norm_act_fwd_mask_stats(const adell_norm_act_desc* d, const float* x,
+                                             const float* partials, int ntiles, long count,
+                                             float eps, float* mean, float* rstd,
+                                             const float* gamma, const float* beta,
+                                             const float* act_w, float* out, void* keep_mask,
+                                             void* workspace, size_t workspace_bytes, void* stream) {
+  ADELL_REQUIRE(d && (d->drop_p == 0.f || keep_mask), "norm_act_fwd_mask_stats: null mask");
+  return adell_norm_act_fwd_stats_impl(d, x, partials, ntiles, count, eps, mean, rstd, gamma, beta,
+                                       act_w, out, d->drop_p > 0.f ? keep_mask : nullptr, workspace,
+                                       workspace_bytes, stream, 0, 0);
+}
+
+extern "C" int adell_norm_act_fwd_split_stats(const adell_norm_act_desc* d, const float* x,
+                                              const float* partials, int ntiles, long count,
+                                              float eps, float* mean, float* rstd,
+                                              const float* gamma, const float* beta,
+                                              const float* act_w, void* out_rows, int split_exp,
+                                              void* keep_mask, void* workspace,
+                                              size_t workspace_bytes, void* stream) {
+  ADELL_REQUIRE(d && d->N > 0 && d->V > 0 && d->C > 0, "norm_act_fwd_split_stats: bad dims");
+  ADELL_REQUIRE(split_exp >= -100 && split_exp <= 100, "norm_act_fwd_split_stats: bad exponent");
+  ADELL_REQUIRE(adell_na_plan(d, adell_na_al16(x), adell_na_al16(out_rows), true, true,
+                              keep_mask != nullptr, true, 0, false, false).fwd == ADELL_NA_FAST,
+                "norm_act_fwd_split_stats: C must be a power of two in 16..1024, the tensors 16-byte aligned");
+  return adell_norm_act_fwd_stats_impl(d, x, partials, ntiles, count, eps, mean, rstd, gamma, beta,
+                                       act_w, (float*)out_rows, d->drop_p > 0.f ? keep_mask : nullptr,
+                                       workspace, workspace_bytes, stream, 1, split_exp);
 }
 
 typedef _Float16 na_half8 __attribute__((ext_vector_type(8)));
@@ -737,6 +976,7 @@
   const float* lr_g;
   const float* lr_w;
   int lr_co, lr_shift;
+  NaFin fin;
 };
 
 __device__ __forceinline__ void adell_na_bwd_elem(const NormActBwdArgs& a, float x, float dout,
@@ -889,39 +1129,21 @@
     const float* __restrict__ part, int ntiles, int C, double count,
     const float* __restrict__ gamma, float* __restrict__ c1, float* __restrict__ c2,
     int pstride, int poff) {
-  __shared__ double sh[32][8][2];
+  __shared__ double sh[32 * 8 * 2];
   const int cl = threadIdx.x & 7, sl = threadIdx.x >> 3;
   const int c = blockIdx.x * 8 + cl, n = blockIdx.y;
-  double a0 = 0.0, a1 = 0.0, b0 = 0.0, b1 = 0.0;
-  if (c < C) {
-    int t = sl;
-    for (; t + ADELL_FIN2_SPAN < ntiles; t += 64) {
-      const float2 u =
-          *reinterpret_cast<const float2*>(part + (((size_t)n * ntiles + t) * pstride + poff + c) * 2);
-      const float2 v = *reinterpret_cast<const float2*>(
-          part + (((size_t)n * ntiles + t + 32) * pstride + poff + c) * 2);
-      a0 += (double)u.x; b0 += (double)u.y;
-      a1 += (double)v.x; b1 += (double)v.y;
-    }
-    for (; t < ntiles; t += 32) {
-      const float2 u =
-          *reinterpret_cast<const float2*>(part + (((size_t)n * ntiles + t) * pstride + poff + c) * 2);
-      a0 += (double)u.x; b0 += (double)u.y;
-    }
-  }
-  sh[sl][cl][0] = a0 + a1;
-  sh[sl][cl][1] = b0 + b1;
+  double s1 = 0.0, s2 = 0.0;
+  if (c < C)
+    adell_fold32_slot(part + ((size_t)n * ntiles * pstride + poff + c) * 2, (size_t)pstride * 2,
+                      ntiles, sl, s1, s2);
+  sh[(sl * 8 + cl) * 2] = s1;
+  sh[(sl * 8 + cl) * 2 + 1] = s2;
   __syncthreads();
   if (sl == 0 && c < C) {
-    double A = 0.0, B = 0.0;
-#pragma unroll
-    for (int k = 0; k < 32; ++k) {
-      A += sh[k][cl][0];
-      B += sh[k][cl][1];
-    }
+    double A, B;
+    adell_fold_slots<32, 8>(sh, cl, A, B);
     const double g = gamma ? (double)gamma[c] : 1.0;
-    c1[(size_t)n * C + c] = (float)(g * A / count);
-    c2[(size_t)n * C + c] = (float)(g * B / count);
+    adell_c12_from_sums(A, B, g, count, c1[(size_t)n * C + c], c2[(size_t)n * C + c]);
   }
 }
 
@@ -1087,7 +1309,12 @@
     float* c2 = c1 + (size_t)d->N * d->C;
     a.part = part; a.c1 = c1; a.c2 = c2;
     adell_na_bwd_partials_launch(a, d, p, st);
-    if (p.finalize == ADELL_NA_FIN_PER_ITEM)
+    const AdellNaFinPlan f = adell_na_fin_plan(p.bwd, p.finalize, d->N, a.ntiles, d->C, false);
+    if (p.finalize == ADELL_NA_FIN_PER_ITEM && p.bwd == ADELL_NA_FAST) ++g_adell_na_fin_counts[f.fused ? 2 : 3];
+    if (f.fused) {
+      a.fin = NaFin{part, nullptr, nullptr, (double)d->V, a.ntiles, d->C, 0, 0.f};
+      a.c1 = a.c2 = nullptr;
+    } else if (p.finalize == ADELL_NA_FIN_PER_ITEM)
       hipLaunchKernelGGL(adell_na_bwd_finalize_item_kernel,
                          dim3(adell_cdiv(d->C, 8), (unsigned)d->N), dim3(256), 0, st,
                          (const float*)part, a.ntiles, d->C, (double)d->V, gamma, c1, c2, d->C, 0);
@@ -1123,6 +1350,42 @@
   }
 }
 
+__device__ __forceinline__ void adell_fin_fwd_block(const NaFin& f, int C, int n, float* st) {
+  __shared__ double fsh[512];
+  const bool store = blockIdx.x == 0;
+  adell_fin_block<8, 1>(f, C, n, fsh, [&](int ch, double A, double B) {
+    float m, r;
+    adell_stats_from_sums(A, B, f.count, f.eps, m, r);
+    st[ch] = m;
+    st[C + ch] = r;
+    if (store) {
+      f.mean[(size_t)n * C + ch] = m;
+      f.rstd[(size_t)n * C + ch] = r;
+    }
+  });
+}
+__device__ __forceinline__ void adell_fin_bwd_block(const NaFin& f, int C, int n, const float* gamma,
+                                                 float* st) {
+  __shared__ double fsh[4 * 512];
+  adell_fin_block<32, 4>(f, C, n, fsh, [&](int ch, double A, double B) {
+    const double g = gamma ? (double)gamma[ch] : 1.0;
+    adell_c12_from_sums(A, B, g, f.count, st[ch], st[C + ch]);
+  });
+}
+
+__shared__ float g_adell_fin_c12[2 * ADELL_NA_FUSE_MAXC];
+__device__ __forceinline__ void adell_fin_bwd_fold(const NormActBwdArgs& a, int n) {
+  if (a.fin.part != nullptr) adell_fin_bwd_block(a.fin, a.C, n, a.gamma, g_adell_fin_c12);
+}
+__device__ __forceinline__ void adell_fin_bwd_consts(NaConst& k, const NormActBwdArgs& a, int c) {
+  if (a.fin.part == nullptr) return;
+#pragma unroll
+  for (int j = 0; j < 4; ++j) {
+    k.c1[j] = g_adell_fin_c12[(c + j) & (a.C - 1)];
+    k.c2[j] = g_adell_fin_c12[a.C + ((c + j) & (a.C - 1))];
+  }
+}
+
 struct NaLowRank {
   float w[4][4];
 };
@@ -1147,15 +1410,25 @@
   return r;
 }
 
-template <int ACT>
+template <int ACT, bool FUSED>
 __global__ __launch_bounds__(256) void adell_norm_act_fwd_fast_kernel(NormActArgs a) {
   const int n = a.rev ? (int)(gridDim.y - 1 - blockIdx.y) : (int)blockIdx.y;
   const long n4 = a.VC >> 2;
   ADELL_EW_RANGE(n4);
   const int c = (int)((j0 << 2) & (a.C - 1));
+  __shared__ float fst[2 * ADELL_NA_FUSE_MAXC];
+  constexpr bool fused = FUSED;
+  if constexpr (FUSED) adell_fin_fwd_block(a.fin, a.C, n, fst);
   NaConst k;
-  adell_na_consts(k, a.mean, a.rstd, a.gamma, a.beta, a.act_w, a.act_w_n, a.act_p, nullptr,
-                  nullptr, (long)n * a.stat_stride_n, c, a.C - 1);
+  adell_na_consts(k, fused ? nullptr : a.mean, fused ? nullptr : a.rstd, a.gamma, a.beta, a.act_w,
+                  a.act_w_n, a.act_p, nullptr, nullptr, (long)n * a.stat_stride_n, c, a.C - 1);
+  if (fused) {
+#pragma unroll
+    for (int j = 0; j < 4; ++j) {
+      k.m[j] = fst[(c + j) & (a.C - 1)];
+      k.r[j] = fst[a.C + ((c + j) & (a.C - 1))];
+    }
+  }
   const float keep_scale = a.drop_p > 0.f ? 1.0f / (1.0f - a.drop_p) : 1.0f;
   const float4* xin = reinterpret_cast<const float4*>(a.x) + (long)n * n4;
   float4* yout = reinterpret_cast<float4*>(a.out) + (long)n * n4;
@@ -1228,8 +1501,10 @@
   ADELL_EW_RANGE(n4);
   const int c = (int)((j0 << 2) & (a.C - 1));
   NaConst k;
+  adell_fin_bwd_fold(a, n);
   adell_na_consts(k, a.mean, a.rstd, a.gamma, a.beta, a.act_w, a.act_w_n, a.act_p, a.c1, a.c2,
                   (long)n * a.stat_stride_n, c, a.C - 1);
+  adell_fin_bwd_consts(k, a, c);
   const float keep_scale = a.drop_p > 0.f ? 1.0f / (1.0f - a.drop_p) : 1.0f;
   const float4* xin = reinterpret_cast<const float4*>(a.x) + (long)n * n4;
   const float4* gin = reinterpret_cast<const float4*>(a.dout) + (long)n * n4;
@@ -1350,8 +1625,10 @@
   ADELL_EW_RANGE(n4);
   const int c = (int)((j0 << 2) & (a.C - 1));
   NaConst k;
+  adell_fin_bwd_fold(a, n);
   adell_na_consts(k, a.mean, a.rstd, nullptr, nullptr, nullptr, 0, 0.f, a.c1, a.c2,
                   (long)n * a.stat_stride_n, c, a.C - 1);
+  adell_fin_bwd_consts(k, a, c);
   const float4* xin = reinterpret_cast<const float4*>(a.x) + (long)n * n4;
   const float4* gin = reinterpret_cast<const float4*>(a.dout) + (long)n * n4;
   float4* dxo = reinterpret_cast<float4*>(a.dx) + (long)n * n4;
@@ -1398,6 +1675,7 @@
                 "norm_act_bwd_from_dt: needs a power-of-two C in 4..1024 and aligned tensors");
   const AdellNaStatsPlan sp = adell_na_stats_plan(d->N, ntiles, d->C);
   const int Z = sp.Z;
+  const AdellNaFinPlan fp = adell_na_fin_plan(p.bwd, p.finalize, d->N, ntiles, d->C, true);
   ADELL_REQUIRE(workspace && workspace_bytes >= sizeof(float) * 2 * (size_t)d->N * d->C + (size_t)sp.ws_bytes,
                 "norm_act_bwd_from_dt: workspace too small");
   ADELL_REQUIRE(x && dt && dx && mean && rstd && partials, "norm_act_bwd_from_dt: null pointer");
@@ -1413,10 +1691,16 @@
     pstride = d->C;
     poff = 0;
   }
-  hipLaunchKernelGGL(adell_na_bwd_finalize_item_kernel, dim3(adell_cdiv(d->C, 8), (unsigned)d->N),
-                     dim3(256), 0, st, partials, ntiles, d->C, (double)d->V, (const float*)nullptr,
-                     c1, c2, pstride, poff);
   a.x = x; a.dout = dt; a.mean = mean; a.rstd = rstd; a.c1 = c1; a.c2 = c2; a.dx = dx;
+  ++g_adell_na_fin_counts[fp.fused ? 2 : 3];
+  if (fp.fused) {
+    a.fin = NaFin{partials, nullptr, nullptr, (double)d->V, ntiles, pstride, poff, 0.f};
+    a.c1 = a.c2 = nullptr;
+  } else {
+    hipLaunchKernelGGL(adell_na_bwd_finalize_item_kernel, dim3(adell_cdiv(d->C, 8), (unsigned)d->N),
+                       dim3(256), 0, st, partials, ntiles, d->C, (double)d->V, (const float*)nullptr,
+                       c1, c2, pstride, poff);
+  }
   hipLaunchKernelGGL(adell_na_bwd_apply_dt_kernel, dim3((unsigned)p.apply_gx, (unsigned)p.apply_gy),
                      dim3(256), 0, st, a);
   ADELL_CHECK_HIP(hipGetLastError());
diff --git a/adell_mri_amd/functional.py b/adell_mri_amd/functional.py
--- a/adell_mri_amd/functional.py
+++ b/adell_mri_amd/functional.py
@@ -26,7 +26,16 @@
          "no_seq_attention": bool(os.environ.get("ADELL_NO_SEQ_ATTENTION")),
          "no_mlp_fuse": not bool(os.environ.get("ADELL_MLP_FUSE")),
          "mlp_min_elems": int(os.environ.get("ADELL_MLP_MIN_ELEMS", str(1 << 20))),
-         "no_cinfold_wgrad_f16": bool(os.environ.get("ADELL_NO_CINFOLD_WGRAD_F16"))}
+         "no_cinfold_wgrad_f16": bool(os.environ.get("ADELL_NO_CINFOLD_WGRAD_F16")),
+         "no_fused_finalize": bool(os.environ.get("ADELL_NO_FUSED_FINALIZE"))}
+_FUSED_FINALIZE_PUSHED = [None]
+
+
+def _sync_fused_finalize():
+    want = not FLAGS["no_fused_finalize"]
+    if _FUSED_FINALIZE_PUSHED[0] is not want:
+        ops.norm_act_set_fused_finalize(want)
+        _FUSED_FINALIZE_PUSHED[0] = want
 
 
 def set_conv_precision(mode):
@@ -837,6 +846,7 @@
                   momentum=0.1, act="identity", act_p=0.0, act_w=None, drop_p=0.0,
                   training=False, rows_reader=None, sync_group=None):
     part = getattr(x, "_adell_partials", None)
+    _sync_fused_finalize()
     x = ops.ndhwc(x)
     N, C = x.shape[:2]
     V = x.shape[2] * x.shape[3] * x.shape[4]
diff --git a/adell_mri_amd/ops.py b/adell_mri_amd/ops.py
--- a/adell_mri_amd/ops.py
+++ b/adell_mri_amd/ops.py
@@ -1148,6 +1148,68 @@
     return (out, mask) if want_mask else out
 
 
+def norm_act_fwd_stats(x, partials, eps, act, gamma=None, beta=None, act_w=None, act_p=0.0,
+                       drop_p=0.0, seed=0, rng_offset=0, want_mask=False, split_exp=None):
+    _require_cuda(x, partials, gamma, beta, act_w)
+    x = ndhwc(x)
+    d = make_na_desc(x, act, 1, act_p, 0 if act_w is None else act_w.numel(), drop_p, seed, rng_offset)
+    N, nt, C, _ = partials.shape
+    V = x.shape[2] * x.shape[3] * x.shape[4]
+    out = new_act(*x.shape, x.device)
+    mean = torch.empty((N, C), device=x.device, dtype=torch.float32)
+    rstd = torch.empty_like(mean)
+    mask = None
+    if want_mask and drop_p > 0.0:
+        nbytes = _lib.lib().adell_norm_act_mask_bytes(ctypes.byref(d))
+        if nbytes < 0:
+            check(int(nbytes))
+        mask = torch.empty((nbytes // 8,), device=x.device, dtype=torch.int64)
+    nbytes = _lib.lib().adell_stats_finalize_workspace(N, nt, C)
+    ws = _workspace(nbytes, x.device) if nbytes > 0 else None
+    head = (ctypes.byref(d), _ptr(x), _ptr(partials), nt, int(V), float(eps), _ptr(mean), _ptr(rstd),
+            _ptr(gamma), _ptr(beta), _ptr(act_w), _ptr(out))
+    tail = (_ptr(ws), 0 if ws is None else ws.numel() * 4, _stream())
+    if split_exp is not None:
+        call = lambda: _lib.lib().adell_norm_act_fwd_split_stats(*head, int(split_exp), _ptr(mask), *tail)
+    elif mask is not None:
+        call = lambda: _lib.lib().adell_norm_act_fwd_mask_stats(*head, _ptr(mask), *tail)
+    else:
+        call = lambda: _lib.lib().adell_norm_act_fwd_stats(*head, *tail)
+    check(_timed(NORM_ACT_FAMILY, 0.0, call, "fwd", 8.0 * x.numel()))
+    return out, mean, rstd, mask
+
+
+def norm_act_set_fused_finalize(on):
+    check(_lib.lib().adell_norm_act_set_fused_finalize(1 if on else 0))
+
+
+def norm_act_get_fused_finalize():
+    return bool(_lib.lib().adell_norm_act_get_fused_finalize())
+
+
+def norm_act_finalize_counts():
+    out = (ctypes.c_long * 4)()
+    check(_lib.lib().adell_norm_act_finalize_counts(out))
+    return tuple(out)
+
+
+NormActFinalizePlan = collections.namedtuple(
+    "NormActFinalizePlan", "fwd_fused fwd_rows fwd_bytes bwd_fused bwd_rows bwd_bytes")
+
+
+def norm_act_finalize_plan(N, V, C, fwd_ntiles=0, bwd_ntiles=0, act="swish", stats_per_item=1,
+                           affine_grads=False, lowrank=0, unaligned=()):
+    d = NormActDesc(int(N), int(V), int(C), int(stats_per_item),
+                    ACT_IDS[act] if isinstance(act, str) else int(act), 0, 0.0, 0.0, 0, 0)
+    al = sum(bit for name, bit in _NA_ALIGNED.items() if name not in unaligned)
+    out = (ctypes.c_long * 6)()
+    check(_lib.lib().adell_norm_act_finalize_plan(ctypes.byref(d), al, int(lowrank),
+                                                  int(bool(affine_grads)), int(fwd_ntiles),
+                                                  int(bwd_ntiles), out))
+    o = list(out)
+    return NormActFinalizePlan(bool(o[0]), o[1], o[2], bool(o[3]), o[4], o[5])
+
+
 def norm_act_bwd_from_dt(x, dt, mean, rstd, partials, poff=0):
     _require_cuda(x, dt, mean, rstd, partials)
     x, dt = ndhwc(x), ndhwc(dt)
diff --git a/include/adell_hip.h b/include/adell_hip.h
--- a/include/adell_hip.h
+++ b/include/adell_hip.h
@@ -256,6 +256,25 @@
                               void* stream);
 int adell_split_rows_to_f32(const void* rows, int N, long V, int C, const int* xk, float* x,
                             void* stream);
+int adell_norm_act_fwd_stats(const adell_norm_act_desc* d, const float* x, const float* partials,
+                             int ntiles, long count, float eps, float* mean, float* rstd,
+                             const float* gamma, const float* beta, const float* act_w, float* out,
+                             void* workspace, size_t workspace_bytes, void* stream);
+int adell_norm_act_fwd_mask_stats(const adell_norm_act_desc* d, const float* x, const float* partials,
+                                  int ntiles, long count, float eps, float* mean, float* rstd,
+                                  const float* gamma, const float* beta, const float* act_w,
+                                  float* out, void* keep_mask, void* workspace,
+                                  size_t workspace_bytes, void* stream);
+int adell_norm_act_fwd_split_stats(const adell_norm_act_desc* d, const float* x, const float* partials,
+                                   int ntiles, long count, float eps, float* mean, float* rstd,
+                                   const float* gamma, const float* beta, const float* act_w,
+                                   void* out_rows, int split_exp, void* keep_mask, void* workspace,
+                                   size_t workspace_bytes, void* stream);
+int adell_norm_act_set_fused_finalize(int on);
+int adell_norm_act_get_fused_finalize(void);
+int adell_norm_act_finalize_counts(long* out);
+int adell_norm_act_finalize_plan(const adell_norm_act_desc* d, int aligned, int lowrank,
+                                 int affine_grads, int fwd_ntiles, int bwd_ntiles, long* out);
 int adell_norm_act_bwd_from_dt(const adell_norm_act_desc* d, const float* x, const float* dt,
                                const float* mean, const float* rstd, const float* partials,
                                int ntiles, int pstride, int poff, float* dx, void* workspace,
```

Result: slower. 62.34 volumes/s (-1.8%).
